# nianticlabs/panoptic-forecasting

Hardware: AMD Instinct MI355X
Metric: forecast frames/sec @1024x2048, 3-in->dt=3 bg (higher is better)
Workload: dtype f32 as 2 fp16 terms/operand, 3 MFMA products, f32 accumulate (strict f32: fp32_only); 1 GPU; configs[1] bg short-term forecast 3-in dt=3 @1024x2048: 3 warp/splats + HarDNet-70 + upsample/argmax; resident_frames_per_gpu=128, streams=4, sub_batch=32, launch=hipGraph replay, sub-batches staggered, weights=random-init, calibrated (tests/golden/calib_seed1234.json), world=1, device=AMD Radeon Graphics, backend=single process

## Files before the change

include/pfhip.h:

```cpp
#ifndef PFHIP_H
#define PFHIP_H

#include <stddef.h>
#include <stdint.h>

#ifdef __cplusplus
extern "C" {
#endif

#define PF_OK 0
#define PF_EINVAL (-1)
#define PF_EWORKSPACE (-2)
#define PF_EBLOB (-3)
#define PF_EHIP (-4)
#define PF_EUNSUPPORTED (-5)

typedef struct pf_plan pf_plan;

int pf_version(void);
const char *pf_last_error(void);

#define PF_SPLAT_PER_FRAME 1
#define PF_SPLAT_PER_SAMPLE_SENTINEL 2
int pf_warp_splat_workspace(int B, int T, int H, int W, int per_frame, size_t *bytes);
int pf_warp_splat(const float *depth, const uint8_t *depth_mask, const uint8_t *seg, int seg_channels,
                  const float *Kinv, const float *E, const float *T_tgt, const float *Einv,
                  const float *K, int B, int T_total, int t_first, int T, int H, int W, int per_frame,
                  uint8_t *out_seg, float *out_depth, int64_t *out_result2d,
                  void *ws, size_t ws_bytes, void *stream);

int pf_hardnet_plan_create(const void *blob_host, size_t bytes, int in_ch, int n_cls, pf_plan **out);
void pf_hardnet_plan_destroy(pf_plan *plan);
int pf_hardnet_workspace(const pf_plan *plan, int B, int H, int W, size_t *bytes);

#define PF_STATUS_RANGE 1u
#define PF_STATUS_RANGE_LOW 2u
#define PF_WS_STATUS_OFFSET 0
#define PF_WS_STICKY_OFFSET 4
#define PF_WS_STATUS_BYTES 2048
int pf_hardnet_status(const void *ws, unsigned *status, void *stream);
int pf_hardnet_status_sticky(void *ws, unsigned *status, int clear, void *stream);
int pf_hardnet_status_reset(void *ws, void *stream);
int pf_hardnet_range_maxima(const pf_plan *plan, const void *ws, float *maxima, int cap, int *n_ops, void *stream);

#define PF_HOP_NONE 0
#define PF_HOP_TRAINID_LUT 1
#define PF_HOP_DEPTH_U16 2

int pf_bg_forward(const pf_plan *plan, const void *seg, int seg_is_i64, const float *depth,
                  const uint8_t *depth_mask, float depth_mean, float depth_std, int hop_flags,
                  float min_depth, float max_depth, int B, int T, int H, int W, int out_h, int out_w,
                  void *out_seg, int out_seg_is_i64, float *out_logits, float *out_orig_logits,
                  void *ws, size_t ws_bytes, void *stream);

int pf_hardnet_forward_dense(const pf_plan *plan, const float *x, int B, int H, int W, int out_h,
                             int out_w, void *out_seg, int out_seg_is_i64, float *out_logits,
                             float *out_orig_logits, void *ws, size_t ws_bytes, void *stream);

int pf_hop_export(const void *seg, int seg_is_i64, int seg_mode, const float *depth, size_t n, uint8_t *out_seg,
                  uint16_t *out_depth_u16, void *stream);
int pf_hop_load(const uint16_t *depth_u16, size_t n, float min_depth, float max_depth, float *out_depth,
                uint8_t *out_mask, void *stream);

int pf_bg_augment(const uint8_t *seg_src, const uint8_t *label_src, const uint16_t *depth_src, int B, int T, int Hs, int Ws,
                  const int *y_map, const int *x_map, const int *y_arr, const int *x_arr, int oh, int ow, int pad_label,
                  float min_depth, float max_depth, uint8_t *out_seg, uint8_t *out_label, float *out_depth,
                  uint8_t *out_mask, void *stream);

int pf_fg_assemble(const float *bboxes, const uint8_t *feat_mask, const float *depth, const int32_t *classes,
                   const int32_t *feat_row, const float *feat_table, int N, int T, int T_in, int M, int use_ulbr,
                   double max_depth, double filter_car_gap, int img_w, float *trajectories, uint8_t *bbox_masks,
                   uint8_t *bbox_vel_masks, uint8_t *feat_masks, float *depths, uint8_t *depth_masks, int64_t *classes_out,
                   float *one_hot_classes, float *final_bboxes, float *feats, void *stream);

int pf_panoptic_merge_workspace(int n_instances, size_t *bytes);
int pf_panoptic_merge(const void *background, int bg_kind, const float *bg_depth, const uint8_t *bg_depth_mask,
                      const float *masks, int MH, int MW, const float *boxes, int box_is_ulbr,
                      const float *inst_depth, const int64_t *classes, const int32_t *inst_offsets,
                      int n_instances, int B, int H, int W, int use_depth_sorting, int panoptic_ids,
                      int clear_things, void *out, int out_is_i64, void *ws, size_t ws_bytes, void *stream);
int pf_panoptic_encode(const void *seg, int seg_is_i64, int convert_to_ids, int B, int H, int W, uint8_t *out_rgb,
                       int32_t *out_ids, uint8_t *out_present, void *stream);
int pf_panoptic_max_ids(void);

#define PF_PQ_STATUS_FULL 1u
#define PF_PQ_STATUS_VALUE 2u
int pf_pq_workspace(int B, size_t *bytes);
int pf_pq_table_slots(void);
int pf_pq_accumulate(const void *pred, int pred_is_i64, const void *gt, int gt_is_i64, int fmt, int crowd, int n_cls, int B,
                     int H, int W, double *acc, double *per_image, void *ws, size_t ws_bytes, void *stream);
int pf_pq_status(const void *ws, void *stream, int *host_status);
int pf_pq_status_reset(void *ws, void *stream);

int pf_bg_dense_input(const void *frames, int kind, int channels, const float *depth, const uint8_t *depth_mask, float depth_mean,
                      float depth_std, int B, int T, int H, int W, float *x, void *stream);

int pf_seg_loss_workspace(int B, int out_h, int out_w, size_t *bytes);
int pf_seg_loss(const float *logits, int B, int C, int Hin, int Win, const void *labels, int labels_i64, int out_h,
                int out_w, int ignore_index, double *out3, void *ws, size_t ws_bytes, void *stream);

int pf_fg_weights_size(int flags, size_t *raw_floats, size_t *packed_floats);
int pf_fg_pack(const float *raw, float *packed, int flags, void *stream);
int pf_fg_workspace(int N, int T_in, int T_out, int flags, size_t *bytes);
int pf_fg_forward(const float *packed, int flags, int N, int T_in, int T_out, int odom_T, const float *trajs,
                  const float *traj_mask, const float *vel_mask, const float *feats, const int64_t *output_inds,
                  const float *odom, const float *depths, const float *depth_mask, const int64_t *classes,
                  float *traj_norm, float *traj_unnorm, float *mask_feats, float *output_feats, float *masks,
                  void *ws, size_t ws_bytes, void *stream);

int pf_odom_weights_size(int flags, size_t *raw_floats, size_t *packed_floats);
int pf_odom_pack(const float *raw, float *packed, int flags, void *stream);
int pf_odom_forward(const float *packed, int flags, int B, int T_in, int T_out, const float *inps, float *out,
                    float *out_norm, void *stream);

int pf_odom_train_workspace(int B, int T_in, int T_out, int flags, size_t *bytes);
int pf_odom_train_forward(const float *packed, int flags, int B, int T_in, int T_out, const float *inps, float *out,
                          float *out_norm, void *ws, size_t ws_bytes, void *stream);
int pf_odom_backward(const float *packed, int flags, int B, int T_in, int T_out, const float *inps, const float *out_norm,
                     const float *grad_out, const float *grad_out_norm, void *ws, size_t ws_bytes, float *grad_raw,
                     void *stream);

int pf_set_option(const char *name, int value);
int pf_hardnet_plan_set_option(pf_plan *plan, const char *name, int value);

typedef struct pf_train pf_train;
int pf_train_create(const void *blob, size_t blob_bytes, int in_ch, int n_cls, pf_train **out);
void pf_train_destroy(pf_train *t);
int pf_train_autotune(pf_train *t, int enable);
int pf_train_tuned_shapes(const pf_train *t, int *rows, int cap_rows, int *n_rows);
int pf_train_path_stats(const pf_train *t, int *stats, int cap, int *n);
int pf_train_param_count(const pf_train *t, size_t *n_floats);
int pf_train_param_layout(const pf_train *t, int op_index, size_t *w_off, size_t *aux_off, int *has_bn);
int pf_train_workspace(const pf_train *t, int B, int H, int W, int out_h, int out_w, size_t *bytes);
int pf_train_forward_backward(const pf_train *t, float *theta, float *grad, int accumulate_grads, const void *seg, int seg_is_i64,
                              const float *depth, const uint8_t *depth_mask, float depth_mean, float depth_std, int T,
                              const float *x_dense, int B, int H, int W, const void *labels, int labels_i64, int out_h, int out_w,
                              int ignore_index, float loss_scale, float bn_momentum, float bn_eps, int update_running_stats,
                              double *out3, void *ws, size_t ws_bytes, void *stream);
int pf_train_tensor_view(const pf_train *t, const char *name, int want_grad, int B, int H, int W, int out_h, int out_w,
                         size_t *ws_offset, int *channels, int *h, int *w);
int pf_sgd_workspace(size_t *bytes);
int pf_sgd_step(float *theta, float *grad, float *momentum_buf, const uint8_t *trainable, size_t n, float lr, float momentum,
                float weight_decay, float clip_norm, float clip_value, int first_step, void *ws, size_t ws_bytes, void *stream);

int pf_hardnet_tensor_view(const pf_plan *plan, const char *name, int B, int H, int W,
                           size_t *ws_offset, int *channels, int *h, int *w);
int pf_hardnet_tensor_read(const pf_plan *plan, const char *name, int B, int H, int W, const void *ws, float *dst, void *stream);
int pf_s4_pack(const float *src, void *dst, int B, int C, int H, int W, unsigned *status, void *stream);
int pf_s4_unpack(const void *src, float *dst, int B, int C, int H, int W, void *stream);
int pf_hardnet_flops(const pf_plan *plan, int H, int W, double *flops);

int pf_profile_enable(int on);
int pf_profile_collect(void);
int pf_profile_get(int i, char *label, size_t label_cap, int *launches, double *total_ms, double *flops,
                   double *bytes);

int pf_debug_force_conv(int kind, int p0, int p1, int p2);
int pf_debug_conv_decision(int ks, int stride, int cin, int cout, int hout, int wout, int B, int need, int flags, int rounds,
                           int *out, int cap);
int pf_debug_conv_ranges(int form, int ks, int kc, int pad, int n_src, int n_cases, const int *choff, const int *ch, const int *ctotal,
                         int src_begin, int src_end, int *out, size_t cap);
int pf_debug_plan_arena(const void *blob, size_t bytes, int in_ch, int n_cls, float *out, size_t cap, size_t *n_floats,
                        long long *table, int table_ops);
int pf_debug_train_plan(const void *blob, size_t bytes, int in_ch, int n_cls, int B, int H, int W, int out_h, int out_w,
                        long long *regions, int cap_regions, int *n_regions, int *steps, int cap_steps, int *n_steps, int *slots_streams);
int pf_debug_probe_read(long long *host64);

#ifdef __cplusplus
}
#endif
#endif
```

panoptic-forecasting_amd/bg_model.py:

```python
import collections.abc
import ctypes

import torch
import torch.nn.functional as F
from torch import nn

from . import hardnet_arch as arch
from . import lib as _lib
from . import packing
from .model_api import BaseModel
from .pc_transform_model import _as_u8


PLAN_OPTIONS = {'split_f16': 'split_f16', 'split_bf16': 'split_f16', 'fuse_pool': 'fuse_pool', 'fuse_upsample': 'fuse_upsample',
                'use_tuned_table': 'use_tuned_table', 'valu_remainder': 'valu_remainder', 'conv_table_batch': 'table_batch',
                'range_guard': 'range_guard', 'fuse_front': 'fuse_front', 'fuse_pairs': 'fuse_pairs', 'share_s': 'share_s'}
PF_STATUS_RANGE, PF_STATUS_RANGE_LOW = 1, 2
PF_STATUS_ANY = PF_STATUS_RANGE | PF_STATUS_RANGE_LOW
PF_WS_STATUS_BYTES = 2048


class _Pending:
    __slots__ = ('slot', 'event', 'stream', 'args', 'outs', 'done', 'stamps', 'error')


def _stamp(t):
    if not torch.is_tensor(t):
        return None
    return (t.data_ptr(), None if t.is_inference() else t._version)


def _unversioned(stamps):
    return any(s is not None and s[1] is None for s in stamps)


class LazyResult(collections.abc.MutableMapping):

    __slots__ = ('_data', '_model', '_token')

    def __init__(self, data, model, token):
        self._data, self._model, self._token = dict(data), model, token

    def _resolve(self):
        if self._token is not None:
            self._model._resolve(self._token)
            self._token = None

    def __getitem__(self, k):
        self._resolve()
        return self._data[k]

    def __setitem__(self, k, v):
        self._data[k] = v

    def __delitem__(self, k):
        self._resolve()
        del self._data[k]

    def __iter__(self):
        return iter(self._data)

    def __len__(self):
        return len(self._data)

    def __contains__(self, k):
        return k in self._data

    def keys(self):
        return self._data.keys()

    def copy(self):
        self._resolve()
        return dict(self._data)

    def __or__(self, other):
        return {**self.copy(), **other}

    def __ror__(self, other):
        return {**other, **self.copy()}

    def __reduce__(self):
        return (dict, (self.copy(),))

    def __repr__(self):
        return 'LazyResult(%s%s)' % (list(self._data), ', unchecked' if self._token is not None else '')


class _Node(nn.Module):
    """Anonymous container: gives dotted state_dict paths without any behaviour."""


def _get_or_make(root, path):
    node = root
    for part in path:
        if not hasattr(node, part):
            node.add_module(part, _Node())
        node = getattr(node, part)
    return node


class HardNetParams(nn.Module):

    def __init__(self, in_ch, n_cls):
        super().__init__()
        self.spec = arch.Spec(in_ch, n_cls)
        for op in self.spec.conv_ops():
            parts = op.name.split('.')
            if op.bn:
                holder = _get_or_make(self, parts)
                cin = 3 if op.kind == arch.OP_STEM else op.cin
                holder.add_module('conv', nn.Conv2d(cin, op.cout, op.k, op.stride, op.k // 2, bias=False))
                holder.add_module('norm', nn.BatchNorm2d(op.cout))
            else:
                parent = _get_or_make(self, parts[:-1])
                conv = nn.Conv2d(op.cin, op.cout, op.k, op.stride, 0, bias=True)
                nn.init.kaiming_normal_(conv.weight)
                parent.add_module(parts[-1], conv)
        stem = getattr(self.base, '0').conv
        w = stem.weight.data.mean(1, keepdim=True).expand(-1, in_ch, -1, -1).clone()
        stem.weight = nn.Parameter(w)

    def load_pretrained(self, path):
        sd = torch.load(path, map_location='cpu')['model_state']
        sd = {k[len('module.'):]: v for k, v in sd.items()}
        own = self.state_dict()
        for k, v in sd.items():
            if k in own and own[k].shape == v.shape:
                own[k].copy_(v)
            elif k == 'base.0.conv.weight':
                own[k].copy_(v.mean(1, keepdim=True).expand_as(own[k]))


class BGModel(BaseModel):

    def __init__(self, params):
        super().__init__()
        self.num_classes = num_classes = params['data']['num_classes']
        self.use_depth_inps = params['model'].get('use_depth_inps')
        self.num_inputs = params['model'].get('num_inputs', 1)
        self.min_depth = params['data'].get('min_depth')
        self.max_depth = params['data'].get('max_depth')
        self.convert2onehot = params['model'].get('convert2onehot')
        self.return_logits = params['model'].get('return_logits', True)
        final_w = params['model'].get('final_w')
        final_h = params['model'].get('final_h')
        self.final_size = (final_h, final_w) if final_w is not None and final_h is not None else None
        in_ch = num_classes
        if self.use_depth_inps:
            depth_norm_params = params['data'].get('depth_norm_params')
            if depth_norm_params is None:
                mean, std = torch.zeros(1), torch.zeros(1)
            else:
                mean, std = depth_norm_params
            self.depth_mean = nn.Parameter(torch.as_tensor(mean, dtype=torch.float32).reshape(1).clone(),
                                           requires_grad=False)
            self.depth_std = nn.Parameter(torch.as_tensor(std, dtype=torch.float32).reshape(1).clone(),
                                          requires_grad=False)
            in_ch += 1
        in_ch *= self.num_inputs
        self.in_ch = in_ch
        self.model = HardNetParams(in_ch, num_classes)
        pretrain = params['model'].get('hardnet', {}).get('pretrain_path')
        if pretrain is not None:
            self.model.load_pretrained(pretrain)
        self.plan_options = {c_name: int(params['model'][key]) for key, c_name in PLAN_OPTIONS.items()
                             if params['model'].get(key) is not None}
        self.on_range_overflow = params['model'].get('on_range_overflow', 'rerun')
        if self.on_range_overflow not in ('rerun', 'raise', 'ignore'):
            raise ValueError("model.on_range_overflow must be 'rerun', 'raise' or 'ignore'")
        self.range_check = params['model'].get('range_check', 'lazy')
        if self.range_check not in ('lazy', 'sync'):
            raise ValueError("model.range_check must be 'lazy' or 'sync'")
        self.range_reruns = 0
        self._pending = []
        self._pinned = None
        self._ring_next = 0
        self._plan = None
        self._ws = None
        self._norm = None
        self._trainer = None
        self._params_for_trainer = {'data': dict(params['data']), 'model': dict(params['model']),
                                    'training': dict(params.get('training') or {})}

    def load_state_dict(self, state_dict, strict=True):
        res = super().load_state_dict(state_dict, strict)
        self.invalidate()
        return res

    def invalidate(self):
        if self._pending:
            self._drain()
        if self._plan is not None:
            _lib.load().pf_hardnet_plan_destroy(self._plan)
        self._plan = None
        self._norm = None

    def __del__(self):
        try:
            self._pending = []
            self.invalidate()
        except Exception:
            pass

    def _get_plan(self):
        if self._plan is None:
            L = _lib.load()
            blob = packing.pack_blob(self.state_dict(), self.in_ch, self.num_classes)
            buf = ctypes.create_string_buffer(blob, len(blob))
            plan = ctypes.c_void_p()
            _lib.check(L.pf_hardnet_plan_create(buf, len(blob), self.in_ch, self.num_classes, ctypes.byref(plan)),
                       'pf_hardnet_plan_create')
            self._plan = plan
            for name, value in self.plan_options.items():
                _lib.check(L.pf_hardnet_plan_set_option(plan, name.encode(), value), 'pf_hardnet_plan_set_option')
            if self.use_depth_inps:
                self._norm = (float(self.depth_mean.item()), float(self.depth_std.item()))
        return self._plan

    def _workspace(self, b, h, w, device):
        L = _lib.load()
        need = ctypes.c_size_t()
        _lib.check(L.pf_hardnet_workspace(self._get_plan(), b, h, w, ctypes.byref(need)), 'pf_hardnet_workspace')
        if self._ws is None or self._ws.numel() < need.value or self._ws.device != device:
            if torch.cuda.is_current_stream_capturing():
                raise _lib.PfError('bg forward: the workspace must exist before stream capture (run one forward first)')
            self._drain()
            self._ws = torch.empty(need.value, dtype=torch.uint8, device=device)
            self._ws[:PF_WS_STATUS_BYTES].zero_()
        return self._ws

    def _guarded(self):
        return not (self.on_range_overflow == 'ignore' or self.plan_options.get('split_f16', 1) == 0
                    or self.plan_options.get('range_guard', 1) == 0)

    def range_status(self):
        if self._ws is None:
            return 0
        return int(self._ws[:4].view(torch.int32).item())

    def range_status_sticky(self, clear=False):
        if self._ws is None:
            return 0
        w = self._ws[4:8].view(torch.int32)
        v = int(w.item())
        if clear:
            w.zero_()
        return v

    def check_range(self, clear=True):
        self._drain()
        v = self.range_status_sticky(clear)
        if (v & PF_STATUS_ANY) and self._guarded():
            raise _lib.PfError('bg forward: status %d (PF_STATUS_RANGE = 1: |activation| > 65504, PF_STATUS_RANGE_LOW = 2: a tensor of '
                               'tiny values) on the two-term fp16 operand path inside a captured graph: the outputs of the flagged '
                               'replays are not usable; run eagerly (re-run on fp32) or with model.split_f16 = 0' % v)
        return v

    def range_maxima(self):
        L, plan = _lib.load(), self._get_plan()
        names = [op.name for op in self.model.spec.ops]
        buf = (ctypes.c_float * len(names))()
        n = ctypes.c_int()
        _lib.check(L.pf_hardnet_range_maxima(plan, self._ws.data_ptr(), buf, len(names), ctypes.byref(n), _lib.stream_ptr()),
                   'pf_hardnet_range_maxima')
        return {names[i]: float(buf[i]) for i in range(n.value)}

    _RING = 32

    def _resolve(self, token, owner=True):
        if token.done:
            if token.error is not None and owner:
                raise token.error
            return
        if not token.event.query():
            token.event.synchronize()
        token.done = True
        if token in self._pending:
            self._pending.remove(token)
        status = int(self._pinned[token.slot, 0])
        args, outs, stamps = token.args, token.outs, token.stamps
        token.args = token.outs = token.stamps = None
        if not (status & PF_STATUS_ANY):
            return
        if self.on_range_overflow == 'raise':
            token.error = _lib.PfError('bg forward: status %d on the two-term fp16 operand path (PF_STATUS_RANGE = 1: an activation '
                                       'exceeded 65504; PF_STATUS_RANGE_LOW = 2: a tensor of tiny values, max below 2^-6); run with '
                                       "model.split_f16 = 0 or on_range_overflow = 'rerun'" % status)
        elif stamps is not None and stamps != tuple(_stamp(t) for t in args[:3]):
            token.error = _lib.PfError('bg forward: status %d on the two-term fp16 operand path, and the input tensors of that forward were '
                                       'modified in place before its result was first touched - the fp32 re-run cannot see the original '
                                       "frame.  Keep a forward's inputs unchanged until its result has been read (or model.settle()), or "
                                       "build the model with model.range_check = 'sync'" % status)
        if token.error is not None:
            if owner:
                raise token.error
            return
        L, plan = _lib.load(), self._get_plan()
        self.range_reruns += 1
        prior = self.plan_options.get('split_f16', 1)
        _lib.check(L.pf_hardnet_plan_set_option(plan, b'split_f16', 0), 'pf_hardnet_plan_set_option')
        try:
            here = torch.cuda.current_stream()
            with torch.cuda.stream(token.stream):
                self._run_once(*args, outs=outs)
            if here != token.stream:
                here.wait_stream(token.stream)
        finally:
            _lib.check(L.pf_hardnet_plan_set_option(plan, b'split_f16', prior), 'pf_hardnet_plan_set_option')

    def _poll(self):
        while self._pending and self._pending[0].event.query():
            self._resolve(self._pending[0], owner=False)

    def _drain(self):
        while self._pending:
            self._resolve(self._pending[0], owner=False)

    def settle(self):
        self._drain()

    def run_async(self, inps, depths, depth_masks, want_logits=True, want_orig=True, hop_flags=0, seg_dtype=torch.int64,
                  own_inputs=False):
        capturing = torch.cuda.is_current_stream_capturing()
        if not capturing:
            self._poll()
        args = (inps, depths, depth_masks, want_logits, want_orig, hop_flags, seg_dtype)
        outs = self._run_once(*args)
        if not self._guarded() or capturing:
            return outs, None
        if self._pinned is None:
            self._pinned = torch.zeros((self._RING, 2), dtype=torch.int32).pin_memory()
        slot = self._ring_next
        self._ring_next = (slot + 1) % self._RING
        for t in list(self._pending):
            if t.slot == slot:
                self._resolve(t, owner=False)
        self._pinned[slot].copy_(self._ws[:8].view(torch.int32), non_blocking=True)
        token = _Pending()
        token.slot, token.args, token.outs, token.done, token.error = slot, args, outs, False, None
        token.stamps = None if own_inputs else tuple(_stamp(t) for t in args[:3])
        token.stream = torch.cuda.current_stream()
        token.event = torch.cuda.Event()
        token.event.record(token.stream)
        self._pending.append(token)
        if token.stamps is not None and _unversioned(token.stamps):
            self._resolve(token)
            return outs, None
        return outs, token

    def run(self, inps, depths, depth_masks, want_logits=True, want_orig=True, hop_flags=0, seg_dtype=torch.int64):
        outs, token = self.run_async(inps, depths, depth_masks, want_logits, want_orig, hop_flags, seg_dtype)
        if token is not None:
            self._resolve(token)
        return outs

    def _run_once(self, inps, depths, depth_masks, want_logits, want_orig, hop_flags, seg_dtype, outs=None):
        L = _lib.load()
        plan = self._get_plan()
        fused = bool(self.convert2onehot and self.use_depth_inps and inps.dim() == 4)
        if fused:
            b, t, h, w = inps.shape
        else:
            x = self._dense_input(inps, depths, depth_masks)
            b, _, h, w = x.shape
        dev = inps.device
        oh, ow = self.final_size if self.final_size is not None else (h, w)
        ws = self._workspace(b, h, w, dev)
        if outs is not None:
            seg, logits, orig = outs
        else:
            seg = torch.empty((b, oh, ow), dtype=seg_dtype, device=dev)
            logits = torch.empty((b, self.num_classes, oh, ow), dtype=torch.float32, device=dev) if want_logits else None
            orig = None
            if want_orig:
                vo, vc, vh, vw = ctypes.c_size_t(), ctypes.c_int(), ctypes.c_int(), ctypes.c_int()
                _lib.check(L.pf_hardnet_tensor_view(plan, b'finalConv', b, h, w, ctypes.byref(vo), ctypes.byref(vc),
                                                    ctypes.byref(vh), ctypes.byref(vw)), 'pf_hardnet_tensor_view')
                orig = torch.empty((b, vc.value, vh.value, vw.value), dtype=torch.float32, device=dev)
        ptr = lambda t_: t_.data_ptr() if t_ is not None else None
        i64 = int(seg_dtype == torch.int64)
        if fused:
            if inps.dtype not in (torch.uint8, torch.int64):
                inps = inps.long()
            inps = _lib.require_cuda(inps.contiguous(), 'seg')
            depths = _lib.require_cuda(depths.float().contiguous(), 'depth')
            mask = None
            if not (hop_flags & 2):
                mask = _lib.require_cuda(_as_u8(depth_masks), 'depth_mask')
            mean, std = self._norm
            rc = L.pf_bg_forward(plan, inps.data_ptr(), int(inps.dtype == torch.int64), depths.data_ptr(), ptr(mask),
                                 mean, std, hop_flags, float(self.min_depth or 0.0), float(self.max_depth or 0.0),
                                 b, t, h, w, oh, ow, seg.data_ptr(), i64, ptr(logits), ptr(orig),
                                 ws.data_ptr(), ws.numel(), _lib.stream_ptr())
            _lib.check(rc, 'pf_bg_forward')
        else:
            x = _lib.require_cuda(x.contiguous(), 'input')
            rc = L.pf_hardnet_forward_dense(plan, x.data_ptr(), b, h, w, oh, ow, seg.data_ptr(), i64, ptr(logits),
                                            ptr(orig), ws.data_ptr(), ws.numel(), _lib.stream_ptr())
            _lib.check(rc, 'pf_hardnet_forward_dense')
        return seg, logits, orig

    def _dense_input(self, inps, depths, depth_masks):
        L = _lib.load()
        if self.convert2onehot:
            b, t, h, w = inps.shape
            if inps.dtype not in (torch.uint8, torch.int64):
                inps = inps.long()
            frames, kind, c = _lib.require_cuda(inps.contiguous(), 'seg'), int(inps.dtype == torch.int64), self.num_classes
        else:
            b, t, c, h, w = inps.shape
            frames, kind = _lib.require_cuda(inps.float().contiguous(), 'seg'), 2
        dptr = mptr = None
        mean = std = 0.0
        if self.use_depth_inps:
            depths = _lib.require_cuda(depths.float().contiguous(), 'depth')
            mask = _lib.require_cuda(_as_u8(depth_masks), 'depth_mask')
            dptr, mptr = depths.data_ptr(), mask.data_ptr()
            self._get_plan()
            mean, std = self._norm
        x = torch.empty((b, t * c + (t if self.use_depth_inps else 0), h, w), dtype=torch.float32, device=inps.device)
        _lib.check(L.pf_bg_dense_input(frames.data_ptr(), kind, c, dptr, mptr, mean, std, b, t, h, w, x.data_ptr(), _lib.stream_ptr()),
                   'pf_bg_dense_input')
        return x

    def forward(self, inps, depths, depth_masks, return_orig_size=False):
        _, logits, orig = self.run(inps, depths, depth_masks, True, return_orig_size)
        return (logits, orig) if return_orig_size else logits

    def loss(self, inputs, labels):
        if self.training:
            return self._train_loss(inputs, labels)
        with torch.no_grad():
            return self._eval_loss(inputs, labels)

    def _get_trainer(self):
        from . import bg_train
        if self._trainer is None:
            self._trainer = bg_train.BGTrainer(self._params_for_trainer, device='cuda')
        if not self._trainer.is_adopted():
            self._trainer.adopt(self)
        return self._trainer

    def _train_loss(self, inputs, labels):
        from . import bg_train
        tr = self._get_trainer()
        self.invalidate()
        loss, acc = bg_train.TrainStepFunction.apply(tr, inputs, labels, *tr._adopted)
        torch._foreach_add_(self._bn_counters(), 1)
        return {'loss': loss, 'accuracy': acc}

    def _bn_counters(self):
        return [b for k, b in self.named_buffers() if k.endswith('num_batches_tracked')]

    def _eval_loss(self, inputs, labels):
        L = _lib.load()
        seg_labels = labels['seg']
        _, _, orig = self.run(inputs['seg'], inputs.get('depth'), inputs.get('depth_mask'), want_logits=False, want_orig=True)
        if seg_labels.dtype not in (torch.uint8, torch.int64):
            seg_labels = seg_labels.long()
        seg_labels = _lib.require_cuda(seg_labels.contiguous(), 'labels')
        b, c, hin, win = orig.shape
        oh, ow = seg_labels.shape[-2], seg_labels.shape[-1]
        need = ctypes.c_size_t()
        _lib.check(L.pf_seg_loss_workspace(b, oh, ow, ctypes.byref(need)), 'pf_seg_loss_workspace')
        ws = torch.empty(need.value, dtype=torch.uint8, device=orig.device)
        out3 = torch.empty(3, dtype=torch.float64, device=orig.device)
        _lib.check(L.pf_seg_loss(orig.data_ptr(), b, c, hin, win, seg_labels.data_ptr(), int(seg_labels.dtype == torch.int64), oh, ow,
                                 255, out3.data_ptr(), ws.data_ptr(), ws.numel(), _lib.stream_ptr()), 'pf_seg_loss')
        return {'loss': (out3[0] / out3[1]).float(), 'accuracy': (out3[2] / out3[1]).float()}

    @torch.no_grad()
    def predict(self, inputs, labels=None):
        (seg, logits, orig), token = self.run_async(inputs['seg'], inputs.get('depth'), inputs.get('depth_mask'),
                                                    want_logits=self.return_logits, want_orig=True)
        out = {'seg': seg, 'orig_size_logits': orig}
        if logits is not None:
            out['logits'] = logits
        if token is not None and self.range_check == 'sync':
            self._resolve(token)
            token = None
        return LazyResult(out, self, token)
```

panoptic-forecasting_amd/csrc/conv_mfma.h:

```cpp
#pragma once
#include "pf_blob.h"
#include "pf_common.h"

namespace pf {

struct ConvArgs {
    const float *src[kConvMaxSrc];
    int src_ctotal[kConvMaxSrc];
    int src_choff[kConvMaxSrc];
    int src_cstart[kConvMaxSrc + 1];
    int src_chunk0[kConvMaxSrc + 1];
    int n_src;
    const float *wpk;
    const float *bias;
    float *dst;
    int dst_ctotal, dst_choff;
    int Cin, Cout, Hin, Win, Hout, Wout;
    int tilesX, tilesY, nchunks, relu;
    const float *zero_page;
    int ntiles;
    int no_bias;
    int pool;
    const float *res;
    int res_ctotal, res_choff, Hres, Wres;
    float res_sh, res_sw;
    int res_lds_off;
    int res_rows, res_cols;
    unsigned res_magic_cs, res_magic_cols;
    const float *wrem;
    int rem;
    int src_begin, src_end;
    int chunk_begin, chunk_end;
    long long *probe;
    unsigned *status;
    unsigned *range_slot;
    int kacc;
    int accum;
    float acc_scale;
    int dst_fmt;
    int dst_c4;
    int dst_limit;
    int src_fmt;
    int src_c4[kConvMaxSrc];
    int src_g0[kConvMaxSrc];
    int src_gn[kConvMaxSrc];
    int src_ent0[kConvMaxSrc + 1];
    float *share;
    int share_off;
    int share_cout;
    float share_scale;
};

typedef _Float16 split_t;
typedef split_t split_x2 __attribute__((ext_vector_type(2)));
typedef split_t split_x4 __attribute__((ext_vector_type(4)));
typedef split_t split_x8 __attribute__((ext_vector_type(8)));
constexpr float kSplitMaxAbs = 65504.f;
__device__ __forceinline__ void split_terms2(float x0, float x1, split_x2 &hi, split_x2 &mid) {
#if defined(__HIP_DEVICE_COMPILE__)
    typedef float f32x2 __attribute__((ext_vector_type(2)));
    hi = __builtin_convertvector(f32x2{x0, x1}, split_x2);
    const unsigned hu = __builtin_bit_cast(unsigned, hi);
    unsigned mu;
    asm("v_fma_mixlo_f16 %0, %1, -1.0, %2 op_sel_hi:[1,0,0]" : "=v"(mu) : "v"(hu), "v"(x0));
    asm("v_fma_mixhi_f16 %0, %1, -1.0, %2 op_sel:[1,0,0] op_sel_hi:[1,0,0]" : "+v"(mu) : "v"(hu), "v"(x1));
    mid = __builtin_bit_cast(split_x2, mu);
#endif
}
__device__ __forceinline__ float range_acc(float m, float a, float b, float c, float d) {
#if defined(__HIP_DEVICE_COMPILE__)
    asm("v_max3_f32 %0, %0, |%1|, |%2|" : "+v"(m) : "v"(a), "v"(b));
    asm("v_max3_f32 %0, %0, |%1|, |%2|" : "+v"(m) : "v"(c), "v"(d));
#endif
    return m;
}
constexpr float kRangeTarget = 8.0f;
constexpr float kRangeLowMax = 0.015625f;
__device__ __forceinline__ bool range_sampled() {
#if defined(__HIP_DEVICE_COMPILE__)
    const unsigned total = gridDim.x * gridDim.y * gridDim.z;
    const unsigned id = blockIdx.x + gridDim.x * (blockIdx.y + gridDim.y * blockIdx.z);
    const unsigned mask = total >= 16u ? (1u << (28 - __builtin_clz(total))) - 1u : 0u;
    return (((id * 0x9E3779B1u) >> 9) & mask) == 0u;
#else
    return false;
#endif
}
__device__ __forceinline__ void range_commit(unsigned *status, unsigned *slot, float m) {
#if defined(__HIP_DEVICE_COMPILE__)
    if (status == nullptr) return;
    if (!(m <= kSplitMaxAbs)) atomicOr(status, 1u);
    if (slot == nullptr || !range_sampled()) return;
    const unsigned mb = __builtin_bit_cast(unsigned, m);
    unsigned wm = 0;
    unsigned long long above = __builtin_amdgcn_ballot_w64(mb > wm);
    while (above != 0) {
        wm = (unsigned)__builtin_amdgcn_readlane((int)mb, (int)__builtin_ctzll(above));
        above = __builtin_amdgcn_ballot_w64(mb > wm);
    }
    const unsigned lane_id = __builtin_amdgcn_mbcnt_hi(~0u, __builtin_amdgcn_mbcnt_lo(~0u, 0u));
    if (lane_id == (unsigned)__builtin_ctzll(__builtin_amdgcn_ballot_w64(true))) atomicMax(slot, wm | 1u);
#endif
}
template <typename V4>
__device__ __forceinline__ void split_terms4(const V4 &v, split_x4 &hi, split_x4 &mid) {
    split_x2 h0, m0, h1, m1;
    split_terms2(v[0], v[1], h0, m0);
    split_terms2(v[2], v[3], h1, m1);
    hi = split_x4{h0[0], h0[1], h1[0], h1[1]};
    mid = split_x4{m0[0], m0[1], m1[0], m1[1]};
}
#define PF_MFMA_SPLIT(a, b, c) __builtin_amdgcn_mfma_f32_16x16x32_f16((a), (b), (c), 0, 0, 0)
unsigned short split_host_f16(float x);
float split_host_f32(unsigned short h);
float split_weight_scale(const float *w, size_t n);

__device__ __forceinline__ void xcd_tile_order(int ntiles_xy, int &tile_lin, int &group) {
#if defined(__HIP_DEVICE_COMPILE__)
    if ((ntiles_xy & 7) != 0) {
        tile_lin = (int)blockIdx.x;
        group = (int)blockIdx.y;
        return;
    }
    const int ngroups = (int)gridDim.y;
    const int lin = (int)blockIdx.x + ntiles_xy * (int)blockIdx.y;
    const int xcd = lin & 7, pos = lin >> 3;
    const int t = pos / ngroups;
    group = pos - t * ngroups;
    tile_lin = xcd * (ntiles_xy >> 3) + t;
#endif
}

struct ConvTiling {
    int ks, stride;
    int kc;
    int nt;
    int twt;
    int cout_blocks, nchunks;
    size_t packed_floats() const { return (size_t)cout_blocks * nchunks * (kc / 4) * ks * ks * nt * 64; }
};

ConvTiling choose_tiling(int ks, int stride, int cin, int cout, int wout_hint);
void pack_conv_weights(const float *w_oihw, int cin, int cout, const ConvTiling &t, float *out);
int launch_conv(const ConvArgs &a, const ConvTiling &t, int B, hipStream_t stream);

constexpr int dma_kc_ct(int ks, int stride) { return ks == 1 ? 16 : (stride == 2 ? 4 : 8); }
inline int dma_kc(int ks, int stride) { return dma_kc_ct(ks, stride); }
inline int dma_rem_rv(int rem) { return rem <= 2 ? 2 : (rem + 3) / 4 * 4; }
inline int dma_valu_split(int cout) {
    if (cout < 16) return 0;
    return cout % 16;
}
void pack_conv_weights_rem(const float *w_oihw, int cin, int cout, int rem, int ks, int kc, const int *src_ch, int n_src, float *out);
void pack_conv_weights_tiled(const float *w_oihw, int cin, int cout, int ks, int kc, const int *src_ch, int n_src, float *out);
int launch_conv_dma(const ConvArgs &a, int ks, int stride, int B, hipStream_t stream, int force_wm = 0, int force_nt = 0, int model_B = 0);
bool conv_dma_supported(const ConvArgs &a, int ks, int stride, int B, int force_wm, int force_nt, int model_B, int *wm, int *nt);

constexpr int wave_kc_ct(int ks) { return ks == 1 ? 32 : 8; }
inline int wave_kc(int ks) { return wave_kc_ct(ks); }
void pack_conv_weights_wave(const float *w_oihw, int cin, int cout, int ks, const int *src_ch, int n_src, float *out);
size_t wave_packed_floats(const int *src_ch, int n_src, int cout, int ks);
int launch_conv_wave(const ConvArgs &a, int ks, int mh, int nt, int wk, int B, hipStream_t stream);
bool conv_wave_supported(const ConvArgs &a, int ks, int mh, int nt, int wk);
constexpr size_t wave_lds_bytes(int ks, int mh, int nt, int wk) {
    const int kc = wave_kc_ct(ks), ih = mh + ks - 1, iw = 16 + (ks == 3 ? 8 : 0);
    const int raw = ih * iw, plane = (raw + 15) / 32 * 32 + 16, nit = (kc * (plane / 4) + 63) / 64;
    const size_t ring = (size_t)wk * 2 * nit * 256, red = (size_t)wk * mh * nt * 256;
    return 4 * (ring > red ? ring : red);
}

size_t split_packed_floats(const int *src_ch, int n_src, int cout);
void pack_conv_weights_split(const float *w_oihw, int cin, int cout, const int *src_ch, int n_src, float *out);
int launch_conv_split(const ConvArgs &a, int nt, int wide, int B, hipStream_t stream);
bool conv_split_supported(const ConvArgs &a);
size_t split1_packed_floats(const int *src_ch, int n_src, int cout);
void pack_conv_weights_split1(const float *w_oihw, int cin, int cout, const int *src_ch, int n_src, float *out);
int launch_conv_split1(const ConvArgs &a, int nt, int B, hipStream_t stream);
bool conv_split1_supported(const ConvArgs &a, int nt);

struct S4Range { int choff, ch; };
struct KOrder;
size_t s4_packed_floats(const KOrder &k, int cout, int ks, int pad_sources);
void pack_conv_weights_s4(const float *w_oihw, int cin, int cout, int ks, const KOrder &k, int pad_sources, float *out);
enum S4Tile : int { S4_8x32 = 0, S4_8x64 = 1, S4_16x32 = 2, S4_8x32_K2 = 3, S4_8x32_K4 = 4 };
struct S4Shape { int NT, TW, TH, KS; };
S4Shape s4_resolve(int ks, int nt, int tile, int ntiles, int rounds, bool kacc);
int launch_conv_s4(const ConvArgs &a, int ks, const S4Shape &shape, int B, hipStream_t stream);
int launch_conv_s4_share(const ConvArgs &a, int nt, int B, hipStream_t stream);
int launch_conv_s4_add(const ConvArgs &a, int nt, int B, hipStream_t stream);
inline int share_row0(int p_cout) { return (p_cout + 3) / 4 * 4; }
bool share_wanted(int p_cin, int p_cout, int c_cin, int c_cout, int h, int w, int B, int mode);

struct PairArgs {
    ConvArgs c;
    const float *p_wpk;
    const float *p_w9;
    const float *p_bias;
    float p_acc_scale;
    float *p_dst;
    int p_dst_c4, p_dst_choff, p_dst_limit, p_cout, p_cin, p_ntiles, p_relu;
    unsigned *p_range_slot;
    int rounds_s;
    int round_d;
    int merged;
};
bool conv_pair_supports(int c_cout, int p_cout);
bool conv_pair_merged_supports(int c_cout, int p_cout);
bool pair_wanted(int p_cin, int p_cout, int c_cin, int c_cout, int h, int w, int B, int mode);
size_t pair_p_two_floats(const S4Range &r, int cout);
size_t pair_p_nine_floats(const S4Range &r, int cout);
void pack_conv_weights_pair_p(const float *w_oihw, int cin, int cout, const S4Range &r, float *two, float *nine);
int launch_conv_pair(const PairArgs &pa, int B, hipStream_t stream);
int launch_s4_pack(const float *src, void *dst, int B, int C, int H, int W, unsigned *status, hipStream_t stream);
int launch_range_check(const float *x, size_t n, unsigned *status, unsigned *slot, hipStream_t stream);
int launch_range_finalize(unsigned *st, int live_word, int first_slot, int n_slots, int sticky_word, hipStream_t stream);
int launch_s4_unpack(const void *src, float *dst, int B, int C, int H, int W, hipStream_t stream);

struct FrontArgs {
    const void *x;
    const void *w1, *w2;
    const float *bias1, *bias2;
    float scale1, scale2;
    float *dst;
    int dst_fmt, dst_c4, dst_ctotal, dst_choff, dst_limit;
    int H1, W1, H2, W2, C1, C2, relu1, relu2;
    int tilesX, tilesY;
    int seg_steps;
    unsigned *status;
    unsigned *range_slot_mid, *range_slot;
    long long *probe;
};

bool conv_front_supports(int c0, int c1, int c2, int h1, int w1, int dst_ctotal);
int launch_conv_front(const FrontArgs &a, int B, hipStream_t s);

enum ConvKind : int { CONV_AUTO = 0, CONV_DMA = 1, CONV_WAVE = 2, CONV_SPLIT = 4, CONV_S4 = 5 };
struct ConvChoice {
    int kind, p0, p1, p2;
    static ConvChoice dma(int wm = 0, int nt = 0) { return {CONV_DMA, wm, nt, 0}; }
    static ConvChoice wave(int mh, int nt, int wk) { return {CONV_WAVE, mh, nt, wk}; }
    static ConvChoice split(int nt, int wide) { return {CONV_SPLIT, nt, wide, 0}; }
    bool is(ConvKind k) const { return kind == k; }
    int dma_wm() const { return p0; }
    int dma_nt() const { return p1; }
    int wave_mh() const { return p0; }
    int wave_nt() const { return p1; }
    int wave_wk() const { return p2; }
    int split_nt() const { return p0; }
    int split_wide() const { return p1; }
    int s4_nt() const { return p0; }
    int s4_tile() const { return p1; }
};
ConvChoice choose_conv(int ks, int stride, int cin, int cout, int hout, int wout, int B, int need = 0, int use_tuned = 1);
bool choose_s4(int ks, int cin, int cout, int hout, int wout, int B, ConvChoice *out);
struct ConvQuery {
    int ks, stride, cin, cout, hout, wout;
    int B;
    int need;
    bool generic;
    bool has_split, has_s4;
    bool use_tuned, split_f16, kacc;
    int rounds;
    ConvChoice force;
};
struct ConvDecision {
    ConvChoice ch;
    bool wants_s4;
    int s4_nt, s4_tile;
    S4Shape s4;
};
ConvDecision decide_conv(const ConvQuery &q);
long long *probe_buffer();
ConvChoice conv_force();
inline bool conv_forced() { return !conv_force().is(CONV_AUTO); }
inline bool force_allows_s4() { return !conv_forced() || conv_force().is(CONV_S4); }
inline bool forced_dma_shape(int *wm, int *nt) {
    const ConvChoice f = conv_force();
    if (!f.is(CONV_DMA) || f.dma_wm() <= 0) return false;
    *wm = f.dma_wm(); *nt = f.dma_nt();
    return true;
}

}
```

panoptic-forecasting_amd/csrc/conv_s4.hip:

```cpp
#include <cstring>
#include <vector>

#include "conv_ranges.h"
#include "conv_s4.h"
#include "pf_prof.h"

#ifndef PF_PROBE
#define PF_PROBE 0
#endif
#if PF_PROBE
#define S4_PROBE(i) do { if (threadIdx.x == 0 && blockIdx.x == gridDim.x / 2 && blockIdx.y == 0 && blockIdx.z == gridDim.z / 2 && a.probe && (i) < 60) a.probe[i] = clock64(); } while (0)
#else
#define S4_PROBE(i) do { } while (0)
#endif

[[maybe_unused]] constexpr int kS4IssueFirst = 1, kS4IssueStep = 2;

namespace pf {

template <int NT, int TW_, int TH_ = 8, int KS_ = 1>
struct S4Cfg {
    static constexpr int TW = TW_, TH = TH_, MTR = TW / 16, MP = 2 * MTR;
    static constexpr int KS = KS_;
    static constexpr int NW = TH / 2, NTHR = 64 * NW;
    static constexpr int IW = TW + 4, IH = TH + 2;
    static constexpr int ROWP = IW / 2, PIECES = IH * ROWP;
    static constexpr int NDMA_ALL = (PIECES + 63) / 64;
    static constexpr int NDMA = (NDMA_ALL + NW / 4 - 1) / (NW / 4);
    static constexpr bool COLREG = (NT == 2 || NT == 3) && TW_ == 32;
    static constexpr int PLANE = COLREG ? PIECES * 16 : NDMA_ALL * 64 * 16;
    static constexpr int ABUF = 4 * PLANE;
    static constexpr int WBLK = 2 * 64 * 16;
    static constexpr int BPT = COLREG ? 2 : 3;
    static constexpr int WBUF = NT * BPT * WBLK;
    static constexpr int WPIECES = WBUF / 16, NITW = (WPIECES + NTHR - 1) / NTHR;
    static constexpr size_t STAGES_BYTES = 2 * (size_t)ABUF + 2 * (size_t)WBUF;
    static constexpr size_t LDS_BYTES = KS * STAGES_BYTES + NT * 16 * sizeof(float);
    static_assert(KS == 1 || (size_t)MP * NT * NW * 64 * 16 <= STAGES_BYTES, "the K-split hand-over uses group 1's stage ring");
};

#define S4_KERNEL_NAME conv_s4_kernel
#define S4_KERNEL_KACC 0
#define S4_KERNEL_EPI 0
#define S4_KERNEL_WAVES (KS_ == 4 ? 1 : (TH_ == 16 || KS_ == 2) ? 2 : (TW_ == 32 && NT <= 2) ? 4 : (TW_ == 32 && NT == 3) ? 3 : 2)
#include "conv_s4_kernel.inc"
#undef S4_KERNEL_NAME
#undef S4_KERNEL_EPI
#define S4_KERNEL_NAME conv_s4_share_kernel
#define S4_KERNEL_EPI 1
#include "conv_s4_kernel.inc"
#undef S4_KERNEL_NAME
#undef S4_KERNEL_EPI
#define S4_KERNEL_NAME conv_s4_add_kernel
#define S4_KERNEL_EPI 2
#include "conv_s4_kernel.inc"
#undef S4_KERNEL_NAME
#undef S4_KERNEL_EPI
#undef S4_KERNEL_KACC
#undef S4_KERNEL_WAVES
#define S4_KERNEL_NAME conv_s4_blocked_kernel
#define S4_KERNEL_KACC 1
#define S4_KERNEL_EPI 0
#define S4_KERNEL_WAVES (NT == 1 ? 4 : (NT == 2 ? 3 : 2))
#include "conv_s4_kernel.inc"
#undef S4_KERNEL_NAME
#undef S4_KERNEL_KACC
#undef S4_KERNEL_EPI
#undef S4_KERNEL_WAVES

enum S4Form { S4_PLAIN, S4_BLOCKED, S4_SHARE, S4_ADD };
template <S4Form FORM, int NT, int TW_, int TH_, int KS_>
static constexpr auto s4_kernel() {
    if constexpr (FORM == S4_PLAIN) return &conv_s4_kernel<NT, TW_, TH_, KS_>;
    else if constexpr (FORM == S4_BLOCKED) return &conv_s4_blocked_kernel<NT, TW_, TH_, KS_>;
    else if constexpr (FORM == S4_SHARE) return &conv_s4_share_kernel<NT, TW_, TH_, KS_>;
    else return &conv_s4_add_kernel<NT, TW_, TH_, KS_>;
}
template <S4Form FORM, int NT, int TW_ = 32, int TH_ = 8, int KS_ = 1>
static int launch_s4_form(const ConvArgs &a0, int B, hipStream_t s) {
    using C = S4Cfg<NT, TW_, TH_, KS_>;
    constexpr auto kernel = s4_kernel<FORM, NT, TW_, TH_, KS_>();
    constexpr const char *name = FORM == S4_PLAIN ? "conv_s4_kernel" : FORM == S4_BLOCKED ? "conv_s4_blocked_kernel"
                               : FORM == S4_SHARE ? "conv_s4_share_kernel" : "conv_s4_add_kernel";
    ConvArgs a = a0;
    a.tilesX = (a.Wout + C::TW - 1) / C::TW;
    a.tilesY = (a.Hout + C::TH - 1) / C::TH;
    static bool attr_set = false;
    if (!attr_set) {
        PF_HIP_CHECK(hipFuncSetAttribute(reinterpret_cast<const void *>(kernel), hipFuncAttributeMaxDynamicSharedMemorySize, (int)C::LDS_BYTES));
        attr_set = true;
    }
    char label[96];
    snprintf(label, sizeof(label), "void pf::%s<%d, %d, %d, %d>(pf::ConvArgs)", name, NT, TW_, TH_, KS_);
    const double px = (double)B * a.Hout * a.Wout;
    const int rows = FORM == S4_SHARE ? a.Cout + a.share_cout : a.Cout;
    const double sums = FORM == S4_SHARE || FORM == S4_ADD ? (double)(a.share_cout + 3) / 4 * 4 : 0.0;
    ProfScope ps(s, label, 2.0 * px * rows * a.Cin * 9, 4.0 * ((double)B * a.Cin * a.Hin * a.Win + px * (a.Cout + sums) + (double)rows * a.Cin * 9));
    hipLaunchKernelGGL(kernel, dim3(a.tilesX * a.tilesY, (a.ntiles + NT - 1) / NT, B), dim3(C::NTHR * C::KS), C::LDS_BYTES, s, a);
    PF_LAUNCH_CHECK(name);
    return PF_OK;
}

static int check_share(const ConvArgs &a, const char *who) {
    if (!a.src_fmt || !a.dst_fmt) return fail(PF_EINVAL, "%s: sources and destination in the S4 layout only", who);
    if ((a.Wout & 3) != 0 || a.Hin != a.Hout || a.Win != a.Wout) return fail(PF_EUNSUPPORTED, "%s: stride 1, width %% 4 == 0 only", who);
    if (a.pool || a.res || a.no_bias || a.kacc) return fail(PF_EUNSUPPORTED, "%s: no fused epilogue stages", who);
    if (a.chunk_begin != 0 || a.chunk_end != a.nchunks) return fail(PF_EUNSUPPORTED, "%s: whole K range only", who);
    if (!a.share || a.share_cout < 1 || (reinterpret_cast<uintptr_t>(a.share) & 15) != 0) return fail(PF_EINVAL, "%s: no scratch tensor", who);
    return PF_OK;
}
#define PF_S4_SHARE(FORM_) \
    nt = nt < 1 ? 1 : (nt > a.ntiles ? a.ntiles : nt); \
    if (nt == 1) return launch_s4_form<FORM_, 1>(a, B, s); \
    if (nt == 2) return launch_s4_form<FORM_, 2>(a, B, s); \
    return launch_s4_form<FORM_, 3>(a, B, s);
int launch_conv_s4_share(const ConvArgs &a, int nt, int B, hipStream_t s) {
    if (int rc = check_share(a, "conv_s4 share")) return rc;
    if ((a.share_off & 3) != 0 || a.share_off < a.Cout || a.share_off + a.share_cout > a.ntiles * 16)
        return fail(PF_EINVAL, "conv_s4 share: rows %d + %d in %d tiles", a.share_off, a.share_cout, a.ntiles);
    PF_S4_SHARE(S4_SHARE)
}
int launch_conv_s4_add(const ConvArgs &a, int nt, int B, hipStream_t s) {
    if (int rc = check_share(a, "conv_s4 add")) return rc;
    if (a.share_cout != a.Cout) return fail(PF_EINVAL, "conv_s4 add: stored sums of %d channels for %d", a.share_cout, a.Cout);
    PF_S4_SHARE(S4_ADD)
}
#undef PF_S4_SHARE

template <int NT>
struct S41Cfg {
    static constexpr int TW = 32, TH = 8, MP = 4;
    static constexpr int WBUF = NT * 2 * 64 * 16;
    static constexpr int BIAS_OFF = 2 * WBUF;
    static constexpr int MAIN = 2 * WBUF + 256;
    static constexpr int WPIECES = WBUF / 16, NITW = (WPIECES + 255) / 256;
};

typedef unsigned s4_u32x4 __attribute__((ext_vector_type(4)));
typedef unsigned s4_u32x2 __attribute__((ext_vector_type(2)));

template <int NT, int EPI>
__global__ __launch_bounds__(256, NT <= 2 ? 4 : (NT == 3 ? 3 : 2)) void conv_s4_1x1_kernel(ConvArgs a) {
#if defined(__HIP_DEVICE_COMPILE__)
    using C = S41Cfg<NT>;
    extern __shared__ __attribute__((aligned(16))) unsigned char smem_raw[];
    const int tid = threadIdx.x, lane = tid & 63;
    const int wave = __builtin_amdgcn_readfirstlane(tid >> 6);
    int tid_lin, cgroup;
    xcd_tile_order(a.tilesX * a.tilesY, tid_lin, cgroup);
    const int tileY = tid_lin / a.tilesX, tileX = tid_lin - tileY * a.tilesX;
    const int tile0 = cgroup * NT, b = blockIdx.z;
    const size_t plane_bytes = (size_t)a.Hin * a.Win * 8;
    auto wbuf = [&](int i) { return smem_raw + i * C::WBUF; };
    const int g = lane >> 4;

    s4_f32x4 acc[C::MP][NT];
#pragma unroll
    for (int m = 0; m < C::MP; ++m)
#pragma unroll
        for (int n = 0; n < NT; ++n) acc[m][n] = s4_f32x4{0.f, 0.f, 0.f, 0.f};
    const bool has_res = EPI == 1 && a.res && a.res_lds_off >= 0;
    ResWin rw = ResWin();

    int poff[2];
#pragma unroll
    for (int rr = 0; rr < 2; ++rr) {
        const int gy = tileY * C::TH + 2 * wave + rr, gx = tileX * C::TW + 2 * (lane & 15);
        poff[rr] = (gy < a.Hin && gx < a.Win) ? (gy * a.Win + gx) * 8 : -1;
    }
    unsigned woff[C::NITW];
#pragma unroll
    for (int it = 0; it < C::NITW; ++it) {
        const int p = it * 256 + tid, n = p / (2 * 64);
        woff[it] = (p < C::WPIECES && tile0 + n < a.ntiles) ? (unsigned)((tile0 + n) * a.nchunks * (2 * 64) + (p - n * (2 * 64))) * 16u : kS4Oob;
    }
    const __amdgpu_buffer_rsrc_t wrsrc = __builtin_amdgcn_make_buffer_rsrc((void *)a.wpk, 0, 0x7FFFFFFF, 0x00020000);

    float *bias_lds = reinterpret_cast<float *>(smem_raw + C::BIAS_OFF);
    if (wave == 0 && lane < NT * 16) {
        const __amdgpu_buffer_rsrc_t brs = __builtin_amdgcn_make_buffer_rsrc((void *)a.bias, 0, 0x7FFFFFFF, 0x00020000);
        const int co = tile0 * 16 + lane;
        __builtin_amdgcn_raw_ptr_buffer_load_lds(brs, (s4_lds_ptr_t)bias_lds, 4, (!a.no_bias && co < a.ntiles * 16) ? (unsigned)co * 4u : kS4Oob, 0,
                                                 0, 0);
    }

    const int cb = a.chunk_begin, nrounds = a.chunk_end - cb;
    auto load_round = [&](int r, s4_u32x4 (&x)[2][2][2]) {
#pragma unroll
        for (int h = 0; h < 2; ++h) {
            const int e = 8 * (cb + r) + 2 * g + h;
            const float *sp = a.src[0];
            int c4 = a.src_c4[0], g0 = a.src_g0[0], gn = a.src_gn[0], e0 = 0;
#pragma unroll
            for (int k = 1; k < kConvMaxSrc; ++k) {
                const bool take = k < a.n_src && e >= a.src_ent0[k];
                sp = take ? a.src[k] : sp;
                c4 = take ? a.src_c4[k] : c4;
                g0 = take ? a.src_g0[k] : g0;
                gn = take ? a.src_gn[k] : gn;
                e0 = take ? a.src_ent0[k] : e0;
            }
            const bool real = e - e0 < gn;
            const char *hi = reinterpret_cast<const char *>(sp) + ((size_t)b * 2 * c4 + (g0 + min(e - e0, gn - 1))) * plane_bytes;
            const size_t tstride = (size_t)c4 * plane_bytes;
#pragma unroll
            for (int rr = 0; rr < 2; ++rr) {
                const bool ok = real && poff[rr] >= 0;
                const char *p = ok ? hi + poff[rr] : reinterpret_cast<const char *>(a.zero_page);
                x[rr][h][0] = *reinterpret_cast<const s4_u32x4 *>(p);
                x[rr][h][1] = *reinterpret_cast<const s4_u32x4 *>(ok ? p + tstride : p);
            }
        }
    };
    auto load_weights = [&](int r, unsigned char *wdst) {
#pragma unroll
        for (int it = 0; it < C::NITW; ++it)
            if (it * 256 + tid < C::WPIECES)
                __builtin_amdgcn_raw_ptr_buffer_load_lds(wrsrc, (s4_lds_ptr_t)(wdst + (it * 256 + wave * 64) * 16), 16, woff[it],
                                                         (unsigned)(cb + r) * (2 * 64 * 16), 0, 0);
    };

    s4_u32x4 cur[2][2][2], nxt[2][2][2];
    if (nrounds > 0) {
        load_weights(0, wbuf(0));
        load_round(0, cur);
    }
    if (has_res) {
        rw = res_window(a, tileY * C::TH, C::TH, tileX * C::TW, C::TW);
        rw.rows = a.res_rows;
        rw.cols = a.res_cols;
        rw.cs = res_chan_stride(a.res_rows, a.res_cols);
        const unsigned per = (unsigned)(rw.rows * rw.cols), total = (unsigned)(NT * 16 * rw.cs);
        const size_t rplane = (size_t)a.Hres * a.Wres;
        const __amdgpu_buffer_rsrc_t rrs = __builtin_amdgcn_make_buffer_rsrc(
            (void *)(a.res + ((size_t)b * a.res_ctotal + a.res_choff + tile0 * 16) * rplane), 0, 0x7FFFFFFF, 0x00020000);
        unsigned char *rdst = smem_raw + a.res_lds_off * 4;
        for (unsigned e0 = (unsigned)wave * 64; e0 < total; e0 += 256) {
            const unsigned e = e0 + lane;
            const unsigned c = __umulhi(e, a.res_magic_cs), rem = e - c * (unsigned)rw.cs;
            const unsigned r = __umulhi(rem, a.res_magic_cols), x = rem - r * (unsigned)rw.cols;
            const int row = min(rw.sy0 + (int)r, a.Hres - 1), col = min(rw.sx0 + (int)x, a.Wres - 1);
            const bool ok = e < total && rem < per && tile0 * 16 + (int)c < a.Cout;
            const unsigned off = ok ? (unsigned)((c * rplane + (size_t)row * a.Wres + col) * 4) : kS4Oob;
            __builtin_amdgcn_raw_ptr_buffer_load_lds(rrs, (s4_lds_ptr_t)(rdst + e0 * 4), 4, off, 0, 0, 0);
        }
    }

    for (int round = 0; round < nrounds; ++round) {
        asm volatile("s_waitcnt vmcnt(0)" ::: "memory");
        __syncthreads();
        const bool more = round + 1 < nrounds;
        if (more) {
            load_weights(round + 1, wbuf((round + 1) & 1));
            load_round(round + 1, nxt);
        }
        const unsigned char *wb = wbuf(round & 1);
        s4_h8 bh[NT], bm[NT];
#pragma unroll
        for (int n = 0; n < NT; ++n) {
            bh[n] = *reinterpret_cast<const s4_h8 *>(wb + ((n * 2 + 0) * 64 + lane) * 16);
            bm[n] = *reinterpret_cast<const s4_h8 *>(wb + ((n * 2 + 1) * 64 + lane) * 16);
        }
#pragma unroll
        for (int rr = 0; rr < 2; ++rr)
#pragma unroll
            for (int q = 0; q < 2; ++q) {
                const s4_u32x4 h0 = cur[rr][0][0], h1 = cur[rr][1][0], m0 = cur[rr][0][1], m1 = cur[rr][1][1];
                const s4_u32x4 fh = q ? s4_u32x4{h0[2], h0[3], h1[2], h1[3]} : s4_u32x4{h0[0], h0[1], h1[0], h1[1]};
                const s4_u32x4 fm = q ? s4_u32x4{m0[2], m0[3], m1[2], m1[3]} : s4_u32x4{m0[0], m0[1], m1[0], m1[1]};
                const s4_h8 ah = __builtin_bit_cast(s4_h8, fh), am = __builtin_bit_cast(s4_h8, fm);
                const int m = rr * 2 + q;
#pragma unroll
                for (int n = 0; n < NT; ++n) acc[m][n] = PF_MFMA_SPLIT(bh[n], am, acc[m][n]);
#pragma unroll
                for (int n = 0; n < NT; ++n) acc[m][n] = PF_MFMA_SPLIT(bm[n], ah, acc[m][n]);
#pragma unroll
                for (int n = 0; n < NT; ++n) acc[m][n] = PF_MFMA_SPLIT(bh[n], ah, acc[m][n]);
            }
        if (more) {
#pragma unroll
            for (int rr = 0; rr < 2; ++rr)
#pragma unroll
                for (int h = 0; h < 2; ++h)
#pragma unroll
                    for (int t = 0; t < 2; ++t) cur[rr][h][t] = nxt[rr][h][t];
        }
    }

    if (has_res) {
        asm volatile("s_waitcnt vmcnt(0)" ::: "memory");
        __syncthreads();
    }
    {
        __builtin_amdgcn_s_waitcnt(0x0F70);
        const lds_float *res_lds = (const lds_float *)(reinterpret_cast<float *>(smem_raw) + (has_res ? a.res_lds_off : 0));
        const int i2 = 2 * (lane & 15);
        const int ox = tileX * C::TW + i2;
        const bool pooled = EPI == 1 && a.pool;
        const int Ho = pooled ? a.Hout >> 1 : a.Hout, Wo = pooled ? a.Wout >> 1 : a.Wout;
        const size_t hw = (size_t)Ho * Wo, term = (size_t)a.dst_c4 * hw * 8;
        const bool mis = (a.dst_choff & 2) != 0;
        typedef split_x2 h2;
        float vmax = 0.f;
        const float relu_lo1 = a.relu ? 0.f : -__builtin_inff();
        auto finish = [&](int rr, int q, int n, const int (&o0)[2], const int (&o1)[2], const float (&lx1)[2], float hy1) {
            s4_f32x4 v = acc[rr * 2 + q][n];
            const s4_f32x4 b4 = *reinterpret_cast<const s4_f32x4 *>(bias_lds + n * 16 + 4 * g);
#pragma unroll
            for (int r = 0; r < 4; ++r) {
                v[r] = v[r] * a.acc_scale + b4[r];
                if (has_res) {
                    const lds_float *chan = res_lds + (n * 16 + 4 * g + r) * rw.cs;
                    const float lx0 = 1.f - lx1[q], hy0 = 1.f - hy1;
                    const float t0 = lx0 * chan[o0[q]] + lx1[q] * chan[o0[q] + 1];
                    const float t1 = lx0 * chan[o1[q]] + lx1[q] * chan[o1[q] + 1];
                    v[r] += hy0 * t0 + hy1 * t1;
                }
                v[r] = fmaxf(v[r], relu_lo1);
            }
            vmax = range_acc(vmax, v[0], v[1], v[2], v[3]);
            return v;
        };
        auto store_px = [&](int co, size_t pix, s4_f32x4 v) {
            if (a.dst_fmt) {
                s4_h4 hi, mid;
                split_terms4(v, hi, mid);
                const int chb = a.dst_choff + co;
                const bool ok0 = chb < a.dst_limit, ok1 = chb + 2 < a.dst_limit;
                char *p = reinterpret_cast<char *>(a.dst) + (size_t)b * 2 * term + pix * 8 + (size_t)(chb >> 2) * hw * 8;
                if (!mis) {
                    if (ok1) {
                        *reinterpret_cast<s4_h4 *>(p) = hi;
                        *reinterpret_cast<s4_h4 *>(p + term) = mid;
                    } else if (ok0) {
                        *reinterpret_cast<h2 *>(p) = h2{hi[0], hi[1]};
                        *reinterpret_cast<h2 *>(p + term) = h2{mid[0], mid[1]};
                    }
                } else {
                    if (ok0) {
                        *reinterpret_cast<h2 *>(p + 4) = h2{hi[0], hi[1]};
                        *reinterpret_cast<h2 *>(p + 4 + term) = h2{mid[0], mid[1]};
                    }
                    if (ok1) {
                        *reinterpret_cast<h2 *>(p + hw * 8) = h2{hi[2], hi[3]};
                        *reinterpret_cast<h2 *>(p + hw * 8 + term) = h2{mid[2], mid[3]};
                    }
                }
            } else {
#pragma unroll
                for (int r = 0; r < 4; ++r)
                    if (co + r < a.Cout) a.dst[((size_t)b * a.dst_ctotal + a.dst_choff + co + r) * hw + pix] = v[r];
            }
        };
        auto store_pair = [&](int co, size_t pix, s4_f32x4 v0, s4_f32x4 v1) {
            const int chb = a.dst_choff + co;
            if (a.dst_fmt && !mis && chb + 2 < a.dst_limit) {
                s4_h4 h0, m0, h1, m1;
                split_terms4(v0, h0, m0);
                split_terms4(v1, h1, m1);
                const s4_h8 hi = s4_join(h0, h1), mid = s4_join(m0, m1);
                char *p = reinterpret_cast<char *>(a.dst) + (size_t)b * 2 * term + pix * 8 + (size_t)(chb >> 2) * hw * 8;
                *reinterpret_cast<s4_h8 *>(p) = hi;
                *reinterpret_cast<s4_h8 *>(p + term) = mid;
            } else if (!a.dst_fmt) {
                typedef float f2 __attribute__((ext_vector_type(2)));
#pragma unroll
                for (int r = 0; r < 4; ++r)
                    if (co + r < a.Cout)
                        *reinterpret_cast<f2 *>(a.dst + ((size_t)b * a.dst_ctotal + a.dst_choff + co + r) * hw + pix) = f2{v0[r], v1[r]};
            } else {
                store_px(co, pix, v0);
                store_px(co, pix + 1, v1);
            }
        };
#pragma unroll
        for (int rr = 0; rr < 2; ++rr) {
            if (pooled && rr == 1) continue;
            const int oy = tileY * C::TH + 2 * wave + rr;
            if (oy >= a.Hout || ox >= a.Wout) continue;
            if (pooled && oy + 1 >= a.Hout) continue;
            int o0[2] = {0, 0}, o1[2] = {0, 0}, p0[2] = {0, 0}, p1[2] = {0, 0};
            float lx1[2] = {0.f, 0.f}, hy1 = 0.f, hy1b = 0.f;
            if (has_res) {
                int y0, y1;
                float hy0;
                lin_coord(oy, a.res_sh, a.Hres, y0, y1, hy0, hy1);
                int z0 = 0, z1 = 0;
                if (pooled) lin_coord(oy + 1, a.res_sh, a.Hres, z0, z1, hy0, hy1b);
#pragma unroll
                for (int q = 0; q < 2; ++q) {
                    int x0, x1;
                    float lx0;
                    lin_coord(min(ox + q, a.Wout - 1), a.res_sw, a.Wres, x0, x1, lx0, lx1[q]);
                    o0[q] = (y0 - rw.sy0) * rw.cols + (x0 - rw.sx0);
                    o1[q] = (y1 - rw.sy0) * rw.cols + (x0 - rw.sx0);
                    p0[q] = (z0 - rw.sy0) * rw.cols + (x0 - rw.sx0);
                    p1[q] = (z1 - rw.sy0) * rw.cols + (x0 - rw.sx0);
                }
            }
#pragma unroll
            for (int n = 0; n < NT; ++n) {
                const int co = (tile0 + n) * 16 + 4 * g;
                if (co >= a.Cout + 2) continue;
                const s4_f32x4 va = finish(rr, 0, n, o0, o1, lx1, hy1), vb = finish(rr, 1, n, o0, o1, lx1, hy1);
                if (!pooled) {
                    store_pair(co, (size_t)oy * a.Wout + ox, va, vb);
                } else {
                    const s4_f32x4 vc = finish(1, 0, n, p0, p1, lx1, hy1b), vd = finish(1, 1, n, p0, p1, lx1, hy1b);
                    s4_f32x4 pv;
#pragma unroll
                    for (int r = 0; r < 4; ++r) pv[r] = (((va[r] + vb[r]) + vc[r]) + vd[r]) * 0.25f;
                    if ((oy >> 1) < Ho && (ox >> 1) < Wo) store_px(co, (size_t)(oy >> 1) * Wo + (ox >> 1), pv);
                }
                __builtin_amdgcn_sched_barrier(0);
            }
        }
        range_commit(a.status, a.range_slot, vmax);
    }
#endif
}

template <int NT, int EPI>
static int launch_s41_cfg(const ConvArgs &a0, int B, hipStream_t s) {
    using C = S41Cfg<NT>;
    ConvArgs a = a0;
    a.tilesX = (a.Wout + C::TW - 1) / C::TW;
    a.tilesY = (a.Hout + C::TH - 1) / C::TH;
    size_t lds = C::MAIN;
    a.res_lds_off = -1;
    if (a.res) {
        a.res_rows = res_extent(C::TH, a.res_sh);
        a.res_cols = res_extent(C::TW, a.res_sw);
        const int cs = res_chan_stride(a.res_rows, a.res_cols);
        const size_t need = (size_t)NT * 16 * cs * sizeof(float);
        if (need > 64 * 1024 || (size_t)NT * 16 * cs >= 65536) return fail(PF_EUNSUPPORTED, "conv_s4 1x1: residual window of %zu B does not fit LDS", need);
        a.res_magic_cs = (unsigned)(0x100000000ull / (unsigned)cs) + 1u;
        a.res_magic_cols = (unsigned)(0x100000000ull / (unsigned)a.res_cols) + 1u;
        a.res_lds_off = C::MAIN / 4;
        lds = C::MAIN + align_up(need, 256);
    }
    static size_t attr_lds = 0;
    if (lds > attr_lds) {
        PF_HIP_CHECK(hipFuncSetAttribute(reinterpret_cast<const void *>(&conv_s4_1x1_kernel<NT, EPI>),
                                         hipFuncAttributeMaxDynamicSharedMemorySize, (int)lds));
        attr_lds = lds;
    }
    char label[112];
    snprintf(label, sizeof(label), "void pf::conv_s4_1x1_kernel<%d, %d>(pf::ConvArgs)", NT, EPI);
    if (a.res) strncat(label, " +res", sizeof(label) - strlen(label) - 1);
    if (a.pool) strncat(label, " +pool", sizeof(label) - strlen(label) - 1);
    if (a.no_bias) strncat(label, " lowres-half", sizeof(label) - strlen(label) - 1);
    const double px = (double)B * a.Hout * a.Wout;
    ProfScope ps(s, label, 2.0 * px * a.Cout * a.Cin, 4.0 * ((double)B * a.Cin * a.Hin * a.Win + px * a.Cout + (double)a.Cout * a.Cin));
    hipLaunchKernelGGL((conv_s4_1x1_kernel<NT, EPI>), dim3(a.tilesX * a.tilesY, (a.ntiles + NT - 1) / NT, B), dim3(256), lds, s, a);
    PF_LAUNCH_CHECK("conv_s4_1x1_kernel");
    return PF_OK;
}

int launch_conv_s4(const ConvArgs &a, int ks, const S4Shape &sh, int B, hipStream_t s) {
    if (!a.src_fmt) return fail(PF_EINVAL, "conv_s4: sources are not in the S4 layout");
    if ((a.Wout & 3) != 0 || a.Hin != a.Hout || a.Win != a.Wout) return fail(PF_EUNSUPPORTED, "conv_s4: stride 1, width % 4 == 0 only");
    if (ks == 3) {
        if (a.pool || a.res || a.no_bias) return fail(PF_EUNSUPPORTED, "conv_s4 3x3: no fused epilogue stages");
        if (a.chunk_begin != 0 || a.chunk_end != a.nchunks) return fail(PF_EUNSUPPORTED, "conv_s4 3x3: whole K range only");
#define PF_S4(FORM_, NT_, TW_, TH_, KS_) \
    if (sh.NT == NT_ && sh.TW == TW_ && sh.TH == TH_ && sh.KS == KS_) return launch_s4_form<FORM_, NT_, TW_, TH_, KS_>(a, B, s);
        if (a.kacc) {
            PF_S4(S4_BLOCKED, 1, 32, 8, 1) PF_S4(S4_BLOCKED, 2, 32, 8, 1) PF_S4(S4_BLOCKED, 3, 32, 8, 1)
        } else {
            PF_S4(S4_PLAIN, 1, 32, 8, 1) PF_S4(S4_PLAIN, 2, 32, 8, 1) PF_S4(S4_PLAIN, 3, 32, 8, 1)
            PF_S4(S4_PLAIN, 4, 32, 8, 1)
            PF_S4(S4_PLAIN, 1, 64, 8, 1) PF_S4(S4_PLAIN, 2, 64, 8, 1)
            PF_S4(S4_PLAIN, 1, 32, 16, 1) PF_S4(S4_PLAIN, 2, 32, 16, 1)
            PF_S4(S4_PLAIN, 1, 32, 8, 2) PF_S4(S4_PLAIN, 2, 32, 8, 2)
            PF_S4(S4_PLAIN, 1, 32, 8, 4) PF_S4(S4_PLAIN, 2, 32, 8, 4)
        }
#undef PF_S4
    } else if (sh.TW == 32 && sh.TH == 8 && sh.KS == 1) {
        const bool fused = a.pool || a.res || a.no_bias;
#define PF_S41(NT_) \
    if (sh.NT == NT_) return fused ? launch_s41_cfg<NT_, 1>(a, B, s) : launch_s41_cfg<NT_, 0>(a, B, s);
        PF_S41(1) PF_S41(2) PF_S41(3) PF_S41(4)
#undef PF_S41
    }
    return fail(PF_EUNSUPPORTED, "conv_s4 %dx%d: shape <%d, %d, %d, %d> is not built", ks, ks, sh.NT, sh.TW, sh.TH, sh.KS);
}

size_t s4_packed_floats(const KOrder &k, int cout, int ks, int pad_sources) {
    const int rounds = s4_rounds(k, ks, pad_sources);
    return (size_t)((cout + 15) / 16) * (ks == 3 ? s4_blocks_total(rounds) : rounds) * 2 * 64 * 4;
}

void pack_conv_weights_s4(const float *w, int cin, int cout, int ks, const KOrder &k, int pad_sources, float *out_f) {
    unsigned short *out = reinterpret_cast<unsigned short *>(out_f);
    std::vector<int> ent_c0, ent_lo, ent_hi;
    const int per = s4_per_round(ks);
    for (int j = 0; j < k.n; ++j) {
        const KRange &r = k.r[j];
        const int g0 = r.choff / 4;
        for (int g = g0; g < g0 + s4_range_groups(r.choff, r.ch); ++g) {
            ent_c0.push_back(r.cstart + 4 * g - r.choff);
            ent_lo.push_back(r.cstart);
            ent_hi.push_back(r.cstart + r.ch);
        }
        while (pad_sources && ent_c0.size() % per != 0) {
            ent_c0.push_back(0);
            ent_lo.push_back(0);
            ent_hi.push_back(0);
        }
    }
    const int n_ent = (int)ent_c0.size(), rounds = (n_ent + per - 1) / per, ntiles = (cout + 15) / 16;
    size_t o = 0;
    auto block = [&](int t, auto ent_of, auto tap_of) {
        for (int term = 0; term < 2; ++term)
            for (int lane = 0; lane < 64; ++lane)
                for (int e = 0; e < 8; ++e) {
                    const int co = t * 16 + (lane & 15), g = lane >> 4;
                    const int ent = ent_of(g, e / 4), tap = tap_of(g);
                    float v = 0.f;
                    if (co < cout && tap >= 0 && ent >= 0 && ent < n_ent) {
                        const int ci = ent_c0[ent] + (e & 3);
                        if (ci >= ent_lo[ent] && ci < ent_hi[ent]) v = w[((size_t)co * cin + ci) * ks * ks + tap];
                    }
                    const unsigned short hi = split_host_f16(v);
                    out[o++] = term == 0 ? hi : split_host_f16(v - split_host_f32(hi));
                }
    };
    static const int tap3[2][4] = {{0, 1, 3, 4}, {6, 7, 2, 5}};
    for (int t = 0; t < ntiles; ++t)
        for (int rd = 0; rd < rounds; ++rd) {
            if (ks == 1) {
                block(t, [&](int g, int h) { return rd * 8 + g * 2 + h; }, [](int) { return 0; });
                continue;
            }
            for (int s = 0; s < 2; ++s) block(t, [&](int, int h) { return rd * 2 + h; }, [&](int g) { return tap3[s][g]; });
            if ((rd & 3) == 3 || rd == rounds - 1) {
                const int q = rd / 4;
                block(t, [&](int g, int h) { return 4 * q + g < rounds ? (4 * q + g) * 2 + h : -1; }, [](int) { return 8; });
            }
        }
}

__global__ void s4_pack_kernel(const float *src, unsigned short *dst, int B, int C, int H, int W, unsigned *status) {
    const size_t hw = (size_t)H * W, c4 = (C + 3) / 4, n = (size_t)B * c4 * hw;
    bool bad = false;
    for (size_t i = (size_t)blockIdx.x * blockDim.x + threadIdx.x; i < n; i += (size_t)gridDim.x * blockDim.x) {
        const size_t px = i % hw, g = (i / hw) % c4, b = i / (hw * c4);
        for (int r = 0; r < 4; ++r) {
            const int c = (int)g * 4 + r;
            const float x = c < C ? src[((size_t)b * C + c) * hw + px] : 0.f;
            bad = bad || !(fabsf(x) <= kSplitMaxAbs);
            split_x2 h, m;
            split_terms2(x, 0.f, h, m);
            dst[(((b * 2 + 0) * c4 + g) * hw + px) * 4 + r] = __builtin_bit_cast(unsigned short, h[0]);
            dst[(((b * 2 + 1) * c4 + g) * hw + px) * 4 + r] = __builtin_bit_cast(unsigned short, m[0]);
        }
    }
    if (bad && status) atomicOr(status, 1u);
}
__global__ void range_check_kernel(const float *x, size_t n, unsigned *status, unsigned *slot) {
    bool bad = false;
    float m = 0.f;
    const size_t n4 = n / 4;
    for (size_t i = (size_t)blockIdx.x * blockDim.x + threadIdx.x; i < n4; i += (size_t)gridDim.x * blockDim.x) {
        const s4_f32x4 v = reinterpret_cast<const s4_f32x4 *>(x)[i];
        bad = bad || !(fabsf(v[0]) <= kSplitMaxAbs) || !(fabsf(v[1]) <= kSplitMaxAbs) || !(fabsf(v[2]) <= kSplitMaxAbs) ||
              !(fabsf(v[3]) <= kSplitMaxAbs);
        m = range_acc(m, v[0], v[1], v[2], v[3]);
    }
    if (blockIdx.x == 0 && threadIdx.x < n - n4 * 4) {
        const float t = x[n4 * 4 + threadIdx.x];
        bad = bad || !(fabsf(t) <= kSplitMaxAbs);
        m = range_acc(m, t, 0.f, 0.f, 0.f);
    }
    if (bad) atomicOr(status, 1u);
    range_commit(status, slot, m);
}
int launch_range_check(const float *x, size_t n, unsigned *status, unsigned *slot, hipStream_t s) {
    if (!status || n == 0) return PF_OK;
    if ((reinterpret_cast<uintptr_t>(x) & 15) != 0) return fail(PF_EINVAL, "range check: input is not 16-B aligned");
    const size_t blocks = (n / 4 + 255) / 256;
    hipLaunchKernelGGL(range_check_kernel, dim3((unsigned)(blocks < 2048 ? (blocks ? blocks : 1) : 2048)), dim3(256), 0, s, x, n, status, slot);
    PF_LAUNCH_CHECK("range_check_kernel");
    return PF_OK;
}
__global__ void range_finalize_kernel(unsigned *st, int live_word, int first_slot, int n_slots, unsigned low_bits, int sticky_word) {
    __shared__ unsigned low;
    if (threadIdx.x == 0) low = 0;
    __syncthreads();
    for (int i = threadIdx.x; i < n_slots; i += blockDim.x) {
        const unsigned v = st[first_slot + i];
        if ((v & ~1u) != 0 && v < low_bits) low = 1;
        st[first_slot + n_slots + i] = v;
        st[first_slot + i] = 0;
    }
    __syncthreads();
    if (threadIdx.x == 0) {
        const unsigned w = st[live_word] | (low ? 2u : 0u);
        st[0] = w;
        st[sticky_word] |= w;
        st[live_word] = 0;
    }
}
int launch_range_finalize(unsigned *st, int live_word, int first_slot, int n_slots, int sticky_word, hipStream_t s) {
    hipLaunchKernelGGL(range_finalize_kernel, dim3(1), dim3(256), 0, s, st, live_word, first_slot, n_slots,
                       __builtin_bit_cast(unsigned, kRangeLowMax), sticky_word);
    PF_LAUNCH_CHECK("range_finalize_kernel");
    return PF_OK;
}
__global__ void s4_unpack_kernel(const unsigned short *src, float *dst, int B, int C, int H, int W) {
    const size_t hw = (size_t)H * W, c4 = (C + 3) / 4, n = (size_t)B * C * hw;
    for (size_t i = (size_t)blockIdx.x * blockDim.x + threadIdx.x; i < n; i += (size_t)gridDim.x * blockDim.x) {
        const size_t px = i % hw, c = (i / hw) % C, b = i / (hw * C);
        const size_t at = ((c / 4) * hw + px) * 4 + (c & 3);
        const unsigned short h = src[(b * 2 + 0) * c4 * hw * 4 + at], m = src[(b * 2 + 1) * c4 * hw * 4 + at];
        dst[i] = (float)__builtin_bit_cast(split_t, h) + (float)__builtin_bit_cast(split_t, m);
    }
}
int launch_s4_pack(const float *src, void *dst, int B, int C, int H, int W, unsigned *status, hipStream_t s) {
    hipLaunchKernelGGL(s4_pack_kernel, dim3(1024), dim3(256), 0, s, src, (unsigned short *)dst, B, C, H, W, status);
    PF_LAUNCH_CHECK("s4_pack_kernel");
    return PF_OK;
}
int launch_s4_unpack(const void *src, float *dst, int B, int C, int H, int W, hipStream_t s) {
    hipLaunchKernelGGL(s4_unpack_kernel, dim3(1024), dim3(256), 0, s, (const unsigned short *)src, dst, B, C, H, W);
    PF_LAUNCH_CHECK("s4_unpack_kernel");
    return PF_OK;
}

}
```

panoptic-forecasting_amd/csrc/conv_select.cpp:

```cpp
#include "conv_mfma.h"

namespace pf {

namespace {
ConvChoice g_conv_force = {CONV_AUTO, 0, 0, 0};
struct Tuned {
    int ks, cin, cout, hout, wout, B;
    ConvChoice c;
};
const Tuned kTuned[] = {
#include "conv_tuned.inc"
};

const Tuned kTunedS4[] = {
    {0, 0, 0, 0, 0, 0, {0, 0, 0, 0}},
#include "conv_s4_tuned.inc"
};

}

namespace {
bool measured_geometry(int ks, int cin, int cout, int hout, int wout, int B, int *ht, int *wt, double *b_eq, bool *exact) {
    const Tuned *first = nullptr;
    for (const Tuned &t : kTunedS4) {
        if (t.B <= 0 || t.ks != ks || t.cin != cin || t.cout != cout) continue;
        if (t.hout == hout && t.wout == wout) {
            *ht = hout;
            *wt = wout;
            *exact = true;
            *b_eq = (double)B;
            return true;
        }
        if (!first) first = &t;
    }
    if (!first) return false;
    *ht = first->hout;
    *wt = first->wout;
    *exact = false;
    *b_eq = (double)B * hout * wout / ((double)first->hout * first->wout);
    return *b_eq >= 0.5;
}
}

bool choose_s4(int ks, int cin, int cout, int hout, int wout, int B, ConvChoice *out) {
    int ht, wt;
    double b_eq;
    bool exact;
    if (!measured_geometry(ks, cin, cout, hout, wout, B, &ht, &wt, &b_eq, &exact)) return false;
    const Tuned *best = nullptr;
    double best_d = 0.0;
    for (const Tuned &t : kTunedS4) {
        if (t.ks != ks || t.cin != cin || t.cout != cout || t.hout != ht || t.wout != wt || t.B <= 0) continue;
        const double d = t.B > b_eq ? (double)t.B / b_eq : b_eq / (double)t.B;
        if (!best || d < best_d || (d == best_d && t.B > best->B)) { best = &t; best_d = d; }
    }
    if (!best) return false;
    *out = best->c;
    return true;
}

bool pair_wanted(int p_cin, int p_cout, int c_cin, int c_cout, int h, int w, int B, int mode) {
    if (mode == 4) return conv_pair_merged_supports(c_cout, p_cout);
    if (mode >= 2) return true;
    if (mode <= 0) return false;
    const long px = (long)B * h * w;
    return c_cout <= 32 && p_cout <= 16 && px >= 65536 && px <= 196608;
}

bool share_wanted(int p_cin, int p_cout, int c_cin, int c_cout, int h, int w, int B, int mode) {
    if (mode >= 2) return true;
    if (mode <= 0) return false;
    const int packed = (share_row0(p_cout) + c_cout + 15) / 16, apart = (p_cout + 15) / 16 + (c_cout + 15) / 16;
    if (packed >= apart || pair_wanted(p_cin, p_cout, c_cin, c_cout, h, w, B, 1)) return false;
    return p_cout == 10 && c_cout == 18 && p_cin >= 48 && (long)B * h * w >= 4194304;
}

ConvChoice choose_conv(int ks, int stride, int cin, int cout, int hout, int wout, int B, int need, int use_tuned) {
    if (stride != 1) return ConvChoice::dma();
    int Bt = B, ht = hout, wt = wout;
    if (use_tuned) {
        double b_eq = (double)B;
        bool exact = true;
        if (!measured_geometry(ks, cin, cout, hout, wout, B, &ht, &wt, &b_eq, &exact)) { ht = hout; wt = wout; b_eq = (double)B; }
        const int measured[6] = {1, 2, 4, 8, 16, 32};
        Bt = measured[5];
        for (int m : measured)
            if ((double)m >= b_eq) { Bt = (m > 1 && (double)m != b_eq && b_eq * b_eq < (double)m * (m / 2)) ? m / 2 : m; break; }
    }
    for (const Tuned &t : kTuned)
        if (use_tuned && t.ks == ks && t.cin == cin && t.cout == cout && t.hout == ht && t.wout == wt && t.B == Bt &&
            (!(need & 2) || !t.c.is(CONV_WAVE) || t.c.wave_mh() != 1))
            return t.c;
    if (ks == 3 && (need == 0) && (wout & 3) == 0 && (long)B * hout * wout >= 32768) {
        const int nt = cout <= 16 ? 1 : (cout <= 32 ? 2 : 3);
        const long tiles_wide = (long)B * ((hout + 7) / 8) * ((wout + 63) / 64) * (((cout + 15) / 16 + nt - 1) / nt);
        return ConvChoice::split(nt, (nt <= 2 && tiles_wide >= 512) ? 1 : 0);
    }
    const long px = (long)B * hout * wout;
    if (px >= 131072 || (ks == 1 && px >= 32768)) return ConvChoice::dma();
    const int ntiles = (cout + 15) / 16;
    ConvChoice best = ConvChoice::wave((need & 2) ? 2 : 1, 1, 8);
    long best_reuse = -1, best_waves = -1;
    const int mhs[3] = {4, 2, 1}, wks[3] = {2, 4, 8};
    for (int mh : mhs)
        for (int nt = 2; nt >= 1; --nt) {
            if ((need & 2) && mh == 1) continue;
            if (nt > ntiles) continue;
            for (int wk : wks) {
                if (wave_lds_bytes(ks, mh, nt, wk) > 64 * 1024) continue;
                const long waves = (long)B * ((hout + mh - 1) / mh) * ((wout + 15) / 16) * ((ntiles + nt - 1) / nt) * wk;
                const long reuse = waves >= 2048 ? mh * nt : 0;
                if (reuse > best_reuse || (reuse == best_reuse && reuse == 0 && waves > best_waves)) {
                    best = ConvChoice::wave(mh, nt, wk);
                    best_reuse = reuse;
                    best_waves = waves;
                }
            }
        }
    return best;
}

S4Shape s4_resolve(int ks, int nt, int tile, int ntiles, int rounds, bool kacc) {
    nt = nt < 1 ? 1 : (nt > ntiles ? ntiles : nt);
    if (ks != 3) return {nt > 4 ? 4 : nt, 32, 8, 1};
    if (kacc) return {nt > 3 ? 3 : nt, 32, 8, 1};
    const int nt2 = nt == 1 ? 1 : 2;
    if (tile == S4_16x32) return {nt2, 32, 16, 1};
    if (tile == S4_8x32_K4 && rounds >= 16) return {nt2, 32, 8, 4};
    if (tile >= S4_8x32_K2 && rounds >= 8) return {nt2, 32, 8, 2};
    if (tile >= S4_8x32_K2 || tile == S4_8x32) return {nt > 4 ? 4 : nt, 32, 8, 1};
    if (nt <= 2) return {nt, 64, 8, 1};
    return {3, 32, 8, 1};
}

ConvChoice conv_force() { return g_conv_force; }

ConvDecision decide_conv(const ConvQuery &q) {
    const ConvChoice &f = q.force;
    const bool forced_s4 = f.is(CONV_S4), split_ok = q.has_split && (!q.need || q.ks == 1);
    ConvDecision d{{CONV_AUTO, 0, 0, 0}, false, 0, 0, {}};
    ConvChoice &ch = d.ch;
    if (!q.generic) {
        ch = choose_conv(q.ks, q.stride, q.cin, q.cout, q.hout, q.wout, q.B, q.need, q.use_tuned);
        if (f.is(CONV_WAVE) && q.stride == 1) ch = ConvChoice::wave((q.need & 2) && f.wave_mh() == 1 ? 2 : f.wave_mh(), f.wave_nt(), f.wave_wk());
        if (f.is(CONV_DMA) || (f.is(CONV_SPLIT) && split_ok)) ch = f;
        if (forced_s4 || (ch.is(CONV_SPLIT) && !(split_ok && q.split_f16))) ch = ConvChoice::dma();
    }
    const bool split = ch.is(CONV_SPLIT);
    bool want = split || (q.ks == 1 && (long)q.B * q.hout * q.wout >= 32768 && ch.is(CONV_DMA)) || forced_s4;
    d.s4_nt = forced_s4 ? f.s4_nt() : (q.ks == 1 ? 4 : (split ? ch.split_nt() : 2));
    d.s4_tile = forced_s4 ? f.s4_tile() : (split ? ch.split_wide() : S4_8x32);
    ConvChoice row;
    if (!forced_s4 && !q.generic && q.use_tuned && choose_s4(q.ks, q.cin, q.cout, q.hout, q.wout, q.B, &row)) {
        want = row.is(CONV_S4);
        if (want) { d.s4_nt = row.s4_nt(); d.s4_tile = row.s4_tile(); }
    }
    d.wants_s4 = want && (forced_s4 || f.is(CONV_AUTO)) && !q.generic && q.stride == 1 && q.has_s4 && (q.need == 0 || q.ks == 1);
    d.s4 = s4_resolve(q.ks, d.s4_nt, d.s4_tile, (q.cout + 15) / 16, q.rounds, q.kacc);
    return d;
}

}

static long long *g_probe_dev = nullptr;
namespace pf {
long long *probe_buffer() {
    if (!g_probe_dev) {
        if (hipMalloc((void **)&g_probe_dev, 64 * sizeof(long long)) != hipSuccess) return nullptr;
        (void)hipMemset(g_probe_dev, 0, 64 * sizeof(long long));
        (void)hipMemset(g_probe_dev + 60, 0xFF, sizeof(long long));
    }
    return g_probe_dev;
}
}

extern "C" int pf_debug_probe_read(long long *host64) {
    if (!g_probe_dev) return PF_EINVAL;
    if (hipMemcpy(host64, g_probe_dev, 64 * sizeof(long long), hipMemcpyDeviceToHost) != hipSuccess) return PF_EHIP;
    (void)hipMemset(g_probe_dev, 0, 64 * sizeof(long long));
    (void)hipMemset(g_probe_dev + 60, 0xFF, sizeof(long long));
    return PF_OK;
}

extern "C" int pf_debug_force_conv(int kind, int p0, int p1, int p2) {
    pf::g_conv_force = pf::ConvChoice{kind, p0, p1, p2};
    return PF_OK;
}

extern "C" int pf_debug_conv_decision(int ks, int stride, int cin, int cout, int hout, int wout, int B, int need, int flags, int rounds,
                                      int *out, int cap) {
    if (!out || cap < 11) return pf::fail(PF_EINVAL, "pf_debug_conv_decision: 11 ints of output");
    const pf::ConvDecision d = pf::decide_conv({ks, stride, cin, cout, hout, wout, B, need, (flags & 1) != 0, (flags & 2) != 0, (flags & 4) != 0,
                                                (flags & 8) != 0, (flags & 16) != 0, (flags & 32) != 0, rounds, pf::conv_force()});
    const int v[11] = {d.ch.kind, d.ch.p0, d.ch.p1, d.ch.p2, d.wants_s4, d.s4_nt, d.s4_tile, d.s4.NT, d.s4.TW, d.s4.TH, d.s4.KS};
    for (int i = 0; i < 11; ++i) out[i] = v[i];
    return PF_OK;
}
```

panoptic-forecasting_amd/csrc/hardnet_plan.h:

```cpp
#pragma once
#include <vector>

#include "conv_epilogue.h"
#include "conv_ranges.h"
#include "net_kernels.h"
#include "pf_net.h"

struct ConvPlan {
    pf::ConvTiling tiling;
    size_t wpk_off = 0;
    size_t bias_off = 0;
    size_t raw_off = 0;
    size_t dep_off = 0;
    size_t oh_off = 0;
    size_t tiled_off = 0;
    int tiled_chunks = 0;
    size_t rem_off = 0;
    int rem_count = 0;
    size_t wave_off = 0;
    int wave_chunks = 0;
    size_t split_off = 0;
    int split_chunks = 0;
    size_t s4_off = 0;
    int s4_rounds = 0;
    bool s4_pad = false;
    size_t front_off = 0;
    float split_acc_scale = 1.0f;
    size_t pair_c_off = 0, pair_two_off = 0, pair_nine_off = 0;
    int pair_rounds = 0;
    bool pair_merged = false;
    size_t share_a_off = 0, share_b_off = 0;
    int share_a_tiles = 0, share_b_rounds = 0;
};

struct PlanOptions {
    int fuse_pool = 1, fuse_upsample = 1, valu_remainder = 1, split_f16 = 1, use_tuned_table = 1;
    int table_batch = 0;
    int fuse_front = 1;
    int range_guard = 1;
    int packed_acts = 1;
    int normalize_ranges = 1;
    int profile_tag_ops = 0;
    int fuse_pairs = 1;
    int share_s = 1;
};

struct pf_plan {
    pf::NetTable net;
    std::vector<ConvPlan> conv;
    std::vector<int> readers;
    float *dev_weights = nullptr;
    uint8_t *dev_lut = nullptr;
    size_t dev_floats = 0;
    PlanOptions opt;
    mutable std::vector<uint8_t> last_fmt;
    std::vector<std::vector<float>> chan_scale;
    std::vector<size_t> inv_scale_off;
    std::vector<uint8_t> feeds_conv;
};

namespace pf {

extern PlanOptions g_plan_opt;

constexpr size_t kStatusBytes = PF_WS_STATUS_BYTES;
constexpr int kStickyWord = PF_WS_STICKY_OFFSET / 4, kLiveWord = 2, kSlot0 = 16, kMaxSlots = ((int)(kStatusBytes / 4) - kSlot0) / 2;

int layout(const pf_plan *p, int B, int H, int W, std::vector<Dims> &d, std::vector<size_t> &off, size_t &total, size_t *share_off = nullptr);

bool is_conv_pair(const NetTable &t, size_t i);

}
```

panoptic-forecasting_amd/csrc/hardnet_plan.hip:

```cpp
#include <cstdlib>
#include <cstring>

#include "hardnet_plan.h"
#include "pf_prof.h"

using namespace pf;

namespace {

enum StepKind : uint8_t {
    S_RANGE_CHECK, S_STEM, S_STEM_FRONT, S_PAIR, S_CONV, S_CONV_S4, S_CONV_S4_SHARE, S_CONV_S4_ADD, S_CONV_GENERIC, S_CONV_SPLIT, S_CONV_SPLIT1, S_CONV_WAVE, S_CONV_DMA,
    S_POOL, S_UPSAMPLE, S_HEAD };
struct PlainArgs { const float *src; float *dst; int planes, hin, win, hout, wout; size_t n; unsigned *status, *slot; };
struct Step {
    StepKind kind;
    int op;
    char tag[96];
    int ci, need, sb, se;
    uint32_t src_t[kConvMaxSrc], dst_t;
    bool can_read, can_write, can_write_s4;
    ConvDecision dec;
    union {
        ConvArgs c; PairArgs pair; PlainArgs x;
        struct { StemArgs stem; FrontArgs front; char front_tag[96]; } sf;
        struct { HeadArgs h; float *orig; size_t orig_bytes; } head;
    } u;
};
inline bool is_conv_step(StepKind k) { return k >= S_CONV_S4 && k <= S_CONV_DMA; }

int build_schedule(const pf_plan *p, const StemArgs *stem, const float *dense_x, int B, int H, int W, int out_h, int out_w,
                   void *out_seg, int out_seg_is_i64, float *out_logits, float *out_orig, void *ws, size_t ws_bytes,
                   std::vector<Step> &steps, std::vector<uint8_t> &fmt) {
    std::vector<Dims> d;
    std::vector<size_t> off;
    size_t ws_need = 0;
    size_t share_off = (size_t)-1;
    int rc = layout(p, B, H, W, d, off, ws_need, &share_off);
    if (rc) return rc;
    if (ws_bytes < ws_need) return fail(PF_EWORKSPACE, "workspace %zu B < required %zu B", ws_bytes, ws_need);
    const uint32_t input = p->net.ops[0].src[0].tensor;
    auto tptr = [&](uint32_t t) -> float * {
        return t == input ? const_cast<float *>(dense_x) : reinterpret_cast<float *>((char *)ws + off[t]);
    };
    auto tref = [&](uint32_t t) { return TensorRef{tptr(t), (int)p->net.tensors[t].channels}; };

    const bool tags = (p->opt.profile_tag_ops != 0 || g_plan_opt.profile_tag_ops != 0) && prof_enabled();
    const bool fuse = p->opt.fuse_pool != 0;
    const int Bt = p->opt.table_batch > 0 ? p->opt.table_batch : B;
    unsigned *const st_words = reinterpret_cast<unsigned *>(ws);
    unsigned *const status_all = (p->opt.split_f16 && p->opt.range_guard) ? st_words + kLiveWord : nullptr;
    auto status_of = [&](uint32_t dst_t) -> unsigned * { return p->feeds_conv[dst_t] ? status_all : nullptr; };
    auto slot_of = [&](size_t op_i, uint32_t dst_t) -> unsigned * {
        return (status_all && p->feeds_conv[dst_t]) ? st_words + kSlot0 + op_i : nullptr;
    };

    const size_t nT = p->net.tensors.size();
    fmt.assign(nT, 0);
    std::vector<uint8_t> cand(nT, 1);
    std::vector<std::vector<uint8_t>> written(nT);
    for (size_t t = 0; t < nT; ++t) written[t].assign(p->net.tensors[t].channels + 8, 0);
    const bool s4_allowed = p->opt.packed_acts && p->opt.split_f16 && force_allows_s4();
    auto claim = [&](uint32_t t, int lo, int hi) -> int {
        std::vector<uint8_t> &wr = written[t];
        if ((lo & 3) == 2 && !wr[lo - 2]) cand[t] = 0;
        const int limit = ((hi & 3) != 0 && !wr[hi]) ? (hi + 3) / 4 * 4 : hi;
        for (int c = lo; c < hi; ++c) wr[c] = 1;
        return limit;
    };
    auto pin_fp32 = [&](const BlobOp &op) {
        for (uint32_t j = 0; j < op.n_src; ++j) cand[op.src[j].tensor] = 0;
        cand[op.dst] = 0;
    };

    steps.clear();
    steps.reserve(2 * p->net.ops.size());
    auto push = [&](StepKind kind, size_t i) -> Step & {
        Step &st = steps.emplace_back();
        memset(&st, 0, sizeof(st));
        st.kind = kind; st.op = (int)i;
        const BlobOp &o = p->net.ops[i];
        const Dims out = o.kind == OP_HEAD ? d[o.src[0].tensor] : d[o.dst];
        if (tags) snprintf(st.tag, sizeof(st.tag), "%02zu %s %u->%u %dx%d", i, p->net.tensors[o.dst].name, o.cin, o.cout, out.h, out.w);
        return st;
    };
    auto conv_step = [&](size_t i, size_t ci, const KOrder &ko, const Dims &in, const Dims &out) -> Step & {
        Step &st = push(S_CONV, i);
        const BlobOp &o = p->net.ops[ci];
        ConvArgs &a = st.u.c;
        st.ci = (int)ci; st.dst_t = o.dst;
        set_sources(a, ko, tref);
        for (int j = 0; j < ko.n; ++j) st.src_t[j] = ko.r[j].tensor;
        a.bias = p->dev_weights + p->conv[ci].bias_off;
        a.dst = tptr(o.dst);
        a.dst_ctotal = (int)p->net.tensors[o.dst].channels; a.dst_choff = (int)o.dst_choff;
        a.Cin = (int)o.cin; a.Cout = (int)o.cout;
        a.Hin = in.h; a.Win = in.w; a.Hout = out.h; a.Wout = out.w;
        a.relu = (int)o.relu;
        a.zero_page = p->dev_weights;
        a.ntiles = ((int)o.cout + 15) / 16;
        a.acc_scale = 1.0f;
        a.status = status_of(o.dst); a.range_slot = slot_of(ci, o.dst);
        return st;
    };
    auto choose = [&](Step &st, int need) {
        const BlobOp &o = p->net.ops[st.ci];
        const ConvPlan &cp = p->conv[st.ci];
        const ConvArgs &a = st.u.c;
        const bool generic = (a.Win & 3) != 0;
        st.dec = decide_conv({(int)o.k, (int)o.stride, a.Cin, a.Cout, a.Hout, a.Wout, Bt, need, generic, cp.split_off != 0, cp.s4_off != 0,
                              p->opt.use_tuned_table != 0, p->opt.split_f16 != 0, false, cp.s4_rounds, conv_force()});
        st.need = need; st.sb = a.src_begin; st.se = a.src_end;
        const bool res_fits = !a.res || (size_t)st.dec.s4.NT * 16 * res_chan_stride(res_extent(8, a.res_sh), res_extent(32, a.res_sw)) * sizeof(float) <= 60 * 1024;
        st.can_read = s4_allowed && o.kind == OP_CONV && st.dec.wants_s4 && res_fits && ((a.src_begin == 0 && a.src_end == a.n_src) || cp.s4_pad);
        st.can_write_s4 = s4_allowed && !generic && (a.dst_choff & 1) == 0;
        st.can_write = st.can_write_s4 && (st.dec.ch.is(CONV_DMA) || st.dec.ch.is(CONV_SPLIT));
        st.u.c.dst_limit = claim(st.dst_t, a.dst_choff, a.dst_choff + a.Cout);
    };
    const bool fuse_up = p->opt.fuse_upsample != 0;
    auto can_commute_upsample = [&](size_t i, const Dims &in, const Dims &out) -> bool {
        if (!fuse || !fuse_up || i + 1 >= p->net.ops.size()) return false;
        const BlobOp &o = p->net.ops[i], &n = p->net.ops[i + 1];
        return n.kind == OP_CONV && n.k == 1 && n.stride == 1 && n.n_src == 2 && n.src[0].tensor == o.dst &&
               n.src[0].choff == 0 && n.src[0].ch == p->net.tensors[o.dst].channels && p->readers[o.dst] == 1 &&
               (in.w & 3) == 0 && (out.w & 3) == 0 && n.cout <= p->net.tensors[o.dst].channels &&
               2 * in.h <= out.h + 1 && 2 * in.w <= out.w + 1;
    };

    cand[input] = 0;
    for (size_t i = 0; i < p->net.ops.size(); ++i) {
        const BlobOp &o = p->net.ops[i];
        const Dims in = d[o.src[0].tensor];
        const Dims out = o.kind == OP_HEAD ? in : d[o.dst];
        if (o.kind == OP_STEM && stem) {
            StemArgs a = *stem;
            a.w = p->dev_weights + p->conv[i].raw_off; a.wdep = p->dev_weights + p->conv[i].dep_off;
            a.woh = p->conv[i].oh_off ? p->dev_weights + p->conv[i].oh_off : nullptr; a.bias = p->dev_weights + p->conv[i].bias_off;
            a.status = status_of(o.dst); a.range_slot = slot_of(i, o.dst);
            a.lut = p->dev_lut; a.dst = tptr(o.dst); a.Hout = out.h; a.Wout = out.w;
            bool front = false;
            if (s4_allowed && p->opt.fuse_front && i + 2 < p->net.ops.size()) {
                const BlobOp &n1 = p->net.ops[i + 1], &n2 = p->net.ops[i + 2];
                front = n1.kind == OP_CONV && n1.k == 3 && n1.stride == 1 && n1.n_src == 1 && n1.src[0].tensor == o.dst && n1.src[0].choff == 0 &&
                        n1.src[0].ch == p->net.tensors[o.dst].channels && n1.dst_choff == 0 && n1.cout == p->net.tensors[n1.dst].channels &&
                        p->readers[o.dst] == 1 && p->readers[n1.dst] == 1 && n1.relu && p->conv[i + 1].s4_off && p->conv[i + 1].s4_rounds == 2 &&
                        n2.kind == OP_CONV && n2.k == 3 && n2.stride == 2 && n2.n_src == 1 && n2.src[0].tensor == n1.dst && n2.src[0].choff == 0 &&
                        n2.src[0].ch == n1.cout && p->conv[i + 2].front_off && (n2.dst_choff & 3) == 0 &&
                        conv_front_supports((int)o.cout, (int)n1.cout, (int)n2.cout, out.h, out.w, (int)p->net.tensors[n2.dst].channels) && stem_writes_s4(a) && !conv_forced();
            }
            if (!front) {
                if (o.cout != 16 || o.k != 3 || o.stride != 2 || o.dst_choff != 0 ||
                    p->net.tensors[o.dst].channels != 16 || (uint32_t)(a.T * (a.n_cls + 1)) != o.cin)
                    return fail(PF_EUNSUPPORTED, "fused stem expects a 3x3/s2 conv %d->16, got %u->%u k%u s%u",
                                a.T * (a.n_cls + 1), o.cin, o.cout, o.k, o.stride);
                push(S_STEM, i).u.sf.stem = a;
                pin_fp32(o);
                continue;
            }
            const BlobOp &n1 = p->net.ops[i + 1], &n2 = p->net.ops[i + 2];
            const Dims o2 = d[n2.dst];
            cand[o.dst] = 0; cand[n1.dst] = 0;
            Step &st = push(S_STEM_FRONT, i);
            st.u.sf.stem = a; st.u.sf.stem.dst_fmt = 1;
            FrontArgs &f = st.u.sf.front;
            f.x = tptr(o.dst);
            f.w1 = p->dev_weights + p->conv[i + 1].s4_off; f.w2 = p->dev_weights + p->conv[i + 2].front_off;
            f.bias1 = p->dev_weights + p->conv[i + 1].bias_off; f.bias2 = p->dev_weights + p->conv[i + 2].bias_off;
            f.scale1 = p->conv[i + 1].split_acc_scale; f.scale2 = p->conv[i + 2].split_acc_scale;
            f.dst = tptr(n2.dst);
            f.dst_ctotal = (int)p->net.tensors[n2.dst].channels; f.dst_c4 = (f.dst_ctotal + 3) / 4; f.dst_choff = (int)n2.dst_choff;
            f.dst_limit = claim(n2.dst, f.dst_choff, f.dst_choff + (int)n2.cout);
            f.H1 = out.h; f.W1 = out.w; f.H2 = o2.h; f.W2 = o2.w;
            f.C1 = (int)n1.cout; f.C2 = (int)n2.cout; f.relu1 = (int)n1.relu; f.relu2 = (int)n2.relu;
            f.status = status_all;
            f.range_slot_mid = slot_of(i + 1, n1.dst); f.range_slot = slot_of(i + 2, n2.dst);
            st.dst_t = n2.dst; st.can_write = st.can_write_s4 = true;
            if (tags)
                snprintf(st.u.sf.front_tag, sizeof(st.u.sf.front_tag), "%02zu+%02zu %s+%s %u->%u->%u %dx%d", i + 1, i + 2, p->net.tensors[n1.dst].name,
                         p->net.tensors[n2.dst].name, o.cout, n1.cout, n2.cout, o2.h, o2.w);
            i += 2;
        } else if (o.kind == OP_STEM || o.kind == OP_CONV) {
            if (o.src[0].tensor == input && !dense_x)
                return fail(PF_EINVAL, "network input is consumed by a generic conv: use pf_hardnet_forward_dense");
            if (o.src[0].tensor == input && status_all) {
                PlainArgs &x = push(S_RANGE_CHECK, i).u.x;
                x.src = dense_x; x.n = (size_t)B * p->net.tensors[input].channels * in.h * in.w;
                x.status = status_all; x.slot = st_words + kSlot0 + kMaxSlots - 1;
            }
            const BlobOp *pool = nullptr;
            if (fuse && i + 1 < p->net.ops.size() && p->net.ops[i + 1].kind == OP_POOL && o.stride == 1 && o.k == 1 && (in.w & 3) == 0 &&
                p->net.ops[i + 1].src[0].tensor == o.dst && o.dst_choff == 0 && o.cout == p->net.tensors[o.dst].channels &&
                p->readers[o.dst] == 1 && out.h >= 2 && out.w >= 2)
                pool = &p->net.ops[i + 1];
            Step &st = conv_step(i, i, order_plain(o.src, (int)o.n_src), in, out);
            if (pool) {
                ConvArgs &a = st.u.c;
                a.pool = 1; a.dst = tptr(pool->dst); a.dst_ctotal = (int)p->net.tensors[pool->dst].channels;
                st.dst_t = pool->dst;
                a.status = status_of(pool->dst); a.range_slot = slot_of(i, pool->dst);
                ++i;
            }
            choose(st, pool ? 2 : 0);
        } else if (o.kind == OP_UPSAMPLE && can_commute_upsample(i, in, out)) {
            const BlobOp &n = p->net.ops[i + 1];
            const Dims hi = out;
            cand[o.dst] = 0;
            auto tag_half = [&](Step &st, const char *half, int cin, const Dims &dd) {
                if (tags)
                    snprintf(st.tag, sizeof(st.tag), "%02zu%c %s.%s %d->%u %dx%d", i + 1, half[0] == 'l' ? 'a' : 'b', p->net.tensors[n.dst].name,
                             half, cin, n.cout, dd.h, dd.w);
            };
            const KOrder kn = order_plain(n.src, (int)n.n_src);
            KOrder kx = kn;
            kx.r[0].tensor = o.src[0].tensor; kx.r[0].choff = (int)o.src[0].choff;
            Step &ls = conv_step(i, i + 1, kx, in, in);
            ConvArgs &lo = ls.u.c;
            lo.dst = tptr(o.dst);
            ls.dst_t = o.dst;
            lo.dst_ctotal = (int)n.cout; lo.dst_choff = 0;
            lo.relu = 0; lo.no_bias = 1;
            lo.status = nullptr; lo.range_slot = nullptr;
            lo.Cin = (int)n.src[0].ch;
            lo.src_end = 1;
            tag_half(ls, "lo", lo.Cin, in);
            choose(ls, 4);
            Step &hs = conv_step(i, i + 1, kn, hi, hi);
            ConvArgs &ha = hs.u.c;
            ha.Cin = (int)n.src[1].ch;
            ha.src_begin = 1; ha.src_end = 2;
            tag_half(hs, "hi", ha.Cin, hi);
            ha.res = tptr(o.dst); ha.res_ctotal = (int)n.cout;
            ha.Hres = in.h; ha.Wres = in.w;
            ha.res_sh = hi.h > 1 ? (float)(in.h - 1) / (float)(hi.h - 1) : 0.f;
            ha.res_sw = hi.w > 1 ? (float)(in.w - 1) / (float)(hi.w - 1) : 0.f;
            choose(hs, 4);
            ++i;
        } else if (o.kind == OP_HEAD) {
            pin_fp32(o);
            Step &st = push(S_HEAD, i);
            HeadArgs &a = st.u.head.h;
            a.logits = tptr(o.src[0].tensor);
            a.out_seg = out_seg; a.out_logits = out_logits; a.out_is_i64 = out_seg_is_i64;
            a.B = B; a.C = (int)o.cin; a.Hin = in.h; a.Win = in.w; a.Hout = out_h; a.Wout = out_w;
            st.u.head.orig = out_orig; st.u.head.orig_bytes = (size_t)B * a.C * in.h * in.w * sizeof(float);
        } else {
            pin_fp32(o);
            PlainArgs &x = push(o.kind == OP_POOL ? S_POOL : S_UPSAMPLE, i).u.x;
            x.src = tptr(o.src[0].tensor); x.dst = tptr(o.dst); x.planes = B * (int)o.cin;
            x.hin = in.h; x.win = in.w; x.hout = out.h; x.wout = out.w;
            x.status = status_of(o.dst); x.slot = slot_of(i, o.dst);
        }
    }

    if (!s4_allowed) std::fill(cand.begin(), cand.end(), 0);
    for (bool changed = true; changed;) {
        changed = false;
        for (const Step &r : steps) {
            if (r.kind != S_CONV && r.kind != S_STEM_FRONT) continue;
            bool all = r.can_read;
            for (int j = r.sb; j < r.se; ++j) all = all && cand[r.src_t[j]];
            if (!all)
                for (int j = r.sb; j < r.se; ++j)
                    if (cand[r.src_t[j]]) { cand[r.src_t[j]] = 0; changed = true; }
            if (!(r.can_write || (all && r.can_write_s4)) && cand[r.dst_t]) { cand[r.dst_t] = 0; changed = true; }
        }
    }
    std::vector<uint8_t> read_s4(nT, 0);
    for (const Step &r : steps)
        if (r.kind == S_CONV)
            for (int j = r.sb; j < r.se; ++j) read_s4[r.src_t[j]] = 1;
    for (size_t t = 0; t < nT; ++t) fmt[t] = cand[t] && read_s4[t];

    for (Step &st : steps) {
        if (st.kind == S_STEM_FRONT) {
            st.u.sf.front.dst_fmt = fmt[st.dst_t];
            fmt[p->net.ops[st.op].dst] = 1;
            fmt[p->net.ops[st.op + 1].dst] = 0xFF;
        }
        if (st.kind != S_CONV) continue;
        const BlobOp &o = p->net.ops[st.ci];
        const ConvPlan &cp = p->conv[st.ci];
        ConvArgs &a = st.u.c;
        a.dst_fmt = fmt[st.dst_t]; a.dst_c4 = (a.dst_ctotal + 3) / 4;
        bool s4 = st.can_read;
        for (int j = st.sb; j < st.se; ++j) s4 = s4 && fmt[st.src_t[j]];
        if (s4) {
            a.src_fmt = 1; a.acc_scale = cp.split_acc_scale;
            a.wpk = p->dev_weights + cp.s4_off; a.nchunks = cp.s4_rounds;
            set_s4_entries(a, (int)o.k, cp.s4_pad);
            st.kind = S_CONV_S4; continue;
        }
        if ((a.Win & 3) != 0) {
            if (st.need) return fail(PF_EUNSUPPORTED, "fused conv on a width that is not a multiple of 4");
            a.wpk = p->dev_weights + cp.wpk_off; a.nchunks = cp.tiling.nchunks;
            st.kind = S_CONV_GENERIC; continue;
        }
        auto use = [&](size_t wpk_off, int nchunks, int kc) {
            a.wpk = p->dev_weights + wpk_off;
            a.nchunks = nchunks;
            set_chunks(a, kc);
        };
        ConvChoice &ch = st.dec.ch;
        if (ch.is(CONV_SPLIT)) {
            use(cp.split_off, cp.split_chunks, o.k == 1 ? 32 : 8);
            a.acc_scale = cp.split_acc_scale;
            st.kind = o.k == 1 ? S_CONV_SPLIT1 : S_CONV_SPLIT;
            if (o.k == 1 ? conv_split1_supported(a, ch.split_nt()) : conv_split_supported(a)) continue;
            ch = ConvChoice::dma();
        }
        if (ch.is(CONV_WAVE)) {
            use(cp.wave_off, cp.wave_chunks, wave_kc((int)o.k));
            ch = ConvChoice::wave(ch.wave_mh(), ch.wave_nt() < a.ntiles ? ch.wave_nt() : a.ntiles, ch.wave_wk());
            st.kind = S_CONV_WAVE;
            if (conv_wave_supported(a, (int)o.k, ch.wave_mh(), ch.wave_nt(), ch.wave_wk())) continue;
            ch = ConvChoice::dma();
        }
        use(cp.tiled_off, cp.tiled_chunks, dma_kc((int)o.k, (int)o.stride));
        st.kind = S_CONV_DMA;
        int wm, nt;
        if (p->opt.valu_remainder && cp.rem_off && !st.need && !a.dst_fmt && a.src_begin == 0 && a.src_end == a.n_src && (ch.dma_wm() == 0 || ch.dma_wm() == 4)) {
            ConvArgs r = a;
            r.rem = cp.rem_count;
            r.wrem = p->dev_weights + cp.rem_off;
            r.ntiles = ((int)o.cout - r.rem) / 16;
            if (conv_dma_supported(r, (int)o.k, (int)o.stride, B, 4, ch.dma_wm() == 4 && ch.dma_nt() > 0 ? ch.dma_nt() : 0, p->opt.table_batch, &wm, &nt)) {
                a = r;
                ch = ConvChoice::dma(wm, nt);
                continue;
            }
        }
        conv_dma_supported(a, (int)o.k, (int)o.stride, B, ch.dma_wm(), ch.dma_nt(), p->opt.table_batch, &wm, &nt);
        ch = ConvChoice::dma(wm, nt);
    }

    size_t w = 0;
    for (size_t k = 0; k < steps.size(); ++k, ++w) {
        const size_t i = (size_t)steps[k].op;
        const bool adjacent = k + 1 < steps.size() && steps[k].kind == S_CONV_S4 && steps[k + 1].kind == S_CONV_S4 && steps[k + 1].op == (int)i + 1 &&
                              is_conv_pair(p->net, i) && steps[k].u.c.dst_fmt && steps[k + 1].u.c.dst_fmt;
        const bool pair = p->opt.fuse_pairs && adjacent && p->conv[i + 1].pair_c_off;
        const BlobOp &o = p->net.ops[i];
        if (!pair || !pair_wanted((int)o.cin, (int)o.cout, (int)p->net.ops[i + 1].cin, (int)p->net.ops[i + 1].cout, d[o.dst].h, d[o.dst].w, Bt,
                                  p->opt.fuse_pairs)) {
            if (adjacent && p->opt.share_s && p->conv[i + 1].share_a_off && share_off != (size_t)-1 && steps[k].dec.s4_tile == S4_8x32 && steps[k + 1].dec.s4_tile == S4_8x32 &&
                share_wanted((int)o.cin, (int)o.cout, (int)p->net.ops[i + 1].cin, (int)p->net.ops[i + 1].cout, d[o.dst].h, d[o.dst].w, Bt, p->opt.share_s)) {
                const ConvPlan &cc = p->conv[i + 1];
                Step sa = steps[k], sb = steps[k + 1];
                float *const sums = reinterpret_cast<float *>((char *)ws + share_off);
                ConvArgs &a = sa.u.c, &c = sb.u.c;
                sa.kind = S_CONV_S4_SHARE;
                a.wpk = p->dev_weights + cc.share_a_off; a.ntiles = cc.share_a_tiles;
                a.share = sums; a.share_off = share_row0((int)o.cout); a.share_cout = c.Cout; a.share_scale = cc.split_acc_scale;
                sa.dec.s4_nt = cc.share_a_tiles <= 3 ? cc.share_a_tiles : 2;
                sb.kind = S_CONV_S4_ADD;
                set_sources(c, order_add(p->net.ops[i + 1].src, (int)p->net.ops[i + 1].n_src), tref);
                c.Cin = c.src_cstart[c.n_src];
                c.wpk = p->dev_weights + cc.share_b_off; c.nchunks = cc.share_b_rounds;
                set_s4_entries(c, 3, 0);
                c.share = sums; c.share_cout = c.Cout;
                steps[w] = sa;
                steps[++w] = sb;
                ++k;
                continue;
            }
            if (w != k) steps[w] = steps[k];
            continue;
        }
        const BlobOp &C = p->net.ops[i + 1];
        Step st = steps[k + 1];
        st.kind = S_PAIR; st.op = (int)i;
        if (tags)
            snprintf(st.tag, sizeof(st.tag), "%02zu+%02zu %s+%s %u->%u->%u %dx%d", i, i + 1, p->net.tensors[o.dst].name, p->net.tensors[C.dst].name, o.cin,
                     o.cout, C.cout, d[o.dst].h, d[o.dst].w);
        PairArgs &pa = st.u.pair;
        ConvArgs &a = pa.c;
        const int n = (int)C.n_src;
        set_sources(a, order_pair(C.src, n), tref);
        a.wpk = p->dev_weights + p->conv[i + 1].pair_c_off; a.nchunks = p->conv[i + 1].pair_rounds;
        set_s4_entries(a, 3, 1);
        pa.p_wpk = p->dev_weights + p->conv[i + 1].pair_two_off; pa.p_w9 = p->dev_weights + p->conv[i + 1].pair_nine_off;
        pa.p_bias = p->dev_weights + p->conv[i].bias_off; pa.p_acc_scale = p->conv[i].split_acc_scale;
        pa.p_dst = tptr(o.dst); pa.p_dst_c4 = ((int)p->net.tensors[o.dst].channels + 3) / 4;
        pa.p_dst_choff = (int)o.dst_choff; pa.p_dst_limit = steps[k].u.c.dst_limit;
        pa.p_cout = (int)o.cout; pa.p_cin = (int)o.cin; pa.p_ntiles = ((int)o.cout + 15) / 16; pa.p_relu = (int)o.relu;
        pa.p_range_slot = slot_of(i, o.dst);
        pa.rounds_s = a.src_ent0[1] / 2; pa.round_d = a.src_ent0[n - 1] / 2;
        pa.merged = p->conv[i + 1].pair_merged && p->opt.fuse_pairs != 3;
        steps[w] = st;
        ++k;
    }
    steps.resize(w);
    return PF_OK;
}

int run_net(const pf_plan *p, const StemArgs *stem, const float *dense_x, int B, int H, int W, int out_h, int out_w,
            void *out_seg, int out_seg_is_i64, float *out_logits, float *out_orig, void *ws, size_t ws_bytes,
            hipStream_t s) {
    std::vector<Step> steps;
    std::vector<uint8_t> fmt;
    int rc = build_schedule(p, stem, dense_x, B, H, W, out_h, out_w, out_seg, out_seg_is_i64, out_logits, out_orig, ws, ws_bytes, steps, fmt);
    if (rc) return rc;
    p->last_fmt = fmt;
    static const bool sync_ops = ab_env("PF_SYNC_OPS") != nullptr;
    static const bool probe_on = ab_env("PF_PROBE") != nullptr;
    long long *const probe = probe_on ? probe_buffer() : nullptr;
    for (size_t k = 0; k < steps.size(); ++k) {
        Step &st = steps[k];
        if (sync_ops && (k == 0 || steps[k - 1].op != st.op))
            fprintf(stderr, "[pf] before op %d (%s): %s\n", st.op, p->net.tensors[p->net.ops[st.op].dst].name, hipGetErrorString(hipStreamSynchronize(s)));
        else if (sync_ops && is_conv_step(steps[k - 1].kind) && steps[k - 1].u.c.no_bias)
            fprintf(stderr, "[pf]   low-resolution half: %s\n", hipGetErrorString(hipStreamSynchronize(s)));
        if (st.tag[0]) prof_set_tag(st.tag);
        const BlobOp &o = p->net.ops[st.ci];
        ConvArgs &a = st.u.c;
        const ConvChoice &ch = st.dec.ch;
        const PlainArgs &x = st.u.x;
        if (is_conv_step(st.kind)) a.probe = probe;
        switch (st.kind) {
            case S_RANGE_CHECK: rc = launch_range_check(x.src, x.n, x.status, x.slot, s); break;
            case S_STEM: st.u.sf.stem.probe = probe; rc = launch_stem(st.u.sf.stem, s); break;
            case S_STEM_FRONT:
                if ((rc = launch_stem(st.u.sf.stem, s))) break;
                if (st.u.sf.front_tag[0]) prof_set_tag(st.u.sf.front_tag);
                st.u.sf.front.probe = probe; rc = launch_conv_front(st.u.sf.front, B, s); break;
            case S_PAIR: st.u.pair.c.probe = probe; rc = launch_conv_pair(st.u.pair, B, s); break;
            case S_CONV_S4: rc = launch_conv_s4(a, (int)o.k, st.dec.s4, B, s); break;
            case S_CONV_S4_SHARE: rc = launch_conv_s4_share(a, st.dec.s4_nt, B, s); break;
            case S_CONV_S4_ADD: rc = launch_conv_s4_add(a, st.dec.s4_nt, B, s); break;
            case S_CONV_GENERIC: rc = launch_conv(a, p->conv[st.ci].tiling, B, s); break;
            case S_CONV_SPLIT: rc = launch_conv_split(a, ch.split_nt(), ch.split_wide(), B, s); break;
            case S_CONV_SPLIT1: rc = launch_conv_split1(a, ch.split_nt(), B, s); break;
            case S_CONV_WAVE: rc = launch_conv_wave(a, (int)o.k, ch.wave_mh(), ch.wave_nt(), ch.wave_wk(), B, s); break;
            case S_CONV_DMA: rc = launch_conv_dma(a, (int)o.k, (int)o.stride, B, s, ch.dma_wm(), ch.dma_nt(), p->opt.table_batch); break;
            case S_POOL: rc = launch_avgpool2(x.src, x.dst, x.planes, x.hin, x.win, x.status, x.slot, s); break;
            case S_UPSAMPLE: rc = launch_upsample(x.src, x.dst, x.planes, x.hin, x.win, x.hout, x.wout, x.status, x.slot, s); break;
            case S_HEAD:
                if (st.u.head.orig && (rc = launch_copy(st.u.head.orig, st.u.head.h.logits, st.u.head.orig_bytes, s))) break;
                rc = launch_head(st.u.head.h, s); break;
            case S_CONV: break;
        }
        if (rc) return rc;
    }
    if (p->opt.profile_tag_ops != 0 || g_plan_opt.profile_tag_ops != 0) prof_set_tag(nullptr);
    return launch_range_finalize(reinterpret_cast<unsigned *>(ws), kLiveWord, kSlot0, kMaxSlots, kStickyWord, s);
}

}

extern "C" int pf_bg_forward(const pf_plan *p, const void *seg, int seg_is_i64, const float *depth,
                             const uint8_t *depth_mask, float depth_mean, float depth_std, int hop_flags,
                             float min_depth, float max_depth, int B, int T, int H, int W, int out_h, int out_w,
                             void *out_seg, int out_seg_is_i64, float *out_logits, float *out_orig_logits, void *ws,
                             size_t ws_bytes, void *stream) {
    if (!p || !seg || !depth || !out_seg || !ws) return fail(PF_EINVAL, "pf_bg_forward: null pointer argument");
    if (!depth_mask && !(hop_flags & PF_HOP_DEPTH_U16))
        return fail(PF_EINVAL, "pf_bg_forward: depth_mask is required unless PF_HOP_DEPTH_U16 is set");
    if (B <= 0 || T <= 0 || H <= 0 || W <= 0 || out_h <= 0 || out_w <= 0)
        return fail(PF_EINVAL, "pf_bg_forward: bad dims");
    if (p->net.ops.empty() || p->net.ops[0].kind != OP_STEM)
        return fail(PF_EUNSUPPORTED, "pf_bg_forward: plan does not start with a fused stem");
    StemArgs st;
    memset(&st, 0, sizeof(st));
    st.seg = seg; st.depth = depth; st.mask = depth_mask;
    st.depth_mean = depth_mean; st.depth_std = depth_std; st.min_depth = min_depth; st.max_depth = max_depth;
    st.seg_is_i64 = seg_is_i64; st.hop = hop_flags; st.B = B; st.T = T; st.n_cls = (int)p->net.hdr.n_cls;
    st.H = H; st.W = W;
    return run_net(p, &st, nullptr, B, H, W, out_h, out_w, out_seg, out_seg_is_i64, out_logits, out_orig_logits, ws,
                   ws_bytes, (hipStream_t)stream);
}

extern "C" int pf_hardnet_forward_dense(const pf_plan *p, const float *x, int B, int H, int W, int out_h, int out_w,
                                        void *out_seg, int out_seg_is_i64, float *out_logits, float *out_orig_logits,
                                        void *ws, size_t ws_bytes, void *stream) {
    if (!p || !x || !ws) return fail(PF_EINVAL, "pf_hardnet_forward_dense: null pointer argument");
    if (B <= 0 || H <= 0 || W <= 0) return fail(PF_EINVAL, "pf_hardnet_forward_dense: bad dims");
    const bool has_head = !p->net.ops.empty() && p->net.ops.back().kind == OP_HEAD;
    if (has_head && (!out_seg || out_h <= 0 || out_w <= 0))
        return fail(PF_EINVAL, "pf_hardnet_forward_dense: out_seg/out size required");
    return run_net(p, nullptr, x, B, H, W, out_h, out_w, out_seg, out_seg_is_i64, out_logits, out_orig_logits, ws,
                   ws_bytes, (hipStream_t)stream);
}
```

panoptic-forecasting_amd/csrc/plan_create.hip:

```cpp
#include <algorithm>
#include <cmath>
#include <cstring>

#include "hardnet_plan.h"

using namespace pf;

namespace pf {
PlanOptions g_plan_opt;
extern int g_opt_train_side, g_opt_wgrad_taps, g_opt_train_s4, g_opt_train_kacc, g_opt_train_table_batch, g_opt_up_two_pass;
}

namespace {

struct Option {
    const char *name, *alias;
    int PlanOptions::*member;
    int *global;
    bool process, per_plan, clamp0;
};
const Option kOptions[] = {
    {"fuse_pool", nullptr, &PlanOptions::fuse_pool, nullptr, true, true, false},
    {"fuse_upsample", nullptr, &PlanOptions::fuse_upsample, nullptr, true, true, false},
    {"use_tuned_table", nullptr, &PlanOptions::use_tuned_table, nullptr, true, true, false},
    {"valu_remainder", nullptr, &PlanOptions::valu_remainder, nullptr, true, true, false},
    {"split_f16", "split_bf16", &PlanOptions::split_f16, nullptr, true, true, false},
    {"packed_acts", nullptr, &PlanOptions::packed_acts, nullptr, true, true, false},
    {"range_guard", nullptr, &PlanOptions::range_guard, nullptr, true, true, false},
    {"fuse_front", nullptr, &PlanOptions::fuse_front, nullptr, true, true, false},
    {"fuse_pairs", nullptr, &PlanOptions::fuse_pairs, nullptr, true, true, false},
    {"share_s", nullptr, &PlanOptions::share_s, nullptr, true, true, false},
    {"profile_tag_ops", nullptr, &PlanOptions::profile_tag_ops, nullptr, true, true, false},
    {"table_batch", nullptr, &PlanOptions::table_batch, nullptr, false, true, true},
    {"normalize_ranges", nullptr, &PlanOptions::normalize_ranges, nullptr, true, false, false},
    {"train_side_stream", nullptr, nullptr, &g_opt_train_side, true, false, false},
    {"wgrad_taps", nullptr, nullptr, &g_opt_wgrad_taps, true, false, false},
    {"train_forward_s4", nullptr, nullptr, &g_opt_train_s4, true, false, false},
    {"train_blocked_sum", nullptr, nullptr, &g_opt_train_kacc, true, false, false},
    {"train_table_batch", nullptr, nullptr, &g_opt_train_table_batch, true, false, true},
    {"upsample_bwd_two_pass", nullptr, nullptr, &g_opt_up_two_pass, true, false, false},
};

int set_option(const char *who, PlanOptions *plan, const char *name, int value) {
    for (const Option &o : kOptions) {
        if (strcmp(name, o.name) != 0 && !(o.alias && !strcmp(name, o.alias))) continue;
        if (!(plan ? o.per_plan : o.process)) break;
        if (o.clamp0 && value < 0) value = 0;
        *(o.member ? &((plan ? *plan : g_plan_opt).*o.member) : o.global) = value;
        return PF_OK;
    }
    return fail(PF_EINVAL, "%s: unknown option '%s'", who, name);
}

}

extern "C" int pf_set_option(const char *name, int value) {
    if (!name) return fail(PF_EINVAL, "pf_set_option: null name");
    return set_option("pf_set_option", nullptr, name, value);
}

extern "C" int pf_hardnet_plan_set_option(pf_plan *p, const char *name, int value) {
    if (!p || !name) return fail(PF_EINVAL, "pf_hardnet_plan_set_option: null argument");
    return set_option("pf_hardnet_plan_set_option", &p->opt, name, value);
}

bool pf::is_conv_pair(const NetTable &t, size_t i) {
    if (i + 1 >= t.ops.size()) return false;
    const BlobOp &P = t.ops[i], &C = t.ops[i + 1];
    if (P.kind != OP_CONV || C.kind != OP_CONV || P.k != 3 || C.k != 3 || P.stride != 1 || C.stride != 1) return false;
    if (P.n_src != 1 || C.n_src < 2 || (P.dst_choff & 1) || (C.dst_choff & 1)) return false;
    if (C.src[0].tensor != P.dst || C.src[0].choff != P.dst_choff || C.src[0].ch != P.cout) return false;
    if (C.src[1].tensor != P.src[0].tensor || C.src[1].choff != P.src[0].choff || C.src[1].ch != P.src[0].ch) return false;
    for (uint32_t j = 0; j < C.n_src; ++j)
        if (C.src[j].choff & 1) return false;
    return conv_pair_supports((int)C.cout, (int)P.cout);
}

static void fill_lut(uint8_t *lut) {
    memset(lut, 0, 256);
    for (int i = 0; i < 34; ++i) lut[i] = 255;
    const int ids[19] = {7, 8, 11, 12, 13, 17, 19, 20, 21, 22, 23, 24, 25, 26, 27, 28, 31, 32, 33};
    for (int t = 0; t < 19; ++t) lut[ids[t]] = (uint8_t)t;
}

static void normalize_ranges(pf_plan *p, std::vector<float> &w) {
    const size_t nT = p->net.tensors.size();
    p->chan_scale.assign(nT, std::vector<float>());
    std::vector<std::vector<double>> est(nT);
    for (size_t t = 0; t < nT; ++t) {
        p->chan_scale[t].assign(p->net.tensors[t].channels, 1.0f);
        est[t].assign(p->net.tensors[t].channels, 1.0);
    }
    p->feeds_conv.assign(nT, 0);
    for (size_t i = p->net.ops.size(); i-- > 0;) {
        const BlobOp &o = p->net.ops[i];
        if (o.kind == OP_STEM || o.kind == OP_CONV)
            for (uint32_t j = 0; j < o.n_src; ++j) p->feeds_conv[o.src[j].tensor] = 1;
        else if ((o.kind == OP_POOL || o.kind == OP_UPSAMPLE) && p->feeds_conv[o.dst])
            p->feeds_conv[o.src[0].tensor] = 1;
    }
    std::vector<uint8_t> pinned(nT, 0), read(nT, 0);
    for (const BlobOp &o : p->net.ops) {
        for (uint32_t j = 0; j < (o.kind == OP_UPSAMPLE ? 1u : o.n_src); ++j) read[o.src[j].tensor] = 1;
        if (o.kind == OP_HEAD) pinned[o.src[0].tensor] = 1;
    }
    for (size_t t = 0; t < nT; ++t) pinned[t] = pinned[t] || !read[t] || !p->feeds_conv[t];
    if (p->net.ops.empty()) return;
    const uint32_t input = p->net.ops[0].src[0].tensor;
    pinned[input] = 1;
    if (p->net.ops[0].kind == OP_STEM && p->net.hdr.n_cls > 0) {
        const uint32_t C = p->net.tensors[input].channels, T = C / (p->net.hdr.n_cls + 1);
        if (T * (p->net.hdr.n_cls + 1) == C)
            for (uint32_t c = 0; c < T * p->net.hdr.n_cls; ++c) est[input][c] = std::sqrt(1.0 / p->net.hdr.n_cls);
    }
    for (size_t i = p->net.ops.size(); i-- > 0;) {
        const BlobOp &o = p->net.ops[i];
        if ((o.kind == OP_POOL || o.kind == OP_UPSAMPLE) && pinned[o.dst]) pinned[o.src[0].tensor] = 1;
    }
    for (const BlobOp &o : p->net.ops) {
        if (o.kind == OP_POOL || o.kind == OP_UPSAMPLE) {
            for (uint32_t c = 0; c < o.src[0].ch; ++c) {
                p->chan_scale[o.dst][o.dst_choff + c] = p->chan_scale[o.src[0].tensor][o.src[0].choff + c];
                est[o.dst][o.dst_choff + c] = est[o.src[0].tensor][o.src[0].choff + c];
            }
            continue;
        }
        if (o.kind != OP_STEM && o.kind != OP_CONV) continue;
        const size_t kk = (size_t)o.k * o.k;
        std::vector<double> e_in(o.cin);
        std::vector<float> s_in(o.cin);
        uint32_t k0 = 0;
        for (uint32_t j = 0; j < o.n_src; ++j)
            for (uint32_t c = 0; c < o.src[j].ch; ++c, ++k0) {
                e_in[k0] = est[o.src[j].tensor][o.src[j].choff + c];
                s_in[k0] = p->chan_scale[o.src[j].tensor][o.src[j].choff + c];
            }
        for (uint32_t co = 0; co < o.cout; ++co) {
            float *wr = w.data() + o.w_off + (size_t)co * o.cin * kk;
            float &b = w[o.b_off + co];
            double var = (double)b * b;
            for (uint32_t k = 0; k < o.cin; ++k) {
                double ss = 0;
                for (size_t q = 0; q < kk; ++q) ss += (double)wr[k * kk + q] * wr[k * kk + q];
                var += ss * e_in[k] * e_in[k];
            }
            double e = std::sqrt(var);
            if (o.relu) e *= 0.70710678118654752;
            float s_out = 1.0f;
            if (p->opt.normalize_ranges && !pinned[o.dst] && e > 0 && std::isfinite(e)) {
                int ex = (int)std::lround(std::log2((double)kRangeTarget / e));
                ex = ex < -60 ? -60 : (ex > 60 ? 60 : ex);
                s_out = std::ldexp(1.0f, ex);
            }
            for (uint32_t k = 0; k < o.cin; ++k) {
                const float f = s_out / s_in[k];
                if (f != 1.0f)
                    for (size_t q = 0; q < kk; ++q) wr[k * kk + q] *= f;
            }
            b *= s_out;
            p->chan_scale[o.dst][o.dst_choff + co] = s_out;
            est[o.dst][o.dst_choff + co] = e;
        }
    }
}

namespace {

struct Arena {
    std::vector<float> &f;
    size_t take(size_t n_floats, size_t align = 1) {
        f.resize(align_up(f.size(), align), 0.f);
        f.resize(f.size() + n_floats);
        return f.size() - n_floats;
    }
    float *at(size_t off) { return f.data() + off; }
};

void pack_generic(const BlobOp &o, const float *w, const float *bias, Arena &a, ConvPlan &c) {
    c.tiling = choose_tiling((int)o.k, (int)o.stride, (int)o.cin, (int)o.cout, 0);
    c.wpk_off = a.take(c.tiling.packed_floats());
    pack_conv_weights(w, (int)o.cin, (int)o.cout, c.tiling, a.at(c.wpk_off));
    c.bias_off = a.take((size_t)c.tiling.cout_blocks * c.tiling.nt * 16);
    memcpy(a.at(c.bias_off), bias, o.cout * sizeof(float));
}

void pack_dma(const BlobOp &o, const float *w, const int *src_ch, Arena &a, ConvPlan &c) {
    const int kc = dma_kc((int)o.k, (int)o.stride);
    c.tiled_chunks = range_chunks(src_ch, (int)o.n_src, kc);
    c.tiled_off = a.take((size_t)((o.cout + 15) / 16) * c.tiled_chunks * (kc / 4) * o.k * o.k * 64);
    pack_conv_weights_tiled(w, (int)o.cin, (int)o.cout, (int)o.k, kc, src_ch, (int)o.n_src, a.at(c.tiled_off));
    constexpr int valu_max = 8;
    const int split = (o.k == 3 && o.stride == 1) ? dma_valu_split((int)o.cout) : 0;
    if (split > 0 && split <= valu_max) {
        c.rem_count = split;
        c.rem_off = a.take((size_t)c.tiled_chunks * (kc / 4) * 9 * dma_rem_rv(split) * 4, 4);
        pack_conv_weights_rem(w, (int)o.cin, (int)o.cout, split, 3, kc, src_ch, (int)o.n_src, a.at(c.rem_off));
    }
}

float scale_weights(const float *w, size_t n, std::vector<float> &ws) {
    const float sc = split_weight_scale(w, n);
    ws.resize(n);
    for (size_t q = 0; q < n; ++q) ws[q] = w[q] * sc;
    return sc;
}

void pack_split(const BlobOp &o, const float *ws, const int *src_ch, Arena &a, ConvPlan &c) {
    if (o.k == 3) {
        c.split_chunks = range_chunks(src_ch, (int)o.n_src, 8);
        c.split_off = a.take(split_packed_floats(src_ch, (int)o.n_src, (int)o.cout), 16);
        pack_conv_weights_split(ws, (int)o.cin, (int)o.cout, src_ch, (int)o.n_src, a.at(c.split_off));
    } else {
        c.split_chunks = range_chunks(src_ch, (int)o.n_src, 32);
        c.split_off = a.take(split1_packed_floats(src_ch, (int)o.n_src, (int)o.cout), 16);
        pack_conv_weights_split1(ws, (int)o.cin, (int)o.cout, src_ch, (int)o.n_src, a.at(c.split_off));
    }
}

void pack_s4(const BlobOp &o, const float *ws, Arena &a, ConvPlan &c) {
    for (uint32_t j = 0; j < o.n_src; ++j)
        if (o.src[j].choff & 1) return;
    const KOrder ko = order_plain(o.src, (int)o.n_src);
    c.s4_pad = o.k == 1 && o.n_src == 2;
    c.s4_rounds = s4_rounds(ko, (int)o.k, c.s4_pad);
    c.s4_off = a.take(s4_packed_floats(ko, (int)o.cout, (int)o.k, c.s4_pad), 16);
    pack_conv_weights_s4(ws, (int)o.cin, (int)o.cout, (int)o.k, ko, c.s4_pad, a.at(c.s4_off));
}

void pack_pair(const BlobOp &P, const float *wP, const BlobOp &o, const float *ws, Arena &a, ConvPlan &c) {
    const KOrder ko = order_pair(o.src, (int)o.n_src);
    c.pair_rounds = s4_rounds(ko, 3, 1);
    c.pair_c_off = a.take(s4_packed_floats(ko, (int)o.cout, 3, 1), 16);
    std::vector<float> wp;
    scale_weights(wP, (size_t)P.cout * P.cin * 9, wp);
    c.pair_merged = conv_pair_merged_supports((int)o.cout, (int)P.cout);
    if (c.pair_merged) {
        const int nt = ((int)o.cout + 15) / 16, row0 = ((int)o.cout + 3) / 4 * 4, cS = ko.r[0].cstart;
        std::vector<float> waug((size_t)nt * 16 * o.cin * 9, 0.f);
        std::copy(ws, ws + (size_t)o.cout * o.cin * 9, waug.begin());
        for (int pc = 0; pc < (int)P.cout; ++pc)
            for (int ci = 0; ci < (int)P.cin; ++ci)
                for (int t = 0; t < 9; ++t) waug[((size_t)(row0 + pc) * o.cin + cS + ci) * 9 + t] = wp[((size_t)pc * P.cin + ci) * 9 + t];
        pack_conv_weights_s4(waug.data(), (int)o.cin, nt * 16, 3, ko, 1, a.at(c.pair_c_off));
    } else {
        pack_conv_weights_s4(ws, (int)o.cin, (int)o.cout, 3, ko, 1, a.at(c.pair_c_off));
    }
    const S4Range rs{(int)P.src[0].choff, (int)P.src[0].ch};
    c.pair_two_off = a.take(pair_p_two_floats(rs, (int)P.cout), 16);
    c.pair_nine_off = a.take(pair_p_nine_floats(rs, (int)P.cout), 16);
    pack_conv_weights_pair_p(wp.data(), (int)P.cin, (int)P.cout, rs, a.at(c.pair_two_off), a.at(c.pair_nine_off));
}

void pack_share(const BlobOp &P, const float *wP, const BlobOp &o, const float *ws, Arena &a, ConvPlan &c) {
    const int row0 = share_row0((int)P.cout), rows = row0 + (int)o.cout, cS = (int)o.src[0].ch;
    std::vector<float> wp, wa((size_t)rows * P.cin * 9, 0.f);
    scale_weights(wP, (size_t)P.cout * P.cin * 9, wp);
    std::copy(wp.begin(), wp.end(), wa.begin());
    for (int co = 0; co < (int)o.cout; ++co)
        for (int ci = 0; ci < (int)P.cin; ++ci)
            for (int t = 0; t < 9; ++t) wa[((size_t)(row0 + co) * P.cin + ci) * 9 + t] = ws[((size_t)co * o.cin + cS + ci) * 9 + t];
    const KOrder ko_s = order_plain(P.src, 1), ko_b = order_add(o.src, (int)o.n_src);
    c.share_a_tiles = (rows + 15) / 16;
    c.share_a_off = a.take(s4_packed_floats(ko_s, rows, 3, 0), 16);
    pack_conv_weights_s4(wa.data(), (int)P.cin, rows, 3, ko_s, 0, a.at(c.share_a_off));
    c.share_b_rounds = s4_rounds(ko_b, 3, 0);
    c.share_b_off = a.take(s4_packed_floats(ko_b, (int)o.cout, 3, 0), 16);
    pack_conv_weights_s4(ws, (int)o.cin, (int)o.cout, 3, ko_b, 0, a.at(c.share_b_off));
}

void pack_front(const BlobOp &o, const float *ws, Arena &a, ConvPlan &c) {
    const KOrder ko = order_plain(o.src, 1);
    c.front_off = a.take(s4_packed_floats(ko, (int)o.cout, 3, 0), 16);
    pack_conv_weights_s4(ws, (int)o.cin, (int)o.cout, 3, ko, 0, a.at(c.front_off));
}

void pack_wave(const BlobOp &o, const float *w, const int *src_ch, Arena &a, ConvPlan &c) {
    c.wave_chunks = range_chunks(src_ch, (int)o.n_src, wave_kc((int)o.k));
    c.wave_off = a.take(wave_packed_floats(src_ch, (int)o.n_src, (int)o.cout, (int)o.k));
    pack_conv_weights_wave(w, (int)o.cin, (int)o.cout, (int)o.k, src_ch, (int)o.n_src, a.at(c.wave_off));
}

void pack_stem(const BlobOp &o, const float *w, int n_cls, Arena &a, ConvPlan &c) {
    const int ks2 = (int)(o.k * o.k);
    c.raw_off = a.take((size_t)o.cout * o.cin * ks2);
    memcpy(a.at(c.raw_off), w, (size_t)o.cout * o.cin * ks2 * sizeof(float));
    const int T = (int)o.cin / (n_cls + 1);
    if (T < 1 || (uint32_t)(T * (n_cls + 1)) != o.cin || o.cout != 16) return;
    c.dep_off = a.take((size_t)ks2 * T * 16, 16);
    float *q = a.at(c.dep_off);
    for (int tap = 0; tap < ks2; ++tap)
        for (int t = 0; t < T; ++t)
            for (int co = 0; co < 16; ++co) *q++ = w[((size_t)co * o.cin + T * n_cls + t) * ks2 + tap];
    c.oh_off = a.take((size_t)ks2 * T * (n_cls + 1) * 16, 16);
    q = a.at(c.oh_off);
    for (int tap = 0; tap < ks2; ++tap)
        for (int t = 0; t < T; ++t)
            for (int r = 0; r <= n_cls; ++r)
                for (int co = 0; co < 16; ++co) *q++ = r < n_cls ? w[((size_t)co * o.cin + t * n_cls + r) * ks2 + tap] : 0.f;
}

int build_plan_weights(pf_plan &p, const float *wts, std::vector<float> &host) {
    host.assign(64, 0.f);
    Arena a{host};
    const std::vector<BlobOp> &ops = p.net.ops;
    p.conv.assign(ops.size(), ConvPlan());
    for (size_t i = 0; i < ops.size(); ++i) {
        const BlobOp &o = ops[i];
        if (o.kind != OP_STEM && o.kind != OP_CONV) continue;
        if (o.k == 1 && o.stride != 1) return fail(PF_EUNSUPPORTED, "1x1 conv with stride %u", o.stride);
        ConvPlan &c = p.conv[i];
        const float *w = wts + o.w_off, *ws = w;
        int src_ch[kConvMaxSrc];
        for (uint32_t j = 0; j < o.n_src; ++j) src_ch[j] = (int)o.src[j].ch;
        pack_generic(o, w, wts + o.b_off, a, c);
        pack_dma(o, w, src_ch, a, c);
        std::vector<float> wsc;
        if (o.stride == 1 || o.n_src == 1) {
            c.split_acc_scale = 1.0f / scale_weights(w, (size_t)o.cout * o.cin * o.k * o.k, wsc);
            ws = wsc.data();
        }
        if (o.stride == 1) pack_split(o, ws, src_ch, a, c);
        if (o.stride == 1 && o.kind == OP_CONV) pack_s4(o, ws, a, c);
        if (i > 0 && is_conv_pair(p.net, i - 1)) pack_pair(ops[i - 1], wts + ops[i - 1].w_off, o, ws, a, c);
        if (i > 0 && p.opt.share_s && is_conv_pair(p.net, i - 1)) pack_share(ops[i - 1], wts + ops[i - 1].w_off, o, ws, a, c);
        if (o.k == 3 && o.stride == 2 && o.kind == OP_CONV && o.n_src == 1 && (o.src[0].choff & 3) == 0 && o.cout <= 32) pack_front(o, ws, a, c);
        if (o.stride == 1) pack_wave(o, w, src_ch, a, c);
        if (o.kind == OP_STEM) pack_stem(o, w, (int)p.net.hdr.n_cls, a, c);
        a.take(0, 64);
    }
    p.inv_scale_off.assign(p.net.tensors.size(), 0);
    for (size_t t = 0; t < p.net.tensors.size(); ++t) {
        bool any = false;
        for (float v : p.chan_scale[t]) any = any || v != 1.0f;
        if (!any) continue;
        p.inv_scale_off[t] = a.take(p.chan_scale[t].size());
        for (size_t ch = 0; ch < p.chan_scale[t].size(); ++ch) host[p.inv_scale_off[t] + ch] = 1.0f / p.chan_scale[t][ch];
        a.take(0, 64);
    }
    return PF_OK;
}

int check_plan_ops(const NetTable &t, size_t n_w) {
    for (size_t i = 0; i < t.ops.size(); ++i) {
        const BlobOp &o = t.ops[i];
        uint32_t cin = 0;
        for (uint32_t j = 0; j < o.n_src; ++j) cin += o.src[j].ch;
        bool ok = true;
        if (o.kind == OP_STEM || o.kind == OP_CONV)
            ok = cin == o.cin && o.dst_choff + o.cout <= t.tensors[o.dst].channels && (o.k == 1 || o.k == 3) &&
                 (o.stride == 1 || o.stride == 2) && o.w_off + (uint64_t)o.cout * o.cin * o.k * o.k <= n_w && o.b_off + o.cout <= n_w;
        if (o.kind == OP_POOL || o.kind == OP_UPSAMPLE) ok = o.src[0].ch <= t.tensors[o.dst].channels;
        if (!ok) return fail(PF_EBLOB, "op %zu is inconsistent with the tensor table", i);
    }
    return PF_OK;
}

}

extern "C" int pf_hardnet_plan_create(const void *blob, size_t bytes, int in_ch, int n_cls, pf_plan **out) {
    if (!blob || !out) return fail(PF_EINVAL, "pf_hardnet_plan_create: null argument");
    pf_plan *p = new pf_plan();
    p->opt = g_plan_opt;
    int rc = parse_net_table(blob, bytes, in_ch, n_cls, p->net);
    if ((int)p->net.ops.size() >= kMaxSlots - 1)
        rc = fail(PF_EUNSUPPORTED, "op table of %zu ops: the status block has %d per-op words", p->net.ops.size(), kMaxSlots - 1);
    const size_t n_w = rc ? 0 : (bytes - p->net.hdr.weights_off) / sizeof(float);
    if (!rc) rc = check_plan_ops(p->net, n_w);
    std::vector<float> wnorm, host;
    if (!rc) {
        const float *w0 = reinterpret_cast<const float *>((const char *)blob + p->net.hdr.weights_off);
        wnorm.assign(w0, w0 + n_w);
        normalize_ranges(p, wnorm);
        rc = build_plan_weights(*p, wnorm.data(), host);
    }
    if (rc) {
        delete p;
        return rc;
    }
    p->readers.assign(p->net.tensors.size(), 0);
    for (const BlobOp &o : p->net.ops)
        for (uint32_t j = 0; j < o.n_src; ++j) p->readers[o.src[j].tensor]++;
    p->dev_floats = host.size();
    uint8_t lut[256];
    fill_lut(lut);
    hipError_t e = hipMalloc((void **)&p->dev_weights, (host.size() + 64) * sizeof(float));
    if (e == hipSuccess) e = hipMalloc((void **)&p->dev_lut, 256);
    if (e == hipSuccess) e = hipMemcpy(p->dev_weights, host.data(), host.size() * sizeof(float), hipMemcpyHostToDevice);
    if (e == hipSuccess) e = hipMemcpy(p->dev_lut, lut, 256, hipMemcpyHostToDevice);
    if (e != hipSuccess) {
        pf_hardnet_plan_destroy(p);
        return fail(PF_EHIP, "plan upload: %s", hipGetErrorString(e));
    }
    *out = p;
    return PF_OK;
}

extern "C" int pf_debug_plan_arena(const void *blob, size_t bytes, int in_ch, int n_cls, float *out, size_t cap, size_t *n_floats,
                                   long long *table, int table_ops) {
    if (!blob || !n_floats) return fail(PF_EINVAL, "pf_debug_plan_arena: null argument");
    pf_plan p;
    p.opt = g_plan_opt;
    int rc = parse_net_table(blob, bytes, in_ch, n_cls, p.net);
    const size_t n_w = rc ? 0 : (bytes - p.net.hdr.weights_off) / sizeof(float);
    if (!rc) rc = check_plan_ops(p.net, n_w);
    if (rc) return rc;
    const float *w0 = reinterpret_cast<const float *>((const char *)blob + p.net.hdr.weights_off);
    std::vector<float> wnorm(w0, w0 + n_w), host;
    normalize_ranges(&p, wnorm);
    if ((rc = build_plan_weights(p, wnorm.data(), host))) return rc;
    *n_floats = host.size();
    if (out && cap >= host.size()) memcpy(out, host.data(), host.size() * sizeof(float));
    for (int i = 0; table && i < table_ops && i < (int)p.conv.size(); ++i) {
        const ConvPlan &c = p.conv[i];
        const long long row[6] = {(long long)c.s4_off, c.s4_rounds, (long long)c.share_a_off, c.share_a_tiles, (long long)c.share_b_off, c.share_b_rounds};
        memcpy(table + 6 * i, row, sizeof(row));
    }
    return PF_OK;
}

extern "C" void pf_hardnet_plan_destroy(pf_plan *p) {
    if (!p) return;
    if (p->dev_weights) (void)hipFree(p->dev_weights);
    if (p->dev_lut) (void)hipFree(p->dev_lut);
    delete p;
}
```

panoptic-forecasting_amd/lib.py:

```python
import ctypes
import os

_HERE = os.path.dirname(os.path.abspath(__file__))
LIB_PATH = os.environ.get('PF_LIBPFHIP') or os.path.join(_HERE, 'csrc', 'libpfhip.so')

_c = ctypes
_vp, _i, _f, _sz = _c.c_void_p, _c.c_int, _c.c_float, _c.c_size_t

SIGNATURES = {
    'pf_version': (_i, []),
    'pf_last_error': (_c.c_char_p, []),
    'pf_warp_splat_workspace': (_i, [_i, _i, _i, _i, _i, _c.POINTER(_sz)]),
    'pf_warp_splat': (_i, [_vp, _vp, _vp, _i, _vp, _vp, _vp, _vp, _vp, _i, _i, _i, _i, _i, _i, _i,
                           _vp, _vp, _vp, _vp, _sz, _vp]),
    'pf_hardnet_plan_create': (_i, [_vp, _sz, _i, _i, _c.POINTER(_vp)]),
    'pf_hardnet_plan_destroy': (None, [_vp]),
    'pf_hardnet_workspace': (_i, [_vp, _i, _i, _i, _c.POINTER(_sz)]),
    'pf_bg_forward': (_i, [_vp, _vp, _i, _vp, _vp, _f, _f, _i, _f, _f, _i, _i, _i, _i, _i, _i,
                           _vp, _i, _vp, _vp, _vp, _sz, _vp]),
    'pf_hardnet_forward_dense': (_i, [_vp, _vp, _i, _i, _i, _i, _i, _vp, _i, _vp, _vp, _vp, _sz, _vp]),
    'pf_hardnet_tensor_view': (_i, [_vp, _c.c_char_p, _i, _i, _i, _c.POINTER(_sz), _c.POINTER(_i),
                                    _c.POINTER(_i), _c.POINTER(_i)]),
    'pf_hardnet_tensor_read': (_i, [_vp, _c.c_char_p, _i, _i, _i, _vp, _vp, _vp]),
    'pf_hardnet_status': (_i, [_vp, _c.POINTER(_c.c_uint), _vp]),
    'pf_hardnet_status_sticky': (_i, [_vp, _c.POINTER(_c.c_uint), _i, _vp]),
    'pf_hardnet_status_reset': (_i, [_vp, _vp]),
    'pf_hardnet_range_maxima': (_i, [_vp, _vp, _vp, _i, _c.POINTER(_i), _vp]),
    'pf_s4_pack': (_i, [_vp, _vp, _i, _i, _i, _i, _vp, _vp]),
    'pf_s4_unpack': (_i, [_vp, _vp, _i, _i, _i, _i, _vp]),
    'pf_hardnet_flops': (_i, [_vp, _i, _i, _c.POINTER(_c.c_double)]),
    'pf_hop_export': (_i, [_vp, _i, _i, _vp, _sz, _vp, _vp, _vp]),
    'pf_hop_load': (_i, [_vp, _sz, _f, _f, _vp, _vp, _vp]),
    'pf_bg_augment': (_i, [_vp, _vp, _vp, _i, _i, _i, _i, _vp, _vp, _vp, _vp, _i, _i, _i, _f, _f, _vp, _vp, _vp, _vp, _vp]),
    'pf_fg_assemble': (_i, [_vp, _vp, _vp, _vp, _vp, _vp, _i, _i, _i, _i, _i, _c.c_double, _c.c_double, _i,
                            _vp, _vp, _vp, _vp, _vp, _vp, _vp, _vp, _vp, _vp, _vp]),
    'pf_panoptic_merge_workspace': (_i, [_i, _c.POINTER(_sz)]),
    'pf_panoptic_merge': (_i, [_vp, _i, _vp, _vp, _vp, _i, _i, _vp, _i, _vp, _vp, _vp, _i, _i, _i, _i, _i, _i, _i,
                               _vp, _i, _vp, _sz, _vp]),
    'pf_panoptic_encode': (_i, [_vp, _i, _i, _i, _i, _i, _vp, _vp, _vp, _vp]),
    'pf_panoptic_max_ids': (_i, []),
    'pf_pq_workspace': (_i, [_i, _c.POINTER(_sz)]),
    'pf_pq_table_slots': (_i, []),
    'pf_pq_accumulate': (_i, [_vp, _i, _vp, _i, _i, _i, _i, _i, _i, _i, _vp, _vp, _vp, _sz, _vp]),
    'pf_pq_status': (_i, [_vp, _vp, _c.POINTER(_i)]),
    'pf_pq_status_reset': (_i, [_vp, _vp]),
    'pf_bg_dense_input': (_i, [_vp, _i, _i, _vp, _vp, _f, _f, _i, _i, _i, _i, _vp, _vp]),
    'pf_seg_loss_workspace': (_i, [_i, _i, _i, _c.POINTER(_sz)]),
    'pf_seg_loss': (_i, [_vp, _i, _i, _i, _i, _vp, _i, _i, _i, _i, _vp, _vp, _sz, _vp]),
    'pf_train_create': (_i, [_vp, _sz, _i, _i, _c.POINTER(_vp)]),
    'pf_train_destroy': (None, [_vp]),
    'pf_train_autotune': (_i, [_vp, _i]),
    'pf_train_tuned_shapes': (_i, [_vp, _c.POINTER(_i), _i, _c.POINTER(_i)]),
    'pf_train_path_stats': (_i, [_vp, _c.POINTER(_i), _i, _c.POINTER(_i)]),
    'pf_train_param_count': (_i, [_vp, _c.POINTER(_sz)]),
    'pf_train_param_layout': (_i, [_vp, _i, _c.POINTER(_sz), _c.POINTER(_sz), _c.POINTER(_i)]),
    'pf_train_workspace': (_i, [_vp, _i, _i, _i, _i, _i, _c.POINTER(_sz)]),
    'pf_train_forward_backward': (_i, [_vp, _vp, _vp, _i, _vp, _i, _vp, _vp, _f, _f, _i, _vp, _i, _i, _i, _vp, _i, _i, _i, _i, _f, _f,
                                       _f, _i, _vp, _vp, _sz, _vp]),
    'pf_train_tensor_view': (_i, [_vp, _c.c_char_p, _i, _i, _i, _i, _i, _i, _c.POINTER(_sz), _c.POINTER(_i), _c.POINTER(_i),
                                  _c.POINTER(_i)]),
    'pf_sgd_workspace': (_i, [_c.POINTER(_sz)]),
    'pf_sgd_step': (_i, [_vp, _vp, _vp, _vp, _sz, _f, _f, _f, _f, _f, _i, _vp, _sz, _vp]),
    'pf_fg_weights_size': (_i, [_i, _c.POINTER(_sz), _c.POINTER(_sz)]),
    'pf_fg_pack': (_i, [_vp, _vp, _i, _vp]),
    'pf_fg_workspace': (_i, [_i, _i, _i, _i, _c.POINTER(_sz)]),
    'pf_fg_forward': (_i, [_vp, _i, _i, _i, _i, _i, _vp, _vp, _vp, _vp, _vp, _vp, _vp, _vp, _vp, _vp, _vp, _vp, _vp, _vp,
                           _vp, _sz, _vp]),
    'pf_odom_weights_size': (_i, [_i, _c.POINTER(_sz), _c.POINTER(_sz)]),
    'pf_odom_pack': (_i, [_vp, _vp, _i, _vp]),
    'pf_odom_forward': (_i, [_vp, _i, _i, _i, _i, _vp, _vp, _vp, _vp]),
    'pf_odom_train_workspace': (_i, [_i, _i, _i, _i, _c.POINTER(_sz)]),
    'pf_odom_train_forward': (_i, [_vp, _i, _i, _i, _i, _vp, _vp, _vp, _vp, _sz, _vp]),
    'pf_odom_backward': (_i, [_vp, _i, _i, _i, _i, _vp, _vp, _vp, _vp, _vp, _sz, _vp, _vp]),
    'pf_set_option': (_i, [_c.c_char_p, _i]),
    'pf_hardnet_plan_set_option': (_i, [_vp, _c.c_char_p, _i]),
    'pf_debug_force_conv': (_i, [_i, _i, _i, _i]),
    'pf_debug_conv_decision': (_i, [_i, _i, _i, _i, _i, _i, _i, _i, _i, _i, _c.POINTER(_i), _i]),
    'pf_debug_probe_read': (_i, [_c.POINTER(_c.c_longlong)]),
    'pf_debug_conv_ranges': (_i, [_i, _i, _i, _i, _i, _i, _vp, _vp, _vp, _i, _i, _vp, _sz]),
    'pf_debug_plan_arena': (_i, [_vp, _sz, _i, _i, _vp, _sz, _c.POINTER(_sz), _vp, _i]),
    'pf_debug_train_plan': (_i, [_vp, _sz, _i, _i, _i, _i, _i, _i, _i, _vp, _i, _c.POINTER(_i), _vp, _i, _c.POINTER(_i), _vp]),
    'pf_profile_enable': (_i, [_i]),
    'pf_profile_collect': (_i, []),
    'pf_profile_get': (_i, [_i, _c.c_char_p, _sz, _c.POINTER(_i), _c.POINTER(_c.c_double),
                            _c.POINTER(_c.c_double), _c.POINTER(_c.c_double)]),
}


def profile(enable):
    check(load().pf_profile_enable(int(enable)), 'pf_profile_enable')


def profile_results():
    L = load()
    n = L.pf_profile_collect()
    if n < 0:
        check(n, 'pf_profile_collect')
    out = []
    for i in range(n):
        buf = ctypes.create_string_buffer(160)
        la, ms, fl, by = _i(), _c.c_double(), _c.c_double(), _c.c_double()
        check(L.pf_profile_get(i, buf, 160, ctypes.byref(la), ctypes.byref(ms), ctypes.byref(fl), ctypes.byref(by)),
              'pf_profile_get')
        out.append({'label': buf.value.decode(), 'launches': la.value, 'ms': ms.value, 'flops': fl.value,
                    'bytes': by.value})
    return out

_lib = None


class PfError(RuntimeError):
    pass


def load():
    global _lib
    if _lib is None:
        import torch
        if not os.path.exists(LIB_PATH):
            raise PfError('%s not found: build it with `python -c "import __graft_entry__ as g; g.build()"` '
                          '(make -C panoptic-forecasting_amd/csrc). There is no fallback path.' % LIB_PATH)
        lib = ctypes.CDLL(LIB_PATH)
        for name, (res, args) in SIGNATURES.items():
            fn = getattr(lib, name)
            fn.restype, fn.argtypes = res, args
        _lib = lib
    return _lib


def check(rc, what):
    if rc != 0:
        raise PfError('%s failed (%d): %s' % (what, rc, load().pf_last_error().decode()))


def require_cuda(t, name):
    if not t.is_cuda:
        raise PfError('%s must live on the GPU (got %s): the HIP path has no CPU fallback' % (name, t.device))
    if not t.is_contiguous():
        raise PfError('%s must be contiguous' % name)
    return t


def stream_ptr():
    import torch
    return ctypes.c_void_p(torch.cuda.current_stream().cuda_stream)
```

Baseline: 2819 frames/s.

## Add K-resident 1x1 split-f16 conv kernel that keeps input in registers across output tiles

```diff
diff --git a/include/pfhip.h b/include/pfhip.h
--- a/include/pfhip.h
+++ b/include/pfhip.h
@@ -158,6 +158,7 @@
 int pf_debug_force_conv(int kind, int p0, int p1, int p2);
 int pf_debug_conv_decision(int ks, int stride, int cin, int cout, int hout, int wout, int B, int need, int flags, int rounds,
                            int *out, int cap);
+int pf_debug_resident_decision(int ks, int cin, int cout, int hout, int wout, int B, int fused, int nt, int rounds, int mode);
 int pf_debug_conv_ranges(int form, int ks, int kc, int pad, int n_src, int n_cases, const int *choff, const int *ch, const int *ctotal,
                          int src_begin, int src_end, int *out, size_t cap);
 int pf_debug_plan_arena(const void *blob, size_t bytes, int in_ch, int n_cls, float *out, size_t cap, size_t *n_floats,
diff --git a/panoptic-forecasting_amd/bg_model.py b/panoptic-forecasting_amd/bg_model.py
--- a/panoptic-forecasting_amd/bg_model.py
+++ b/panoptic-forecasting_amd/bg_model.py
@@ -14,7 +14,8 @@
 
 PLAN_OPTIONS = {'split_f16': 'split_f16', 'split_bf16': 'split_f16', 'fuse_pool': 'fuse_pool', 'fuse_upsample': 'fuse_upsample',
                 'use_tuned_table': 'use_tuned_table', 'valu_remainder': 'valu_remainder', 'conv_table_batch': 'table_batch',
-                'range_guard': 'range_guard', 'fuse_front': 'fuse_front', 'fuse_pairs': 'fuse_pairs', 'share_s': 'share_s'}
+                'range_guard': 'range_guard', 'fuse_front': 'fuse_front', 'fuse_pairs': 'fuse_pairs', 'share_s': 'share_s',
+                'k_resident': 'k_resident'}
 PF_STATUS_RANGE, PF_STATUS_RANGE_LOW = 1, 2
 PF_STATUS_ANY = PF_STATUS_RANGE | PF_STATUS_RANGE_LOW
 PF_WS_STATUS_BYTES = 2048
diff --git a/panoptic-forecasting_amd/csrc/conv_mfma.h b/panoptic-forecasting_amd/csrc/conv_mfma.h
--- a/panoptic-forecasting_amd/csrc/conv_mfma.h
+++ b/panoptic-forecasting_amd/csrc/conv_mfma.h
@@ -183,9 +183,13 @@
 size_t s4_packed_floats(const KOrder &k, int cout, int ks, int pad_sources);
 void pack_conv_weights_s4(const float *w_oihw, int cin, int cout, int ks, const KOrder &k, int pad_sources, float *out);
 enum S4Tile : int { S4_8x32 = 0, S4_8x64 = 1, S4_16x32 = 2, S4_8x32_K2 = 3, S4_8x32_K4 = 4 };
-struct S4Shape { int NT, TW, TH, KS; };
+struct S4Shape { int NT, TW, TH, KS, RES; };
 S4Shape s4_resolve(int ks, int nt, int tile, int ntiles, int rounds, bool kacc);
 int launch_conv_s4(const ConvArgs &a, int ks, const S4Shape &shape, int B, hipStream_t stream);
+constexpr int kS4ResRounds = 4;
+bool resident_wanted(int cin, int cout, int h, int w, int B, int fused, int mode);
+bool resident_exists(int cin, int cout, int nt, int rounds);
+bool conv_s4_1x1_res_supported(const ConvArgs &a, int nt);
 int launch_conv_s4_share(const ConvArgs &a, int nt, int B, hipStream_t stream);
 int launch_conv_s4_add(const ConvArgs &a, int nt, int B, hipStream_t stream);
 inline int share_row0(int p_cout) { return (p_cout + 3) / 4 * 4; }
diff --git a/panoptic-forecasting_amd/csrc/conv_s4.hip b/panoptic-forecasting_amd/csrc/conv_s4.hip
--- a/panoptic-forecasting_amd/csrc/conv_s4.hip
+++ b/panoptic-forecasting_amd/csrc/conv_s4.hip
@@ -300,79 +300,7 @@
         const int Ho = pooled ? a.Hout >> 1 : a.Hout, Wo = pooled ? a.Wout >> 1 : a.Wout;
         const size_t hw = (size_t)Ho * Wo, term = (size_t)a.dst_c4 * hw * 8;
         const bool mis = (a.dst_choff & 2) != 0;
-        typedef split_x2 h2;
-        float vmax = 0.f;
-        const float relu_lo1 = a.relu ? 0.f : -__builtin_inff();
-        auto finish = [&](int rr, int q, int n, const int (&o0)[2], const int (&o1)[2], const float (&lx1)[2], float hy1) {
-            s4_f32x4 v = acc[rr * 2 + q][n];
-            const s4_f32x4 b4 = *reinterpret_cast<const s4_f32x4 *>(bias_lds + n * 16 + 4 * g);
-#pragma unroll
-            for (int r = 0; r < 4; ++r) {
-                v[r] = v[r] * a.acc_scale + b4[r];
-                if (has_res) {
-                    const lds_float *chan = res_lds + (n * 16 + 4 * g + r) * rw.cs;
-                    const float lx0 = 1.f - lx1[q], hy0 = 1.f - hy1;
-                    const float t0 = lx0 * chan[o0[q]] + lx1[q] * chan[o0[q] + 1];
-                    const float t1 = lx0 * chan[o1[q]] + lx1[q] * chan[o1[q] + 1];
-                    v[r] += hy0 * t0 + hy1 * t1;
-                }
-                v[r] = fmaxf(v[r], relu_lo1);
-            }
-            vmax = range_acc(vmax, v[0], v[1], v[2], v[3]);
-            return v;
-        };
-        auto store_px = [&](int co, size_t pix, s4_f32x4 v) {
-            if (a.dst_fmt) {
-                s4_h4 hi, mid;
-                split_terms4(v, hi, mid);
-                const int chb = a.dst_choff + co;
-                const bool ok0 = chb < a.dst_limit, ok1 = chb + 2 < a.dst_limit;
-                char *p = reinterpret_cast<char *>(a.dst) + (size_t)b * 2 * term + pix * 8 + (size_t)(chb >> 2) * hw * 8;
-                if (!mis) {
-                    if (ok1) {
-                        *reinterpret_cast<s4_h4 *>(p) = hi;
-                        *reinterpret_cast<s4_h4 *>(p + term) = mid;
-                    } else if (ok0) {
-                        *reinterpret_cast<h2 *>(p) = h2{hi[0], hi[1]};
-                        *reinterpret_cast<h2 *>(p + term) = h2{mid[0], mid[1]};
-                    }
-                } else {
-                    if (ok0) {
-                        *reinterpret_cast<h2 *>(p + 4) = h2{hi[0], hi[1]};
-                        *reinterpret_cast<h2 *>(p + 4 + term) = h2{mid[0], mid[1]};
-                    }
-                    if (ok1) {
-                        *reinterpret_cast<h2 *>(p + hw * 8) = h2{hi[2], hi[3]};
-                        *reinterpret_cast<h2 *>(p + hw * 8 + term) = h2{mid[2], mid[3]};
-                    }
-                }
-            } else {
-#pragma unroll
-                for (int r = 0; r < 4; ++r)
-                    if (co + r < a.Cout) a.dst[((size_t)b * a.dst_ctotal + a.dst_choff + co + r) * hw + pix] = v[r];
-            }
-        };
-        auto store_pair = [&](int co, size_t pix, s4_f32x4 v0, s4_f32x4 v1) {
-            const int chb = a.dst_choff + co;
-            if (a.dst_fmt && !mis && chb + 2 < a.dst_limit) {
-                s4_h4 h0, m0, h1, m1;
-                split_terms4(v0, h0, m0);
-                split_terms4(v1, h1, m1);
-                const s4_h8 hi = s4_join(h0, h1), mid = s4_join(m0, m1);
-                char *p = reinterpret_cast<char *>(a.dst) + (size_t)b * 2 * term + pix * 8 + (size_t)(chb >> 2) * hw * 8;
-                *reinterpret_cast<s4_h8 *>(p) = hi;
-                *reinterpret_cast<s4_h8 *>(p + term) = mid;
-            } else if (!a.dst_fmt) {
-                typedef float f2 __attribute__((ext_vector_type(2)));
-#pragma unroll
-                for (int r = 0; r < 4; ++r)
-                    if (co + r < a.Cout)
-                        *reinterpret_cast<f2 *>(a.dst + ((size_t)b * a.dst_ctotal + a.dst_choff + co + r) * hw + pix) = f2{v0[r], v1[r]};
-            } else {
-                store_px(co, pix, v0);
-                store_px(co, pix + 1, v1);
-            }
-        };
+#include "conv_s4_1x1_epilogue.inc"
 #pragma unroll
         for (int rr = 0; rr < 2; ++rr) {
             if (pooled && rr == 1) continue;
@@ -457,6 +385,321 @@
     return PF_OK;
 }
 
+template <int NT>
+struct S41ResCfg {
+    static constexpr int TW = 32, TH = 8, NTHR = 512;
+    static constexpr int RBLK = 2 * 64 * 16;
+    static constexpr int WAVES = NT <= 3 ? 4 : 2;
+    static constexpr size_t LDS_MAX = 64 * 1024;
+};
+constexpr bool s41_res_built(int nt, int epi, int r) { return epi == 0 || nt == 4 || (r <= 3 && nt + r <= 5); }
+__host__ __device__ inline int s41_res_bias_bytes(int tiles) { return (tiles * 64 + 255) & ~255; }
+__host__ __device__ inline int s41_res_win_bytes(int nt, int cs) { return (nt * 16 * cs * 4 + 255) & ~255; }
+
+__device__ __forceinline__ float s41_row_partner(float x) {
+    return __int_as_float(__builtin_amdgcn_mov_dpp(__float_as_int(x), 0x128, 0xF, 0xF, true));
+}
+__device__ __forceinline__ bool s41_res_sampled(int n_xy, int ngroups, int tile_lin, int j, int b) {
+    int bx = tile_lin, by = j;
+    if ((n_xy & 7) == 0) {
+        const int per = n_xy >> 3, xcd = tile_lin / per, t = tile_lin - xcd * per;
+        const int lin = ((t * ngroups + j) << 3) + xcd;
+        by = lin / n_xy;
+        bx = lin - by * n_xy;
+    }
+    const unsigned total = (unsigned)n_xy * (unsigned)ngroups * gridDim.z;
+    const unsigned id = (unsigned)bx + (unsigned)n_xy * ((unsigned)by + (unsigned)ngroups * (unsigned)b);
+    const unsigned mask = total >= 16u ? (1u << (28 - __builtin_clz(total))) - 1u : 0u;
+    return (((id * 0x9E3779B1u) >> 9) & mask) == 0u;
+}
+__device__ __forceinline__ void s41_res_range_commit(unsigned *status, unsigned *slot, float m, bool sampled) {
+    if (status == nullptr) return;
+    if (!(m <= kSplitMaxAbs)) atomicOr(status, 1u);
+    if (slot == nullptr || !sampled) return;
+    const unsigned mb = __builtin_bit_cast(unsigned, m);
+    unsigned wm = 0;
+    unsigned long long above = __builtin_amdgcn_ballot_w64(mb > wm);
+    while (above != 0) {
+        wm = (unsigned)__builtin_amdgcn_readlane((int)mb, (int)__builtin_ctzll(above));
+        above = __builtin_amdgcn_ballot_w64(mb > wm);
+    }
+    const unsigned lane_id = __builtin_amdgcn_mbcnt_hi(~0u, __builtin_amdgcn_mbcnt_lo(~0u, 0u));
+    if (lane_id == (unsigned)__builtin_ctzll(__builtin_amdgcn_ballot_w64(true))) atomicMax(slot, wm | 1u);
+}
+
+template <int NT, int EPI, int R>
+__global__ __launch_bounds__(512, S41ResCfg<NT>::WAVES) void conv_s4_1x1_res_kernel(ConvArgs a) {
+#if defined(__HIP_DEVICE_COMPILE__)
+    using C = S41ResCfg<NT>;
+    extern __shared__ __attribute__((aligned(16))) unsigned char smem_raw[];
+    const int tid = threadIdx.x, lane = tid & 63;
+    const int wave = __builtin_amdgcn_readfirstlane(tid >> 6);
+    const int n_xy = a.tilesX * a.tilesY;
+    int tid_lin, cgroup0;
+    xcd_tile_order(n_xy, tid_lin, cgroup0);
+    const int tileY = tid_lin / a.tilesX, tileX = tid_lin - tileY * a.tilesX;
+    const int b = blockIdx.z;
+    const int lg = lane >> 4, i = lane & 15;
+    const int cb = a.chunk_begin;
+    constexpr int nrounds = R;
+    const int ngroups = (a.ntiles + NT - 1) / NT;
+    const size_t plane_bytes = (size_t)a.Hin * a.Win * 8;
+    const int wbytes = NT * nrounds * C::RBLK;
+    float *const bias_all = reinterpret_cast<float *>(smem_raw);
+    unsigned char *const wbuf0 = smem_raw + s41_res_bias_bytes(ngroups * NT);
+    const bool has_res = EPI == 1 && a.res && a.res_lds_off >= 0;
+
+    const int oy = tileY * C::TH + 2 * (wave >> 1) + (i >> 3), ox = tileX * C::TW + 16 * (wave & 1) + 2 * (i & 7);
+    const int poff = (oy < a.Hin && ox < a.Win) ? (oy * a.Win + ox) * 8 : -1;
+
+    const __amdgpu_buffer_rsrc_t wrsrc = __builtin_amdgcn_make_buffer_rsrc((void *)a.wpk, 0, 0x7FFFFFFF, 0x00020000);
+    auto load_weights = [&](int j) {
+        unsigned char *wdst = wbuf0 + (j & 1) * wbytes;
+        if (wave * 64 < nrounds * 128) {
+#pragma unroll
+            for (int n = 0; n < NT; ++n) {
+                const int t = j * NT + n;
+                __builtin_amdgcn_raw_ptr_buffer_load_lds(wrsrc, (s4_lds_ptr_t)(wdst + (n * nrounds * 128 + wave * 64) * 16), 16,
+                                                         t < a.ntiles ? (unsigned)tid * 16u : kS4Oob, (unsigned)(t * a.nchunks + cb) * (unsigned)C::RBLK,
+                                                         0, 0);
+            }
+        }
+    };
+    ResWin rw = ResWin();
+    const size_t rplane = (size_t)a.Hres * a.Wres;
+    const __amdgpu_buffer_rsrc_t rrs = __builtin_amdgcn_make_buffer_rsrc(
+        (void *)(a.res + ((size_t)b * a.res_ctotal + a.res_choff) * (has_res ? rplane : 0)), 0, 0x7FFFFFFF, 0x00020000);
+    int win_floats = 0;
+    if (has_res) {
+        rw = res_window(a, tileY * C::TH, C::TH, tileX * C::TW, C::TW);
+        rw.rows = a.res_rows;
+        rw.cols = a.res_cols;
+        rw.cs = res_chan_stride(a.res_rows, a.res_cols);
+        win_floats = s41_res_win_bytes(NT, rw.cs) / 4;
+    }
+    auto stage_res = [&](int j) {
+        const unsigned per = (unsigned)(rw.rows * rw.cols), total = (unsigned)(NT * 16 * rw.cs);
+        unsigned char *rdst = smem_raw + (size_t)(a.res_lds_off + (j & 1) * win_floats) * 4;
+        for (unsigned e0 = (unsigned)wave * 64; e0 < total; e0 += C::NTHR) {
+            const unsigned e = e0 + lane;
+            const unsigned c = __umulhi(e, a.res_magic_cs), rem = e - c * (unsigned)rw.cs;
+            const unsigned r = __umulhi(rem, a.res_magic_cols), x = rem - r * (unsigned)rw.cols;
+            const int row = min(rw.sy0 + (int)r, a.Hres - 1), col = min(rw.sx0 + (int)x, a.Wres - 1);
+            const unsigned ch = (unsigned)(j * NT * 16) + c;
+            const bool ok = e < total && rem < per && (int)ch < a.Cout;
+            const unsigned off = ok ? (unsigned)((ch * rplane + (size_t)row * a.Wres + col) * 4) : kS4Oob;
+            __builtin_amdgcn_raw_ptr_buffer_load_lds(rrs, (s4_lds_ptr_t)(rdst + e0 * 4), 4, off, 0, 0, 0);
+        }
+    };
+
+    load_weights(0);
+    {
+        const __amdgpu_buffer_rsrc_t brs = __builtin_amdgcn_make_buffer_rsrc((void *)a.bias, 0, 0x7FFFFFFF, 0x00020000);
+        for (int c0 = wave * 64; c0 < ngroups * NT * 16; c0 += C::NTHR) {
+            const int co = c0 + lane;
+            __builtin_amdgcn_raw_ptr_buffer_load_lds(brs, (s4_lds_ptr_t)(bias_all + c0), 4, (!a.no_bias && co < a.ntiles * 16) ? (unsigned)co * 4u : kS4Oob,
+                                                     0, 0, 0);
+        }
+    }
+    s4_u32x4 x[R][2][2];
+#pragma unroll
+    for (int r = 0; r < R; ++r) {
+#pragma unroll
+        for (int h = 0; h < 2; ++h) {
+            const int e = 8 * (cb + r) + 2 * lg + h;
+            const float *sp = a.src[0];
+            int c4 = a.src_c4[0], g0 = a.src_g0[0], gn = a.src_gn[0], e0 = 0;
+#pragma unroll
+            for (int k = 1; k < kConvMaxSrc; ++k) {
+                const bool take = k < a.n_src && e >= a.src_ent0[k];
+                sp = take ? a.src[k] : sp;
+                c4 = take ? a.src_c4[k] : c4;
+                g0 = take ? a.src_g0[k] : g0;
+                gn = take ? a.src_gn[k] : gn;
+                e0 = take ? a.src_ent0[k] : e0;
+            }
+            const bool ok = e - e0 < gn && poff >= 0;
+            const char *hi = reinterpret_cast<const char *>(sp) + ((size_t)b * 2 * c4 + (g0 + min(e - e0, gn - 1))) * plane_bytes;
+            const char *zp = reinterpret_cast<const char *>(a.zero_page);
+            const char *p0 = ok ? hi + poff : zp, *p1 = ok ? hi + poff + (size_t)c4 * plane_bytes : zp + 16;
+            x[r][h][0] = *reinterpret_cast<const s4_u32x4 *>(p0);
+            x[r][h][1] = *reinterpret_cast<const s4_u32x4 *>(p1);
+        }
+    }
+    if (has_res) stage_res(0);
+
+    const bool pooled = EPI == 1 && a.pool;
+    const int Ho = pooled ? a.Hout >> 1 : a.Hout, Wo = pooled ? a.Wout >> 1 : a.Wout;
+    const size_t hw = (size_t)Ho * Wo, term = (size_t)a.dst_c4 * hw * 8;
+    const bool mis = (a.dst_choff & 2) != 0;
+    const bool active = oy < a.Hout && ox < a.Wout && (!pooled || (oy | 1) < a.Hout);
+    int o0_[2] = {0, 0}, o1_[2] = {0, 0};
+    float lx1[2] = {0.f, 0.f}, hy1 = 0.f;
+    if (has_res) {
+        int y0, y1;
+        float hy0;
+        lin_coord(oy, a.res_sh, a.Hres, y0, y1, hy0, hy1);
+#pragma unroll
+        for (int q = 0; q < 2; ++q) {
+            int x0, x1;
+            float lx0;
+            lin_coord(min(ox + q, a.Wout - 1), a.res_sw, a.Wres, x0, x1, lx0, lx1[q]);
+            o0_[q] = (y0 - rw.sy0) * rw.cols + (x0 - rw.sx0);
+            o1_[q] = (y1 - rw.sy0) * rw.cols + (x0 - rw.sx0);
+        }
+    }
+
+    for (int j = 0; j < ngroups; ++j) {
+        asm volatile("s_waitcnt vmcnt(0)" ::: "memory");
+        __builtin_amdgcn_s_waitcnt(0x0F70);
+        __syncthreads();
+        if (j + 1 < ngroups) {
+            load_weights(j + 1);
+            if (has_res) stage_res(j + 1);
+        }
+        const unsigned char *wb = wbuf0 + (j & 1) * wbytes;
+        s4_f32x4 acc[2][NT];
+#pragma unroll
+        for (int q = 0; q < 2; ++q)
+#pragma unroll
+            for (int n = 0; n < NT; ++n) acc[q][n] = s4_f32x4{0.f, 0.f, 0.f, 0.f};
+#pragma unroll
+        for (int r = 0; r < R; ++r) {
+            s4_h8 bh[NT], bm[NT];
+#pragma unroll
+            for (int n = 0; n < NT; ++n) {
+                bh[n] = *reinterpret_cast<const s4_h8 *>(wb + (((n * nrounds + r) * 2 + 0) * 64 + lane) * 16);
+                bm[n] = *reinterpret_cast<const s4_h8 *>(wb + (((n * nrounds + r) * 2 + 1) * 64 + lane) * 16);
+            }
+#pragma unroll
+            for (int q = 0; q < 2; ++q) {
+                const s4_u32x4 h0 = x[r][0][0], h1 = x[r][1][0], m0 = x[r][0][1], m1 = x[r][1][1];
+                const s4_u32x4 fh = q ? s4_u32x4{h0[2], h0[3], h1[2], h1[3]} : s4_u32x4{h0[0], h0[1], h1[0], h1[1]};
+                const s4_u32x4 fm = q ? s4_u32x4{m0[2], m0[3], m1[2], m1[3]} : s4_u32x4{m0[0], m0[1], m1[0], m1[1]};
+                const s4_h8 ah = __builtin_bit_cast(s4_h8, fh), am = __builtin_bit_cast(s4_h8, fm);
+#pragma unroll
+                for (int n = 0; n < NT; ++n) acc[q][n] = PF_MFMA_SPLIT(bh[n], am, acc[q][n]);
+#pragma unroll
+                for (int n = 0; n < NT; ++n) acc[q][n] = PF_MFMA_SPLIT(bm[n], ah, acc[q][n]);
+#pragma unroll
+                for (int n = 0; n < NT; ++n) acc[q][n] = PF_MFMA_SPLIT(bh[n], ah, acc[q][n]);
+            }
+        }
+
+        {
+            int g = lg, o0[2] = {o0_[0], o0_[1]}, o1[2] = {o1_[0], o1_[1]};
+            asm volatile("" : "+v"(g), "+v"(o0[0]), "+v"(o0[1]), "+v"(o1[0]), "+v"(o1[1]));
+            const float *bias_lds = bias_all + j * NT * 16;
+            const lds_float *res_lds = (const lds_float *)(reinterpret_cast<float *>(smem_raw) + (has_res ? a.res_lds_off + (j & 1) * win_floats : 0));
+#include "conv_s4_1x1_epilogue.inc"
+#pragma unroll
+            for (int n = 0; n < NT; ++n) {
+                const int co = (j * NT + n) * 16 + 4 * g;
+                const bool live = active && co < a.Cout + 2;
+                s4_f32x4 va = s4_f32x4{0.f, 0.f, 0.f, 0.f}, vb = va;
+                if (live) {
+                    va = finish(0, 0, n, o0, o1, lx1, hy1);
+                    vb = finish(0, 1, n, o0, o1, lx1, hy1);
+                }
+                if (!pooled) {
+                    if (live) store_pair(co, (size_t)oy * a.Wout + ox, va, vb);
+                } else {
+                    s4_f32x4 vc, vd;
+#pragma unroll
+                    for (int r = 0; r < 4; ++r) {
+                        vc[r] = s41_row_partner(va[r]);
+                        vd[r] = s41_row_partner(vb[r]);
+                    }
+                    if (live && (oy & 1) == 0) {
+                        s4_f32x4 pv;
+#pragma unroll
+                        for (int r = 0; r < 4; ++r) pv[r] = (((va[r] + vb[r]) + vc[r]) + vd[r]) * 0.25f;
+                        if ((oy >> 1) < Ho && (ox >> 1) < Wo) store_px(co, (size_t)(oy >> 1) * Wo + (ox >> 1), pv);
+                    }
+                }
+                __builtin_amdgcn_sched_barrier(0);
+            }
+            s41_res_range_commit(a.status, a.range_slot, vmax, s41_res_sampled(n_xy, ngroups, tid_lin, j, b));
+        }
+    }
+#endif
+}
+
+template <int NT>
+static bool s41_res_fits(const ConvArgs &a, size_t *lds_out, int *res_off) {
+    using C = S41ResCfg<NT>;
+    const int rounds = a.chunk_end - a.chunk_begin, ngroups = (a.ntiles + NT - 1) / NT;
+    if (rounds < 1 || rounds > kS4ResRounds || ngroups < 2) return false;
+    if (!s41_res_built(NT, (a.pool || a.res || a.no_bias) ? 1 : 0, rounds)) return false;
+    size_t lds = (size_t)s41_res_bias_bytes(ngroups * NT) + 2 * (size_t)NT * rounds * C::RBLK;
+    if (res_off) *res_off = (int)(lds / 4);
+    if (a.res) {
+        const int cs = res_chan_stride(res_extent(C::TH, a.res_sh), res_extent(C::TW, a.res_sw));
+        if ((size_t)NT * 16 * cs >= 65536) return false;
+        if ((size_t)a.Cout * a.Hres * a.Wres * 4 >= 0x80000000ull) return false;
+        lds += 2 * (size_t)s41_res_win_bytes(NT, cs);
+    }
+    if (lds_out) *lds_out = lds;
+    return lds <= C::LDS_MAX;
+}
+bool conv_s4_1x1_res_supported(const ConvArgs &a, int nt) {
+    if (!a.src_fmt || (a.Wout & 3) != 0 || a.Hin != a.Hout || a.Win != a.Wout) return false;
+    return nt == 1 ? s41_res_fits<1>(a, nullptr, nullptr) : nt == 2 ? s41_res_fits<2>(a, nullptr, nullptr)
+         : nt == 3 ? s41_res_fits<3>(a, nullptr, nullptr) : nt == 4 ? s41_res_fits<4>(a, nullptr, nullptr) : false;
+}
+
+template <int NT, int EPI, int R>
+static int launch_s41_res_cfg(const ConvArgs &a0, int B, hipStream_t s) {
+    using C = S41ResCfg<NT>;
+    if constexpr (!s41_res_built(NT, EPI, R)) {
+        return fail(PF_EUNSUPPORTED, "conv_s4 1x1 K-resident <%d, %d, %d> is not built", NT, EPI, R);
+    } else {
+    ConvArgs a = a0;
+    a.tilesX = (a.Wout + C::TW - 1) / C::TW;
+    a.tilesY = (a.Hout + C::TH - 1) / C::TH;
+    size_t lds = 0;
+    int res_off = 0;
+    if (!s41_res_fits<NT>(a, &lds, &res_off) || a.chunk_end - a.chunk_begin != R)
+        return fail(PF_EUNSUPPORTED, "conv_s4 1x1 K-resident: %d rounds, %d cout tiles in groups of %d, %zu B of LDS", a.chunk_end - a.chunk_begin, a.ntiles, NT, lds);
+    a.res_lds_off = -1;
+    if (a.res) {
+        a.res_rows = res_extent(C::TH, a.res_sh);
+        a.res_cols = res_extent(C::TW, a.res_sw);
+        const int cs = res_chan_stride(a.res_rows, a.res_cols);
+        a.res_magic_cs = (unsigned)(0x100000000ull / (unsigned)cs) + 1u;
+        a.res_magic_cols = (unsigned)(0x100000000ull / (unsigned)a.res_cols) + 1u;
+        a.res_lds_off = res_off;
+    }
+    static size_t attr_lds = 0;
+    if (lds > attr_lds) {
+        PF_HIP_CHECK(hipFuncSetAttribute(reinterpret_cast<const void *>(&conv_s4_1x1_res_kernel<NT, EPI, R>),
+                                         hipFuncAttributeMaxDynamicSharedMemorySize, (int)lds));
+        attr_lds = lds;
+    }
+    char label[112];
+    snprintf(label, sizeof(label), "void pf::conv_s4_1x1_res_kernel<%d, %d, %d>(pf::ConvArgs)", NT, EPI, R);
+    if (a.res) strncat(label, " +res", sizeof(label) - strlen(label) - 1);
+    if (a.pool) strncat(label, " +pool", sizeof(label) - strlen(label) - 1);
+    if (a.no_bias) strncat(label, " lowres-half", sizeof(label) - strlen(label) - 1);
+    const double px = (double)B * a.Hout * a.Wout;
+    ProfScope ps(s, label, 2.0 * px * a.Cout * a.Cin, 4.0 * ((double)B * a.Cin * a.Hin * a.Win + px * a.Cout + (double)a.Cout * a.Cin));
+    hipLaunchKernelGGL((conv_s4_1x1_res_kernel<NT, EPI, R>), dim3(a.tilesX * a.tilesY, 1, B), dim3(C::NTHR), lds, s, a);
+    PF_LAUNCH_CHECK("conv_s4_1x1_res_kernel");
+    return PF_OK;
+    }
+}
+
+template <int NT, int EPI>
+static int launch_s41_res(const ConvArgs &a, int B, hipStream_t s) {
+    switch (a.chunk_end - a.chunk_begin) {
+        case 1: return launch_s41_res_cfg<NT, EPI, 1>(a, B, s);
+        case 2: return launch_s41_res_cfg<NT, EPI, 2>(a, B, s);
+        case 3: return launch_s41_res_cfg<NT, EPI, 3>(a, B, s);
+        case 4: return launch_s41_res_cfg<NT, EPI, 4>(a, B, s);
+    }
+    return fail(PF_EUNSUPPORTED, "conv_s4 1x1 K-resident: %d rounds", a.chunk_end - a.chunk_begin);
+}
+
 int launch_conv_s4(const ConvArgs &a, int ks, const S4Shape &sh, int B, hipStream_t s) {
     if (!a.src_fmt) return fail(PF_EINVAL, "conv_s4: sources are not in the S4 layout");
     if ((a.Wout & 3) != 0 || a.Hin != a.Hout || a.Win != a.Wout) return fail(PF_EUNSUPPORTED, "conv_s4: stride 1, width % 4 == 0 only");
@@ -479,6 +722,7 @@
     } else if (sh.TW == 32 && sh.TH == 8 && sh.KS == 1) {
         const bool fused = a.pool || a.res || a.no_bias;
 #define PF_S41(NT_) \
+    if (sh.NT == NT_ && sh.RES) return fused ? launch_s41_res<NT_, 1>(a, B, s) : launch_s41_res<NT_, 0>(a, B, s); \
     if (sh.NT == NT_) return fused ? launch_s41_cfg<NT_, 1>(a, B, s) : launch_s41_cfg<NT_, 0>(a, B, s);
         PF_S41(1) PF_S41(2) PF_S41(3) PF_S41(4)
 #undef PF_S41
diff --git a/panoptic-forecasting_amd/csrc/conv_s4_1x1_epilogue.inc b/panoptic-forecasting_amd/csrc/conv_s4_1x1_epilogue.inc
--- /dev/null
+++ b/panoptic-forecasting_amd/csrc/conv_s4_1x1_epilogue.inc
@@ -0,0 +1,73 @@
+        typedef split_x2 h2;
+        float vmax = 0.f;
+        const float relu_lo1 = a.relu ? 0.f : -__builtin_inff();
+        auto finish = [&](int rr, int q, int n, const int (&o0)[2], const int (&o1)[2], const float (&lx1)[2], float hy1) {
+            s4_f32x4 v = acc[rr * 2 + q][n];
+            const s4_f32x4 b4 = *reinterpret_cast<const s4_f32x4 *>(bias_lds + n * 16 + 4 * g);
+#pragma unroll
+            for (int r = 0; r < 4; ++r) {
+                v[r] = v[r] * a.acc_scale + b4[r];
+                if (has_res) {
+                    const lds_float *chan = res_lds + (n * 16 + 4 * g + r) * rw.cs;
+                    const float lx0 = 1.f - lx1[q], hy0 = 1.f - hy1;
+                    const float t0 = lx0 * chan[o0[q]] + lx1[q] * chan[o0[q] + 1];
+                    const float t1 = lx0 * chan[o1[q]] + lx1[q] * chan[o1[q] + 1];
+                    v[r] += hy0 * t0 + hy1 * t1;
+                }
+                v[r] = fmaxf(v[r], relu_lo1);
+            }
+            vmax = range_acc(vmax, v[0], v[1], v[2], v[3]);
+            return v;
+        };
+        auto store_px = [&](int co, size_t pix, s4_f32x4 v) {
+            if (a.dst_fmt) {
+                s4_h4 hi, mid;
+                split_terms4(v, hi, mid);
+                const int chb = a.dst_choff + co;
+                const bool ok0 = chb < a.dst_limit, ok1 = chb + 2 < a.dst_limit;
+                char *p = reinterpret_cast<char *>(a.dst) + (size_t)b * 2 * term + pix * 8 + (size_t)(chb >> 2) * hw * 8;
+                if (!mis) {
+                    if (ok1) {
+                        *reinterpret_cast<s4_h4 *>(p) = hi;
+                        *reinterpret_cast<s4_h4 *>(p + term) = mid;
+                    } else if (ok0) {
+                        *reinterpret_cast<h2 *>(p) = h2{hi[0], hi[1]};
+                        *reinterpret_cast<h2 *>(p + term) = h2{mid[0], mid[1]};
+                    }
+                } else {
+                    if (ok0) {
+                        *reinterpret_cast<h2 *>(p + 4) = h2{hi[0], hi[1]};
+                        *reinterpret_cast<h2 *>(p + 4 + term) = h2{mid[0], mid[1]};
+                    }
+                    if (ok1) {
+                        *reinterpret_cast<h2 *>(p + hw * 8) = h2{hi[2], hi[3]};
+                        *reinterpret_cast<h2 *>(p + hw * 8 + term) = h2{mid[2], mid[3]};
+                    }
+                }
+            } else {
+#pragma unroll
+                for (int r = 0; r < 4; ++r)
+                    if (co + r < a.Cout) a.dst[((size_t)b * a.dst_ctotal + a.dst_choff + co + r) * hw + pix] = v[r];
+            }
+        };
+        auto store_pair = [&](int co, size_t pix, s4_f32x4 v0, s4_f32x4 v1) {
+            const int chb = a.dst_choff + co;
+            if (a.dst_fmt && !mis && chb + 2 < a.dst_limit) {
+                s4_h4 h0, m0, h1, m1;
+                split_terms4(v0, h0, m0);
+                split_terms4(v1, h1, m1);
+                const s4_h8 hi = s4_join(h0, h1), mid = s4_join(m0, m1);
+                char *p = reinterpret_cast<char *>(a.dst) + (size_t)b * 2 * term + pix * 8 + (size_t)(chb >> 2) * hw * 8;
+                *reinterpret_cast<s4_h8 *>(p) = hi;
+                *reinterpret_cast<s4_h8 *>(p + term) = mid;
+            } else if (!a.dst_fmt) {
+                typedef float f2 __attribute__((ext_vector_type(2)));
+#pragma unroll
+                for (int r = 0; r < 4; ++r)
+                    if (co + r < a.Cout)
+                        *reinterpret_cast<f2 *>(a.dst + ((size_t)b * a.dst_ctotal + a.dst_choff + co + r) * hw + pix) = f2{v0[r], v1[r]};
+            } else {
+                store_px(co, pix, v0);
+                store_px(co, pix + 1, v1);
+            }
+        };
diff --git a/panoptic-forecasting_amd/csrc/conv_select.cpp b/panoptic-forecasting_amd/csrc/conv_select.cpp
--- a/panoptic-forecasting_amd/csrc/conv_select.cpp
+++ b/panoptic-forecasting_amd/csrc/conv_select.cpp
@@ -73,6 +73,17 @@
     const int packed = (share_row0(p_cout) + c_cout + 15) / 16, apart = (p_cout + 15) / 16 + (c_cout + 15) / 16;
     if (packed >= apart || pair_wanted(p_cin, p_cout, c_cin, c_cout, h, w, B, 1)) return false;
     return p_cout == 10 && c_cout == 18 && p_cin >= 48 && (long)B * h * w >= 4194304;
+}
+
+bool resident_exists(int cin, int cout, int nt, int rounds) {
+    if (nt < 1 || nt > 4) return false;
+    const int ntiles = (cout + 15) / 16;
+    return cin >= 1 && cin <= 32 * kS4ResRounds && rounds >= 1 && rounds <= kS4ResRounds && (ntiles + nt - 1) / nt > 1;
+}
+bool resident_wanted(int cin, int cout, int h, int w, int B, int fused, int mode) {
+    if (mode >= 2) return true;
+    if (mode <= 0) return false;
+    return cin > 32 && cin <= 96 && (long)B * h * w >= 1048576;
 }
 
 ConvChoice choose_conv(int ks, int stride, int cin, int cout, int hout, int wout, int B, int need, int use_tuned) {
@@ -187,6 +198,11 @@
     return PF_OK;
 }
 
+extern "C" int pf_debug_resident_decision(int ks, int cin, int cout, int hout, int wout, int B, int fused, int nt, int rounds, int mode) {
+    if (ks != 1 && ks != 3) return pf::fail(PF_EINVAL, "pf_debug_resident_decision: ks %d", ks);
+    return ks == 1 && pf::resident_exists(cin, cout, nt, rounds) && pf::resident_wanted(cin, cout, hout, wout, B, fused, mode) ? 1 : 0;
+}
+
 extern "C" int pf_debug_conv_decision(int ks, int stride, int cin, int cout, int hout, int wout, int B, int need, int flags, int rounds,
                                       int *out, int cap) {
     if (!out || cap < 11) return pf::fail(PF_EINVAL, "pf_debug_conv_decision: 11 ints of output");
diff --git a/panoptic-forecasting_amd/csrc/hardnet_plan.h b/panoptic-forecasting_amd/csrc/hardnet_plan.h
--- a/panoptic-forecasting_amd/csrc/hardnet_plan.h
+++ b/panoptic-forecasting_amd/csrc/hardnet_plan.h
@@ -43,6 +43,7 @@
     int profile_tag_ops = 0;
     int fuse_pairs = 1;
     int share_s = 1;
+    int k_resident = 1;
 };
 
 struct pf_plan {
diff --git a/panoptic-forecasting_amd/csrc/hardnet_plan.hip b/panoptic-forecasting_amd/csrc/hardnet_plan.hip
--- a/panoptic-forecasting_amd/csrc/hardnet_plan.hip
+++ b/panoptic-forecasting_amd/csrc/hardnet_plan.hip
@@ -287,7 +287,15 @@
             a.src_fmt = 1; a.acc_scale = cp.split_acc_scale;
             a.wpk = p->dev_weights + cp.s4_off; a.nchunks = cp.s4_rounds;
             set_s4_entries(a, (int)o.k, cp.s4_pad);
-            st.kind = S_CONV_S4; continue;
+            st.kind = S_CONV_S4;
+            S4Shape &sh = st.dec.s4;
+            sh.RES = 0;
+            if (o.k == 1 && p->opt.k_resident && sh.TW == 32 && sh.TH == 8 && sh.KS == 1) {
+                const int fused = (a.pool ? 1 : 0) | (a.res ? 2 : 0) | (a.no_bias ? 4 : 0);
+                sh.RES = resident_exists(a.Cin, a.Cout, sh.NT, a.chunk_end - a.chunk_begin) &&
+                         resident_wanted(a.Cin, a.Cout, a.Hout, a.Wout, Bt, fused, p->opt.k_resident) && conv_s4_1x1_res_supported(a, sh.NT);
+            }
+            continue;
         }
         if ((a.Win & 3) != 0) {
             if (st.need) return fail(PF_EUNSUPPORTED, "fused conv on a width that is not a multiple of 4");
diff --git a/panoptic-forecasting_amd/csrc/plan_create.hip b/panoptic-forecasting_amd/csrc/plan_create.hip
--- a/panoptic-forecasting_amd/csrc/plan_create.hip
+++ b/panoptic-forecasting_amd/csrc/plan_create.hip
@@ -30,6 +30,7 @@
     {"fuse_front", nullptr, &PlanOptions::fuse_front, nullptr, true, true, false},
     {"fuse_pairs", nullptr, &PlanOptions::fuse_pairs, nullptr, true, true, false},
     {"share_s", nullptr, &PlanOptions::share_s, nullptr, true, true, false},
+    {"k_resident", nullptr, &PlanOptions::k_resident, nullptr, true, true, false},
     {"profile_tag_ops", nullptr, &PlanOptions::profile_tag_ops, nullptr, true, true, false},
     {"table_batch", nullptr, &PlanOptions::table_batch, nullptr, false, true, true},
     {"normalize_ranges", nullptr, &PlanOptions::normalize_ranges, nullptr, true, false, false},
diff --git a/panoptic-forecasting_amd/lib.py b/panoptic-forecasting_amd/lib.py
--- a/panoptic-forecasting_amd/lib.py
+++ b/panoptic-forecasting_amd/lib.py
@@ -76,7 +76,8 @@
     'pf_hardnet_plan_set_option': (_i, [_vp, _c.c_char_p, _i]),
     'pf_debug_force_conv': (_i, [_i, _i, _i, _i]),
     'pf_debug_conv_decision': (_i, [_i, _i, _i, _i, _i, _i, _i, _i, _i, _i, _c.POINTER(_i), _i]),
-    'pf_debug_probe_read': (_i, [_c.POINTER(_c.c_longlong)]),
+    'pf_debug_resident_decision': (_i, [_i, _i, _i, _i, _i, _i, _i, _i, _i, _i]),
+    'pf_debug_probe_read':(_i, [_c.POINTER(_c.c_longlong)]),
     'pf_debug_conv_ranges': (_i, [_i, _i, _i, _i, _i, _i, _vp, _vp, _vp, _i, _i, _vp, _sz]),
     'pf_debug_plan_arena': (_i, [_vp, _sz, _i, _i, _vp, _sz, _c.POINTER(_sz), _vp, _i]),
     'pf_debug_train_plan': (_i, [_vp, _sz, _i, _i, _i, _i, _i, _i, _i, _vp, _i, _c.POINTER(_i), _vp, _i, _c.POINTER(_i), _vp]),
```

Result: no change. 2831 frames/s, median of 6 (+0.4%).
